# simon-ging/coot-videotext

Measured on AMD Instinct MI355X. Metric: clip-pairs/sec (COOT retrieval train step, whole job), higher is better.
Workload: dtype bf16; 1 GPU; ActivityNet-shaped paper config (anet_coot): 64 videos x 4 clips per GPU, Lc=Lv=80, Ls=16, Lp=64, Dv=2048, Dt=1536, d_model=384; global_batch_videos=64, parallelism=dp1, mode=train, launch=native, deterministic=True, batches=two different synthetic batches in turn

## Files before the change

### coot-videotext_amd/csrc/api.hip

```cpp
#include <stdarg.h>
#include <stdio.h>
#include <string.h>

#include <algorithm>
#include <mutex>
#include <string>
#include <unordered_map>
#include <vector>

#include "../../include/coot_hip.h"
#include "attention.h"
#include "common.h"
#include "fused.h"
#include "gemm.h"
#include "loss.h"
#include "pool.h"
#include "ref_f32.h"
#include "rowops.h"

namespace coot {

static thread_local char g_err[512] = "";
static thread_local hipStream_t g_glob_flush_stream = nullptr;
static thread_local hipEvent_t g_glob_flush_ev = nullptr;
// ... 454 lines not shown
    }
    f.tstamps = g_fz_tstamps;
    RUN(launch_pre_attn_bwd(f, st));
  } else {
    LnBwd l; l.dy = dz2; l.lddy = D; l.dy32 = dz2_f32; l.lddy32 = lddz2_f32; l.x = b.r2; l.x_f32 = 0; l.ldx = D; l.gain = P + lp.ln2g;
    l.R = rows_q; l.D = D; l.dx = w.dr2; l.lddx = D; l.dgain = G + lp.ln2g; l.dbias = G + lp.ln2b; l.dxcolsum = G + lp.b2;
    if (d_ff2.thr) { l.dxm = w.dr2m; l.lddxm = D; l.dxm_drop = d_ff2; l.dxm_drop_ld = D; }
    RUN(launch_ln_bwd(l, st));
  }
  const bf16_t* df2 = d_ff2.thr ? w.dr2m : w.dr2;
  if (!fused) {
    GemmNT g; g.X = df2; g.ldx = D; g.W = lw.w2_kn; g.ldw = D; g.M = rows_q; g.N = F; g.K = D;
    g.epi.act = 2; g.epi.aux = b.h1; g.epi.ldaux = F; g.epi.colsum = G + lp.b1; g.epi.out = w.dh1; g.epi.ldc = F;
    epi_drop(g.epi, mkdrop(train, pdrop, seed, site_base + SITE_FF1), F);
    RUN(launch_gemm_nt(g, st));
  }
  { GemmTN t; t.A = df2; t.lda = D; t.B = b.a1; t.ldb = F; t.T = rows_q; t.Mo = D; t.No = F; t.C = G + lp.w2; t.ldc = F; RUN(launch_gemm_tn(t, st)); }
  if (!fused) {
    GemmNT g; g.X = w.dh1; g.ldx = F; g.W = lw.w1_kn; g.ldw = F; g.M = rows_q; g.N = D; g.K = F;
    g.epi.res = w.dr2; g.epi.ldres = D; g.epi.out = w.dz1; g.epi.ldc = D;
    RUN(launch_gemm_nt(g, st));
  }
  { GemmTN t; t.A = w.dh1; t.lda = F; t.B = b.z1; t.ldb = D; t.T = rows_q; t.Mo = F; t.No = D; t.C = G + lp.w1; t.ldc = D; RUN(launch_gemm_tn(t, st)); }
  if (!fused) {
    LnBwd l; l.dy = w.dz1; l.lddy = D; l.x = b.r1; l.x_f32 = 0; l.ldx = D; l.gain = P + lp.ln1g; l.R = rows_q; l.D = D;
    l.dx = w.dr1; l.lddx = D; l.dgain = G + lp.ln1g; l.dbias = G + lp.ln1b; l.dxcolsum = G + lp.bo;
    l.drop = mkdrop(train, pdrop, seed, site_base + SITE_POSTLN);
    RUN(launch_ln_bwd(l, st));
  }
  if (!fused) {
    GemmNT g; g.X = w.dr1; g.ldx = D; g.W = lw.wo_kn; g.ldw = D; g.M = rows_q; g.N = D; g.K = D; g.epi.out = w.dctx; g.epi.ldc = D;
    RUN(launch_gemm_nt(g, st));
  }
  { GemmTN t; t.A = w.dr1; t.lda = D; t.B = b.ctx; t.ldb = D; t.T = rows_q; t.Mo = D; t.No = D; t.C = G + lp.wo; t.ldc = D; RUN(launch_gemm_tn(t, st)); }
  AttnArgs a; a.q = b.q; a.ldq = b.ldq; a.k = b.k; a.ldk = b.ldk; a.v = b.v; a.ldv = b.ldv; a.o = b.ctx; a.ldo = D; a.lse = b.lse;
  a.H = H; a.dh = dh; a.scale = 1.0f / sqrtf((float)dh);
  a.drop = mkdrop(train, pdrop, seed, site_base + SITE_ATTN);
  a.dout = w.dctx; a.lddo = D; a.delta = w.delta; a.dq = w.dq; a.lddq = w.lddq; a.dk = w.dk; a.lddk = w.lddk; a.dv = w.dv; a.lddv = w.lddv;
  RUN(attention_all(a, sg, !self, true, st));
  if (self) {
    { GemmTN t; t.A = w.dq; t.lda = 3 * D; t.B = xq; t.ldb = D; t.T = rows_q; t.Mo = 3 * D; t.No = D; t.C = G + lp.wqkv; t.ldc = D;
      t.a_colsum = G + lp.bq; RUN(launch_gemm_tn(t, st)); }
    if (qkv_bwd_is_fused(lw, rows_q, dxq_f32 != nullptr, part_ws)) {
      QkvBwd f; f.T = rows_q; f.dqkv = w.dq; f.wqkv = lw.f_wqkv_kn; f.res = w.dr1; f.aux = gelu_aux; f.dz = dxq; f.colsum = gelu_colsum; f.part = part_ws;
      f.colsum_overwrite = 1;
      RUN(launch_qkv_bwd(f, st));
    } else {
      GemmNT g; g.X = w.dq; g.ldx = 3 * D; g.W = lw.wqkv_kn; g.ldw = 3 * D; g.M = rows_q; g.N = D; g.K = 3 * D;
      g.epi.res = w.dr1; g.epi.ldres = D;
      if (gelu_aux) { g.epi.act = 2; g.epi.aux = gelu_aux; g.epi.ldaux = D; g.epi.colsum = gelu_colsum; }
      if (dxq_f32) { g.epi.out = dxq_f32; g.epi.out_f32 = 1; } else g.epi.out = dxq;
      g.epi.ldc = D;
      RUN(launch_gemm_nt(g, st));
    }
  } else {
    { GemmTN t; t.A = w.dq; t.lda = w.lddq; t.B = xq; t.ldb = D; t.T = rows_q; t.Mo = D; t.No = D; t.C = G + lp.wqkv; t.ldc = D;
      t.a_colsum = G + lp.bq; RUN(launch_gemm_tn(t, st)); }
    { GemmTN t; t.A = w.dk; t.lda = w.lddk; t.B = xkv; t.ldb = D; t.T = rows_kv; t.Mo = 2 * D; t.No = D; t.C = G + lp.wqkv + (size_t)D * D; t.ldc = D;
      t.a_colsum = G + lp.bk; RUN(launch_gemm_tn(t, st)); }
    {
      GemmNT g; g.X = w.dq; g.ldx = w.lddq; g.W = lw.wqkv_kn; g.ldw = 3 * D; g.M = rows_q; g.N = D; g.K = D;
      g.epi.res = w.dr1; g.epi.ldres = D;
      if (dxq_f32) { g.epi.out = dxq_f32; g.epi.out_f32 = 1; } else g.epi.out = dxq;
      g.epi.ldc = D;
      RUN(launch_gemm_nt(g, st));
    }
    {
      GemmNT g; g.X = w.dk; g.ldx = w.lddk; g.W = lw.wqkv_kn + D; g.ldw = 3 * D; g.M = rows_kv; g.N = D; g.K = 2 * D;
      g.epi.res = dxkv_accum; g.epi.ldres = D; g.epi.out = dxkv_accum; g.epi.ldc = D;
      RUN(launch_gemm_nt(g, st));
    }
  }
  return 0;
}

static int g_use_glob_fused_bwd = 1;
static int g_use_glob_fused = 1;
static bool glob_fused_ok(const coot_net_config& c, const Segs& sg) {
  return g_use_fused && g_use_glob_fused && fused_layer_ok(c) && c.num_heads == 8 && c.use_context && !c.use_input_fc && c.pooler != 0 &&
         c.num_layers == 1 && c.ctx_num_layers == 1 && sg.n == 1 && glob_fwd_supported(sg.L[0]);
}

static int g_use_packed = 1;
static bool packed_ok(const coot_net_config& c, const WPack& W, const Segs& sg, const coot_packed_seqs* pk) {
  if (!g_use_packed || !pk || !pk->cu_seqlens || pk->total_tokens <= 0) return false;
  return g_use_fused && g_use_fused_infc && c.use_input_fc && !c.use_context && fused_pool_ok(c) && W.f_in_w && W.f_pw1 &&
         W.f_pw1_kn && c.input_dim % 64 == 0 && pk->total_tokens >= g_fused_min_rows && pk->total_tokens <= sg.Tpad() &&
         attn_short_path(sg.L[0]) && (sg.n == 1 || attn_short_path(sg.L[1]));
}

static LayerBufs self_bufs(const LayerS& s, int D) {
  LayerBufs b; b.q = s.qkv; b.ldq = 3 * D; b.k = s.qkv + D; b.ldk = 3 * D; b.v = s.qkv + 2 * D; b.ldv = 3 * D;
  b.ctx = s.ctx; b.r1 = s.r1; b.z1 = s.z1; b.h1 = s.h1; b.a1 = s.a1; b.r2 = s.r2; b.z2 = s.z2; b.lse = s.lse;
  return b;
}
static LayerBufs ctx_bufs(const CtxS& s, int D) {
  LayerBufs b; b.q = s.q; b.ldq = D; b.k = s.kv; b.ldk = 2 * D; b.v = s.kv + D; b.ldv = 2 * D;
  b.ctx = s.cctx; b.r1 = s.r1; b.z1 = s.z1; b.h1 = s.h1; b.a1 = s.a1; b.r2 = s.r2; b.z2 = s.z2; b.lse = s.lse;
  return b;
}

}

using namespace coot;

extern "C" {

const char* coot_last_error(void) { return coot::g_err; }
int coot_version(void) { return COOT_ABI_VERSION; }
int coot_debug_dropout_scales(uint64_t seed, unsigned site, uint64_t idx0, int64_t n, float p, float* out_host) {
  COOT_REQUIRE(out_host && n >= 0 && p > 0.f, "debug_dropout_scales: bad arguments");
  const DropCfg d = mkdrop(1, p, seed, site);
  const unsigned key = drop_key(seed, site);
  for (int64_t i = 0; i < n; ++i) out_host[i] = drop_scale_key(key, idx0 + (uint64_t)i, d.thr, d.inv_keep);
  return 0;
}
int coot_debug_attn_dropout_scales(uint64_t seed, unsigned site, unsigned row32, int Lk, float p, float* out_host) {
  COOT_REQUIRE(out_host && Lk >= 0 && p > 0.f, "debug_attn_dropout_scales: bad arguments");
  const DropCfg d = mkdrop(1, p, seed, site);
  const unsigned key = drop_key(seed, site);
  for (int k = 0; k < Lk; ++k) out_host[k] = attn_drop_scale(key, row32, k, (unsigned)(Lk + 1) >> 1, d.thr, d.inv_keep);
  return 0;
}
int coot_debug_timestamps(void* dev_u64) { g_fz_tstamps = (unsigned long long*)dev_u64; return 0; }
extern "C" void coot_step_stamps_enable(int on);
extern "C" void coot_step_grad_write(int on);
extern "C" void coot_step_det_seg_flush(int on);
extern "C" int coot_step_det_seg_flush_get(void);
extern "C" int coot_internal_stage_hits(void);
extern "C" void coot_step_text_ahead(int on);
extern "C" int coot_step_text_ahead_get(void);
extern "C" int coot_internal_text_ahead_steps(void);
extern "C" int coot_internal_stream_counter(int which);
extern "C++" { namespace coot { int det_bypass_count(); int det_overflow_count(); int det_set_overflow_guard(int on); int det_overflow_guard(); } }
extern "C++" { namespace coot { void set_rt_topk_splits(int n); int get_rt_topk_splits(); void set_rt_few_splits(int n); int get_rt_few_splits(); void set_rt_grouped_splits(int n); int get_rt_grouped_splits(); void set_rt_knn_splits(int n); int get_rt_knn_splits(); void set_rt_comp_blocks_per_wg(int n); int get_rt_comp_blocks_per_wg(); } }
int coot_get_option(const char* name, int* value) {
  if (!value) { set_error("get_option: null result"); return -1; }
  if (!strcmp(name, "tn_dma")) { *value = get_tn_dma(); return 0; }
  if (!strcmp(name, "xcd_order")) { *value = get_xcd_order(); return 0; }
  if (!strcmp(name, "tn_mode")) { *value = get_tn_mode(); return 0; }
  if (!strcmp(name, "stage_hits")) { *value = coot_internal_stage_hits(); return 0; }
  if (!strcmp(name, "text_ahead")) { *value = coot_step_text_ahead_get(); return 0; }
  if (!strcmp(name, "text_ahead_steps")) { *value = coot_internal_text_ahead_steps(); return 0; }
  if (!strcmp(name, "fused_attn_launches")) { *value = fused_attn_launches(); return 0; }
  if (!strcmp(name, "stream_overlap_tests")) { *value = coot_internal_stream_counter(0); return 0; }
  if (!strcmp(name, "stream_candidates_rejected")) { *value = coot_internal_stream_counter(1); return 0; }
  if (!strcmp(name, "stream_unresolved")) { *value = coot_internal_stream_counter(2); return 0; }
  if (!strcmp(name, "operand_f16")) { *value = COOT_OPERAND_IS_F16; return 0; }
  if (!strcmp(name, "det_seg_flush")) { *value = coot_step_det_seg_flush_get(); return 0; }
  if (!strcmp(name, "det_bypasses")) { *value = det_bypass_count(); return 0; }
  if (!strcmp(name, "det_overflows")) { *value = det_overflow_count(); return 0; }
  if (!strcmp(name, "det_overflow_check")) { *value = det_overflow_guard(); return 0; }
  if (!strcmp(name, "attn_bwd_loop")) { *value = get_attn_bwd_loop(); return 0; }
  if (!strcmp(name, "attn_bwd_share")) { *value = get_attn_bwd_share(); return 0; }
  if (!strcmp(name, "attn_bwd_grid")) { *value = get_attn_bwd_grid(); return 0; }
  if (!strcmp(name, "rt_topk_splits")) { *value = get_rt_topk_splits(); return 0; }
  if (!strcmp(name, "rt_few_splits")) { *value = get_rt_few_splits(); return 0; }
  if (!strcmp(name, "rt_grouped_splits")) { *value = get_rt_grouped_splits(); return 0; }
  if (!strcmp(name, "rt_knn_splits")) { *value = get_rt_knn_splits(); return 0; }
  if (!strcmp(name, "rt_comp_blocks_per_wg")) { *value = get_rt_comp_blocks_per_wg(); return 0; }
  set_error("get_option: unknown or write-only option %s", name);
  return -2;
}
int coot_set_option(const char* name, int value) {
  if (!strcmp(name, "tn_mode")) { set_tn_mode(value); return 0; }
  if (!strcmp(name, "step_stamps")) { coot_step_stamps_enable(value); return 0; }
  if (!strcmp(name, "fused")) { g_use_fused = value; return 0; }
  if (!strcmp(name, "glob_fused")) { g_use_glob_fused = value; return 0; }
  if (!strcmp(name, "glob_fused_bwd")) { g_use_glob_fused_bwd = value; return 0; }
  if (!strcmp(name, "packed")) { g_use_packed = value; return 0; }
  if (!strcmp(name, "fused_infc")) { g_use_fused_infc = value; return 0; }
  if (!strcmp(name, "fused_attn")) { set_fused_attn(value); return 0; }
  if (!strcmp(name, "tn_dma")) { set_tn_dma(value); return 0; }
  if (!strcmp(name, "pack_lazy")) { g_pack_lazy = value; return 0; }
  if (!strcmp(name, "pack_poison")) { g_pack_poison = value; return 0; }
  if (!strcmp(name, "grad_poison")) { g_grad_poison = value; return 0; }
  if (!strcmp(name, "tn_target_wgs")) { set_tn_target_wgs(value); return 0; }
  if (!strcmp(name, "xcd_order")) { set_xcd_order(value); return 0; }
  if (!strcmp(name, "grad_write")) { coot_step_grad_write(value); return 0; }
  if (!strcmp(name, "det_seg_flush")) { coot_step_det_seg_flush(value); return 0; }
  if (!strcmp(name, "text_ahead")) { coot_step_text_ahead(value); return 0; }
  if (!strcmp(name, "det_overflow_check")) return det_set_overflow_guard(value);
  if (!strcmp(name, "glob_flush_aux")) { g_glob_flush_aux = value; return 0; }
  if (!strcmp(name, "pool_handover")) { g_pool_handover_on = value; return 0; }
  if (!strcmp(name, "cl_col_split")) { set_cl_col_split(value); return 0; }
  if (!strcmp(name, "cl_small")) { set_cl_small(value); return 0; }
  if (!strcmp(name, "fz_debug")) { g_fz_debug = value; return 0; }
  if (!strcmp(name, "fused_min_rows")) { g_fused_min_rows = value; return 0; }
  if (!strcmp(name, "attn_bwd_loop")) { set_attn_bwd_loop(value); return 0; }
  if (!strcmp(name, "attn_bwd_share")) { set_attn_bwd_share(value); return 0; }
  if (!strcmp(name, "attn_bwd_grid")) { set_attn_bwd_grid(value); return 0; }
  if (!strcmp(name, "rt_topk_splits")) { set_rt_topk_splits(value); return 0; }
  if (!strcmp(name, "rt_few_splits")) { set_rt_few_splits(value); return 0; }
  if (!strcmp(name, "rt_grouped_splits")) { set_rt_grouped_splits(value); return 0; }
  if (!strcmp(name, "rt_knn_splits")) { set_rt_knn_splits(value); return 0; }
  if (!strcmp(name, "rt_comp_blocks_per_wg")) { set_rt_comp_blocks_per_wg(value); return 0; }
  set_error("unknown option %s", name);
  return -2;
}

int64_t coot_net_param_numel(const coot_net_config* cfg) {
  coot_net_config c; if (norm_cfg(cfg, &c)) return -1;
  NetLayout L; build_layout(c, L); return L.total;
}
int coot_net_param_count(const coot_net_config* cfg) {
  coot_net_config c; if (norm_cfg(cfg, &c)) return -1;
  NetLayout L; build_layout(c, L); return (int)L.entries.size();
}
int coot_net_param_info(const coot_net_config* cfg, int index, char* name, int name_len, int64_t* offset, int64_t shape[4], int* ndim) {
  coot_net_config c; RUN(norm_cfg(cfg, &c));
  NetLayout L; build_layout(c, L);
  COOT_REQUIRE(index >= 0 && index < (int)L.entries.size(), "param index %d out of range", index);
  const PEntry& e = L.entries[index];
  snprintf(name, name_len, "%s", e.name.c_str());
  *offset = e.off; *ndim = e.ndim;
  for (int i = 0; i < 4; ++i) shape[i] = e.shape[i];
  return 0;
}
int coot_net_out_dim(const coot_net_config* cfg) { return cfg->hidden_dim * (cfg->use_context ? 2 : 1); }

size_t coot_net_wpack_bytes(const coot_net_config* cfg) {
  coot_net_config c; if (norm_cfg(cfg, &c)) return 0;
  Arena A(nullptr, 0); WPack W; layout_wpack(c, A, W); return A.off + 256;
}

enum { PACK_ALL = 0, PACK_FUSED = 1, PACK_PEROP_REST = 2 };
struct PackState { bool perop_fresh = false, perop_wanted = false; };
static std::mutex g_pack_mu;
static std::unordered_map<const void*, PackState> g_pack_state;
static PackState pack_state_get(const void* wpack) { std::lock_guard<std::mutex> lk(g_pack_mu); auto it = g_pack_state.find(wpack); return it == g_pack_state.end() ? PackState() : it->second; }
static void pack_state_set(const void* wpack, PackState s) { std::lock_guard<std::mutex> lk(g_pack_mu); g_pack_state[wpack] = s; }

static int pack_net_jobs(const coot_net_config* cfg, const float* P, void* wpack, const float* P0, void* wpack0, PackJobs& jobs, hipStream_t st,
                         int mode = PACK_ALL, bool* has_lazy = nullptr) {
  coot_net_config c; RUN(norm_cfg(cfg, &c));
  const int64_t pd = P - P0;
  NetLayout L; build_layout(c, L);
  Arena A(wpack, (size_t)-1); WPack W; layout_wpack(c, A, W);
  const int D = c.hidden_dim, F = c.ff_dim, Din = c.input_dim;
  auto flush = [&]() -> int { int rc = launch_pack_jobs(P0, wpack0, jobs, st); jobs.n = 0; jobs.mv = PackMatvec(); return rc; };
  auto add = [&](int64_t src_off, long lds, int R, int Cc, bf16_t* dst, long ldd, int transpose, int64_t colscale_off) -> int {
    if (jobs.n == 56) RUN(flush());
    PackJob& j = jobs.j[jobs.n++];
    j.src_off = src_off + pd; j.dst_byte_off = (char*)dst - (char*)wpack0; j.R = R; j.C = Cc; j.lds = lds; j.ldd = ldd;
    j.transpose = transpose; j.p48 = 0; j.colscale_off = colscale_off >= 0 ? colscale_off + pd : -1;
    return 0;
  };
  auto add48 = [&](int64_t src_off, long lds, int R, int Cc, bf16_t* dst, int transpose) -> int {
    RUN(add(src_off, lds, R, Cc, dst, 0, transpose, -1));
    jobs.j[jobs.n - 1].p48 = 1;
    return 0;
  };
  bool lazy = false;
  auto perop = [&](bool has_fused) { if (has_fused && mode == PACK_FUSED) lazy = true; return mode == PACK_ALL || (mode == PACK_FUSED ? !has_fused : has_fused); };
  const bool fused_on = mode != PACK_PEROP_REST;
  auto poison = [&](bf16_t* dst, size_t elems) -> int {
    if (!g_pack_poison || mode != PACK_FUSED) return 0;
    return check_hip(hipMemsetAsync(dst, 0xFF, elems * sizeof(bf16_t), st), "poison");
  };
  if (c.use_input_fc) {
    if (perop(W.f_in_w != nullptr)) RUN(add(L.in_w, Din, D, Din, W.in_w, Din, 0, L.n_gain));
    else RUN(poison(W.in_w, (size_t)D * Din));
    if (W.f_in_w && fused_on) { RUN(add(L.in_w, Din, D, Din, W.f_in_w, 0, 0, L.n_gain)); jobs.j[jobs.n - 1].p48 = 1; }
    if (fused_on) { jobs.mv.W = P + L.in_w; jobs.mv.ldw = Din; jobs.mv.N = D; jobs.mv.K = Din; jobs.mv.v = P + L.n_bias; jobs.mv.b = P + L.in_b; jobs.mv.out = W.in_bias; }
  }
  auto pack_layer = [&](const LayerP& lp, const LayerW& lw) -> int {
    if (perop(lw.f_wo != nullptr)) {
      RUN(add(lp.wqkv, D, 3 * D, D, lw.wqkv_nk, D, 0, -1));
      RUN(add(lp.wqkv, D, 3 * D, D, lw.wqkv_kn, 3 * D, 1, -1));
      RUN(add(lp.wo, D, D, D, lw.wo_nk, D, 0, -1));
      RUN(add(lp.wo, D, D, D, lw.wo_kn, D, 1, -1));
      RUN(add(lp.w1, D, F, D, lw.w1_nk, D, 0, -1));
      RUN(add(lp.w1, D, F, D, lw.w1_kn, F, 1, -1));
      RUN(add(lp.w2, F, D, F, lw.w2_nk, F, 0, -1));
      RUN(add(lp.w2, F, D, F, lw.w2_kn, D, 1, -1));
    } else {
      RUN(poison(lw.wqkv_nk, (size_t)(6 * D * D + 4 * F * D)));
    }
    if (lw.f_wo && fused_on) {
      RUN(add48(lp.wo, D, D, D, lw.f_wo, 0));
      RUN(add48(lp.w1, D, F, D, lw.f_w1, 0));
      RUN(add48(lp.w2, F, D, F, lw.f_w2, 0));
      RUN(add48(lp.wo, D, D, D, lw.f_wo_kn, 1));
      RUN(add48(lp.w1, D, F, D, lw.f_w1_kn, 1));
      RUN(add48(lp.w2, F, D, F, lw.f_w2_kn, 1));
      RUN(add48(lp.wqkv, D, 3 * D, D, lw.f_wqkv, 0));
      RUN(add48(lp.wqkv, D, 3 * D, D, lw.f_wqkv_kn, 1));
    }
    return 0;
  };
  for (int i = 0; i < c.num_layers; ++i) RUN(pack_layer(L.layers[i], W.layers[i]));
  for (size_t i = 0; i < L.ctx.size(); ++i) RUN(pack_layer(L.ctx[i], W.ctx[i]));
  if (c.pooler == 0) {
    const int H = c.pool_heads, PH = c.pool_hidden, dhp = PH / H, dop = D / H;
    const bool pool_perop = perop(W.f_pw1 != nullptr);
    if (!pool_perop) RUN(poison(W.pw1_nk, (size_t)(2 * PH * D + 2 * PH * dop)));
    for (int h = 0; h < H; ++h) {
      if (pool_perop) {
        RUN(add(L.pw1 + (int64_t)h * D * dhp, dhp, D, dhp, W.pw1_nk + (size_t)h * dhp * D, D, 1, -1));
        RUN(add(L.pw1 + (int64_t)h * D * dhp, dhp, D, dhp, W.pw1_kn + (size_t)h * dhp, PH, 0, -1));
        RUN(add(L.pw2 + (int64_t)h * dhp * dop, dop, dhp, dop, W.pw2_nk + (size_t)h * dop * dhp, dhp, 1, -1));
        RUN(add(L.pw2 + (int64_t)h * dhp * dop, dop, dhp, dop, W.pw2_kn + (size_t)h * dhp * dop, dop, 0, -1));
      }
      if (W.f_pw1 && fused_on) {
        RUN(add48(L.pw1 + (int64_t)h * D * dhp, dhp, D, dhp, W.f_pw1 + (size_t)h * dhp * D, 1));
        RUN(add48(L.pw2 + (int64_t)h * dhp * dop, dop, dhp, dop, W.f_pw2 + (size_t)h * dop * dhp, 1));
        RUN(add48(L.pw1 + (int64_t)h * D * dhp, dhp, D, dhp, W.f_pw1_kn + (size_t)h * D * dhp, 0));
        RUN(add48(L.pw2 + (int64_t)h * dhp * dop, dop, dhp, dop, W.f_pw2_kn + (size_t)h * dhp * dop, 0));
      }
    }
  }
  if (has_lazy) *has_lazy = lazy;
  return 0;
}

struct PerOpGuard { bool armed = false; coot_net_config cfg; const float* P = nullptr; void* wpack = nullptr; const char* lo[8]; const char* hi[8]; int n = 0; };
static thread_local PerOpGuard g_guard;
static int perop_weight_hook(const void* Wp, hipStream_t st) {
  PerOpGuard& G = g_guard;
  if (!G.armed) return 0;
  bool hit = false;
  for (int i = 0; i < G.n && !hit; ++i) hit = (const char*)Wp >= G.lo[i] && (const char*)Wp < G.hi[i];
  if (!hit) return 0;
  G.armed = false;
  PackJobs jobs;
  RUN(pack_net_jobs(&G.cfg, G.P, G.wpack, G.P, G.wpack, jobs, st, PACK_PEROP_REST));
  RUN(launch_pack_jobs(G.P, G.wpack, jobs, st));
  PackState ps; ps.perop_fresh = true; ps.perop_wanted = true;
  pack_state_set(G.wpack, ps);
  return 0;
}
struct PerOpGuardScope {
  PerOpGuardScope(const coot_net_config& c, const WPack& W, const float* P, const void* wpack) {
    PerOpGuard& G = g_guard;
    G.armed = false;
    if (pack_state_get(wpack).perop_fresh) return;
// ... 498 lines not shown
```

### coot-videotext_amd/csrc/fused.h

```cpp
#pragma once
#include "common.h"
#include "rowops.h"

namespace coot {

constexpr int FZ_D = 384;

__host__ __device__ inline long p48_offset(int n, int k, int K) {
  const int g = n / 48, b = (n % 48) / 16, r = n % 16, kb = k / 32, q = (k % 32) / 8, e = k % 8;
  return ((((long)g * (K / 32) + kb) * 3 + b) * 64 + (q * 16 + r)) * 8 + e;
}

struct FusedAttn {
  int on = 0;
  const bf16_t* qkv = nullptr;
  float* lse = nullptr;
  int N0 = 0, L0 = 0, N1 = 0, L1 = 0;
  const long long *lens0 = nullptr, *lens1 = nullptr;
  DropCfg drop; unsigned long long seed2_delta = 0;
  float scale = 0.f;
};
constexpr int FZ_ATTN_RP(int) { return 56; }
constexpr int FZ_ATTN_LMAX(int RF) { return RF == 8 ? 80 : 64; }
constexpr int FZ_ATTN_SMEM(int RF) { return RF >= 4 ? 8 * 2 * FZ_ATTN_LMAX(RF) * FZ_ATTN_RP(RF) * 2 : 0; }
struct PostAttnFwd {
  int T = 0;
  FusedAttn attn;
  bf16_t* ctx_w = nullptr;
  const bf16_t* ctx = nullptr;
  const bf16_t* xres = nullptr;
  const bf16_t *wo = nullptr, *w1 = nullptr, *w2 = nullptr, *pw1 = nullptr, *pw2 = nullptr;
  const float *bo = nullptr, *ln1g = nullptr, *ln1b = nullptr, *b1 = nullptr, *b2 = nullptr, *ln2g = nullptr, *ln2b = nullptr,
              *pb1 = nullptr, *pb2 = nullptr;
  bf16_t *r1 = nullptr, *z1 = nullptr, *h1 = nullptr, *a1 = nullptr, *r2 = nullptr, *z2 = nullptr;
  float* z2_f32 = nullptr; long ldz2_f32 = 0;
  int do_pool = 0;
  bf16_t *hp = nullptr, *ap = nullptr, *s = nullptr;
  DropCfg d_postln, d_ff1, d_ff2, d_pool1, d_pool2;
  unsigned long long* tstamps = nullptr;
};
int launch_post_attn_fwd(const PostAttnFwd& p, hipStream_t st);
bool post_attn_can_fuse_attention(int T, bool do_pool, int N0, int L0, int N1, int L1);
void set_fused_attn(int on);
int fused_attn_launches();

struct PreAttnBwd {
  int T = 0;
  int do_pool = 0;
  const bf16_t *ds = nullptr, *dzp = nullptr;
  const bf16_t* dz2 = nullptr;
  const bf16_t *hp = nullptr, *h1 = nullptr, *r2 = nullptr, *r1 = nullptr;
  const bf16_t *pw2 = nullptr, *pw1 = nullptr, *w2 = nullptr, *w1 = nullptr, *wo = nullptr;
  const float *ln2g = nullptr, *ln1g = nullptr;
  bf16_t *dhp = nullptr, *dr2 = nullptr, *dr2m = nullptr, *dh1 = nullptr, *dr1 = nullptr, *dctx = nullptr;
  float* part = nullptr;
  float *g_pb1 = nullptr, *g_ln2g = nullptr, *g_ln2b = nullptr, *g_b2 = nullptr, *g_b1 = nullptr, *g_ln1g = nullptr, *g_ln1b = nullptr,
        *g_bo = nullptr;
  DropCfg d_pool1, d_ff2, d_ff1, d_postln;
  unsigned long long* tstamps = nullptr;
};
struct InfcQkvFwd {
  int T = 0, Din = 0;
  const bf16_t* xhat = nullptr;
  const bf16_t* win = nullptr;
  const float* bin = nullptr;
  const float* pe = nullptr; int T0 = 0, L1 = 1, L2 = 1;
  const int* pos = nullptr;
  const bf16_t* wqkv = nullptr; const float* bqkv = nullptr;
  bf16_t *h0 = nullptr, *z0 = nullptr, *qkv = nullptr;
  unsigned long long* tstamps = nullptr;
};
int launch_infc_qkv_fwd(const InfcQkvFwd& p, hipStream_t st);

struct QkvFwd { int T = 0; const bf16_t* z = nullptr; const bf16_t* wqkv = nullptr; const float* bias = nullptr; bf16_t* qkv = nullptr; };
int launch_qkv_fwd(const QkvFwd& p, hipStream_t st);

struct QkvBwd {
  int T = 0;
  const bf16_t* dqkv = nullptr;
  const bf16_t* wqkv = nullptr;
  const bf16_t* res = nullptr;
  const bf16_t* aux = nullptr;
  bf16_t* dz = nullptr;
  float* colsum = nullptr;
  int colsum_overwrite = 0;
  float* part = nullptr;
};
int launch_qkv_bwd(const QkvBwd& p, hipStream_t st);

struct GlobLayerFwd {
  const bf16_t *wqkv = nullptr, *wo = nullptr, *w1 = nullptr, *w2 = nullptr;
  const float *bqkv = nullptr, *bo = nullptr, *ln1g = nullptr, *ln1b = nullptr, *b1 = nullptr, *b2 = nullptr, *ln2g = nullptr, *ln2b = nullptr;
  bf16_t* q = nullptr; long ldq = 0; bf16_t* k = nullptr; long ldk = 0; bf16_t* v = nullptr; long ldv = 0;
  bf16_t *ctx = nullptr, *r1 = nullptr, *z1 = nullptr, *h1 = nullptr, *a1 = nullptr, *r2 = nullptr, *z2 = nullptr; float* lse = nullptr;
  DropCfg d_attn, d_postln, d_ff1, d_ff2;
};
struct GlobFwd {
  int B = 0, Cmax = 0;
  const float* x = nullptr;
  const long long* lens = nullptr;
  const float* hidden = nullptr;
  const float* pe = nullptr;
  const float *n_gain = nullptr, *n_bias = nullptr;
  GlobLayerFwd self, ctx;
  bf16_t *z0 = nullptr, *cq_in = nullptr;
  float* pooled = nullptr;
  float* per_token = nullptr;
  int train = 0;
  int tiles = 0, warm_per_xcd = 0, xcd_first = 0, xcd_count = 8, tiles_per_xcd = 0;
  unsigned long long* tstamps = nullptr;
};
int launch_glob_fwd(const GlobFwd& p, hipStream_t st);
bool glob_fwd_supported(int Cmax);

struct GlobLayerBwd {
  const bf16_t *wqkv_kn = nullptr, *wo_kn = nullptr, *w1_kn = nullptr, *w2_kn = nullptr;
  const float *ln1g = nullptr, *ln2g = nullptr;
  const bf16_t* q = nullptr; long ldq = 0; const bf16_t* k = nullptr; long ldk = 0; const bf16_t* v = nullptr; long ldv = 0;
  const bf16_t *r1 = nullptr, *h1 = nullptr, *r2 = nullptr; const float* lse = nullptr;
  bf16_t *dr2 = nullptr, *dr2m = nullptr, *dh1 = nullptr, *dr1 = nullptr;
  bf16_t* dq = nullptr; long lddq = 0; bf16_t* dk = nullptr; long lddk = 0; bf16_t* dv = nullptr; long lddv = 0;
  float *g_ln2g = nullptr, *g_ln2b = nullptr, *g_ln1g = nullptr, *g_ln1b = nullptr;
  DropCfg d_attn, d_postln, d_ff1, d_ff2;
};
struct GlobBwd {
  int B = 0, Cmax = 0;
  const float* x = nullptr;
  const long long* lens = nullptr;
  const float* n_gain = nullptr;
  const float* dpooled = nullptr;
  GlobLayerBwd self, ctx;
  float* dx = nullptr;
  float* dhidden = nullptr;
  float *g_n_gain = nullptr, *g_n_bias = nullptr;
  int tiles = 0, warm_per_xcd = 0, xcd_first = 0, xcd_count = 8, tiles_per_xcd = 0;
  unsigned long long* tstamps = nullptr;
};
int launch_glob_bwd(const GlobBwd& p, hipStream_t st);
void glob_xcd_set(int first, int count);

constexpr int FZ_BWD_NCS = 9 * FZ_D;
bool half_tiles(int T, int kernel);
int launch_pre_attn_bwd(const PreAttnBwd& p, hipStream_t st);

}
```

### coot-videotext_amd/csrc/fused.hip

```cpp
#include "fused.h"
#include "det.h"
#include "gemm.h"

#include <type_traits>

namespace coot {
namespace {

constexpr int APITCH = 400;
constexpr int SPITCH = 388;
constexpr int NTHR = 512;
constexpr long GSZ = 12L * 3 * 512;

__device__ __forceinline__ void unpack8(u32x4_t u, float* v) {
  v[0] = bflo(u[0]); v[1] = bfhi(u[0]); v[2] = bflo(u[1]); v[3] = bfhi(u[1]);
  v[4] = bflo(u[2]); v[5] = bfhi(u[2]); v[6] = bflo(u[3]); v[7] = bfhi(u[3]);
}
__device__ __forceinline__ u32x4_t pack8(const float* v) {
  return u32x4_t{pack2bf(v[0], v[1]), pack2bf(v[2], v[3]), pack2bf(v[4], v[5]), pack2bf(v[6], v[7])};
}
__device__ __forceinline__ void load8f(const float* p, float* v) {
  const f32x4_t a = reinterpret_cast<const f32x4_t*>(p)[0], b = reinterpret_cast<const f32x4_t*>(p)[1];
  v[0] = a[0]; v[1] = a[1]; v[2] = a[2]; v[3] = a[3]; v[4] = b[0]; v[5] = b[1]; v[6] = b[2]; v[7] = b[3];
}
__device__ __forceinline__ void drop8(const DropCfg& d, unsigned long long idx0, float* sc) {
  drop_scales<8>(eff_seed(d.seed, d.seed_ptr), d.site, idx0, d.thr, d.inv_keep, sc);
}

__device__ __forceinline__ u32x4_t gld16(const void* base, unsigned boff) {
  return *reinterpret_cast<const u32x4_t*>(reinterpret_cast<const char*>(base) + boff);
}
__device__ __forceinline__ void gst16(void* base, unsigned boff, u32x4_t v) {
#ifdef FZ_NO_STORES
  if (boff != 0xFFFFFFF0u) return;
#endif
  *reinterpret_cast<u32x4_t*>(reinterpret_cast<char*>(base) + boff) = v;
}

#ifdef FZ_XCDS
__device__ __forceinline__ int fz_tile_index(int ntiles) {
  const int x = blockIdx.x & 7;
  if (x >= FZ_XCDS) return -1;
  const int t = (blockIdx.x >> 3) * FZ_XCDS + x;
  return t < ntiles ? t : -1;
}
static inline int fz_grid(int tiles) { return (tiles + FZ_XCDS - 1) / FZ_XCDS * 8; }
#else
__device__ __forceinline__ int fz_tile_index(int) { return blockIdx.x; }
static inline int fz_grid(int tiles) { return tiles; }
#endif

__device__ __forceinline__ void lds_barrier() { asm volatile("s_waitcnt lgkmcnt(0)\n\ts_barrier" ::: "memory"); }

template <int RF>
__device__ __forceinline__ void zero_acc(f32x4_t (&acc)[RF][3]) {
#pragma unroll
  for (int a = 0; a < RF; ++a)
#pragma unroll
    for (int b = 0; b < 3; ++b) acc[a][b] = f32x4_t{0.f, 0.f, 0.f, 0.f};
}

constexpr int kPdFull = 2;
#ifndef FZ_PD_SMALL
#define FZ_PD_SMALL 5
#endif
constexpr int kPdSmall = FZ_PD_SMALL;
constexpr int kCarryMaxRF = 4;
template <int PD_, bool CARRY_>
struct WRing { static constexpr int PD = PD_, NB = PD_ + 1; static constexpr bool CARRY = CARRY_; bf16x8_t w[PD_ + 1][3]; };
template <int RF> using TileRing = WRing<(RF <= 2 ? kPdSmall : kPdFull), (RF <= kCarryMaxRF)>;

template <typename Ring>
__device__ __forceinline__ void gemm_load_first(Ring& R, const bf16_t* wg, int lane) {
  const bf16x8_t* wp = reinterpret_cast<const bf16x8_t*>(wg) + lane;
#ifndef FZ_NO_WLOAD
#pragma unroll
  for (int s = 0; s < Ring::PD; ++s)
#pragma unroll
    for (int b = 0; b < 3; ++b) R.w[s][b] = wp[(s * 3 + b) * 64];
#else
  (void)wp;
#endif
  __builtin_amdgcn_sched_barrier(0);
}
template <typename Ring>
__device__ __forceinline__ void gemm_issue(Ring& R, const bf16_t* wg, int lane) {
  if constexpr (Ring::CARRY) gemm_load_first(R, wg, lane);
}

template <int RF, int KB, bool NEXT, typename Ring>
__device__ __forceinline__ void gemm_run(Ring& R, const bf16_t* As, const bf16_t* wg, const bf16_t* next, f32x4_t (&acc)[RF][3], int lane) {
  constexpr int PD = Ring::PD, NB = Ring::NB;
  static_assert(KB % NB == 0 && KB >= PD, "the ring must wrap at the end of a pass");
  asm volatile("" : "+v"(lane));
  if constexpr (!Ring::CARRY) gemm_load_first(R, wg, lane);
  const bf16_t* arow = As + (lane & 15) * APITCH + (lane >> 4) * 8;
  const bf16x8_t* wp = reinterpret_cast<const bf16x8_t*>(wg) + lane;
  const bf16x8_t* np = reinterpret_cast<const bf16x8_t*>(next) + lane;
  bf16x8_t xf[RF];
#pragma unroll
  for (int a = 0; a < RF; ++a) xf[a] = *reinterpret_cast<const bf16x8_t*>(arow + a * 16 * APITCH);
#pragma unroll
  for (int kb = 0; kb < KB; ++kb) {
#ifndef FZ_NO_WLOAD
    if (kb + PD < KB) {
#pragma unroll
      for (int b = 0; b < 3; ++b) R.w[(kb + PD) % NB][b] = wp[((kb + PD) * 3 + b) * 64];
    } else if constexpr (NEXT && Ring::CARRY) {
#pragma unroll
      for (int b = 0; b < 3; ++b) R.w[(kb + PD) % NB][b] = np[((kb + PD - KB) * 3 + b) * 64];
    }
#else
    (void)wp; (void)np;
#endif
    __builtin_amdgcn_sched_barrier(0);
#pragma unroll
    for (int a = 0; a < RF; ++a) {
#pragma unroll
      for (int b = 0; b < 3; ++b) {
#ifndef FZ_NO_MFMA
        acc[a][b] = COOT_MFMA_16x16x32(R.w[kb % NB][b], xf[a], acc[a][b]);
#else
        acc[a][b][0] += __builtin_bit_cast(float, (int)(__builtin_bit_cast(u32x4_t, R.w[kb % NB][b])[0] ^ __builtin_bit_cast(u32x4_t, xf[a])[b]));
#endif
      }
      if (kb + 1 < KB) xf[a] = *reinterpret_cast<const bf16x8_t*>(arow + a * 16 * APITCH + (kb + 1) * 32);
    }
  }
}

template <int RF, int CPR = 48>
__device__ __forceinline__ void load_tile(bf16_t* As, const bf16_t* src, long ld, int col0, int row0) {
  constexpr int CH = 16 * RF * CPR, IT = (CH + NTHR - 1) / NTHR;
  asm volatile("" : "+s"(row0));
  u32x4_t v[IT];
#pragma unroll
  for (int i = 0; i < IT; ++i) {
    const int c = threadIdx.x + NTHR * i, rl = c / CPR, ch = c - rl * CPR;
    v[i] = u32x4_t{0u, 0u, 0u, 0u};
    if (CH % NTHR == 0 || c < CH) v[i] = gld16(src, (unsigned)((row0 + rl) * (int)ld + col0 + ch * 8) * 2u);
  }
#pragma unroll
  for (int i = 0; i < IT; ++i) {
    const int c = threadIdx.x + NTHR * i, rl = c / CPR, ch = c - rl * CPR;
    if (CH % NTHR == 0 || c < CH) *reinterpret_cast<u32x4_t*>(&As[rl * APITCH + ch * 8]) = v[i];
  }
}

template <int NCH, int IT>
__device__ __forceinline__ void load_bias(const float* bias, float (&bs)[IT][8]) {
#pragma unroll
  for (int i = 0; i < IT; ++i) load8f(bias + ((threadIdx.x + NTHR * i) % NCH) * 8, bs[i]);
}

template <int RF, int NCG, typename PreF, typename Fn>
__device__ __forceinline__ void epilogue(f32x4_t (&acc)[RF * NCG / 8][3], float* Stg, bf16_t* As, int row0, const float* bias_lds,
                                         PreF pre, Fn fn, bool to_lds, unsigned long long* prof = nullptr) {
#ifdef FZ_PROFILE_EPI
  unsigned long long pt[7] = {0, 0, 0, 0, 0, 0, 0}, pacc[6] = {0, 0, 0, 0, 0, 0};
  const bool profiling = prof && blockIdx.x == 0 && threadIdx.x == 0;
#define FZ_PT(k) do { if (prof) { asm volatile("s_waitcnt lgkmcnt(0)" ::: "memory"); pt[k] = __builtin_amdgcn_s_memtime(); } } while (0)
#else
#define FZ_PT(k) do { } while (0)
#endif
  constexpr int RR = RF >= 2 ? 32 : 16, FR = RR / 16, RPR = (NCG == 8 ? RR : 2 * RR), ROUNDS = 16 * RF / RPR, CH = RR * 48, IT = CH / NTHR;
  static_assert(CH % NTHR == 0 && IT == 3 && ROUNDS <= 4 && (NCG == 8 || (NCG == 4 && ((ROUNDS == 2 && RF == 8) || (ROUNDS == 1 && RF == 4)))),
                "tile pass geometry");
  int tid = threadIdx.x;
  asm volatile("" : "+v"(tid));
  const int lane = tid & 63, wave = tid >> 6;
  const int cg = wave % NCG, rh = wave / NCG;
  int rl[IT], col[IT];
#pragma unroll
  for (int i = 0; i < IT; ++i) {
    const int c = tid + NTHR * i, r_ = c / 48, ch = c - r_ * 48;
    if constexpr (NCG == 8) { rl[i] = r_; col[i] = ch * 8; }
    else { rl[i] = r_ + (ch >= 24 ? 32 : 0); col[i] = (ch >= 24 ? ch - 24 : ch) * 8; }
  }
  float bs[IT][8];
  if (bias_lds) {
#pragma unroll
    for (int i = 0; i < IT; ++i) load8f(bias_lds + col[i], bs[i]);
  }
  using P = decltype(pre(0, 0));
  P pv[IT];
#pragma unroll
  for (int i = 0; i < IT; ++i) pv[i] = pre(row0 + rl[i], col[i]);
  float* sw = &Stg[(lane & 15) * SPITCH + cg * 48 + (lane >> 4) * 4];
#pragma unroll 1
  for (int r = 0; r < ROUNDS; ++r) {
    FZ_PT(0);
    lds_barrier();
    FZ_PT(1);
#ifndef FZ_NO_STAGING
    if constexpr (NCG == 8) {
      auto put = [&](auto rc) {
        constexpr int R = decltype(rc)::value;
        if constexpr (R < ROUNDS) {
#pragma unroll
          for (int a2 = 0; a2 < FR; ++a2)
#pragma unroll
            for (int b = 0; b < 3; ++b) *reinterpret_cast<f32x4_t*>(sw + a2 * 16 * SPITCH + b * 16) = acc[R * FR + a2][b];
          asm volatile("" ::: "memory");
        }
      };
      switch (r) {
        case 0: put(std::integral_constant<int, 0>{}); break;
        case 1: put(std::integral_constant<int, 1>{}); break;
        case 2: put(std::integral_constant<int, 2>{}); break;
        default: put(std::integral_constant<int, 3>{}); break;
      }
    } else if constexpr (RF == 8) {
      if (rh == r) {
#pragma unroll
        for (int a = 0; a < 4; ++a)
#pragma unroll
          for (int b = 0; b < 3; ++b) *reinterpret_cast<f32x4_t*>(sw + (a & 1) * 16 * SPITCH + (a >> 1) * 192 + b * 16) = acc[a][b];
      }
    } else {
#pragma unroll
      for (int a = 0; a < 2; ++a)
#pragma unroll
        for (int b = 0; b < 3; ++b) *reinterpret_cast<f32x4_t*>(sw + a * 16 * SPITCH + rh * 192 + b * 16) = acc[a][b];
    }
#else
    if (r == 0) {
#pragma unroll
      for (int a = 0; a < RF * NCG / 8; ++a)
#pragma unroll
        for (int b = 0; b < 3; ++b) asm volatile("" :: "v"(acc[a][b]));
    }
#endif
    const int rbase = row0 + r * RPR;
    FZ_PT(2);
    lds_barrier();
    FZ_PT(3);
    float v[IT][8];
#pragma unroll
    for (int i = 0; i < IT; ++i) load8f(&Stg[(rl[i] & 31) * SPITCH + col[i] + (rl[i] >= 32 ? 192 : 0)], v[i]);
    FZ_PT(4);
#pragma unroll
    for (int i = 0; i < IT; ++i) {
      if (bias_lds) {
#pragma unroll
        for (int j = 0; j < 8; ++j) v[i][j] += bs[i][j];
      }
      fn(rbase + rl[i], col[i], v[i], pv[i], i);
      __builtin_amdgcn_sched_barrier(0);
    }
    FZ_PT(5);
    if (to_lds) {
#pragma unroll
      for (int i = 0; i < IT; ++i) *reinterpret_cast<u32x4_t*>(&As[(r * RPR + rl[i]) * APITCH + col[i]]) = pack8(v[i]);
    }
    if (r + 1 < ROUNDS) {
#pragma unroll
      for (int i = 0; i < IT; ++i) pv[i] = pre(rbase + RPR + rl[i], col[i]);
    }
    FZ_PT(6);
#ifdef FZ_PROFILE_EPI
    if (prof) {
#pragma unroll
      for (int k = 0; k < 6; ++k) pacc[k] += pt[k + 1] - pt[k];
    }
#endif
  }
  lds_barrier();
#ifdef FZ_PROFILE_EPI
  if (profiling) {
#pragma unroll
    for (int k = 0; k < 6; ++k) prof[k] = pacc[k];
  }
#endif
#undef FZ_PT
}

__device__ __forceinline__ float row16_sum(float v) {
  auto dpp = [](float x, auto ctrl) {
    return __builtin_bit_cast(float, __builtin_amdgcn_update_dpp(0, __builtin_bit_cast(int, x), decltype(ctrl)::value, 0xF, 0xF, false));
  };
  v += dpp(v, std::integral_constant<int, 0xB1>{});
  v += dpp(v, std::integral_constant<int, 0x4E>{});
  v += dpp(v, std::integral_constant<int, 0x141>{});
  v += dpp(v, std::integral_constant<int, 0x140>{});
  return v;
}

struct DropK { unsigned key = 0, thr = 0; float inv_keep = 1.f; };
__device__ __forceinline__ DropK resolve_drop(const DropCfg& d, unsigned long long base) {
  DropK k; k.key = drop_key(d.seed + base, d.site); k.thr = d.thr; k.inv_keep = d.inv_keep; return k;
}

__device__ __forceinline__ float attn_drop_f(unsigned key, unsigned row, int k, unsigned lk_half, unsigned thr, float inv_keep) {
  return attn_drop_scale(key, row, k, lk_half, thr, inv_keep);
}

template <bool DROP>
__device__ __forceinline__ void apply_drop(const DropK& d, unsigned long long idx0, float (&v)[8]) {
#ifdef FZ_NO_EPI_MATH
  return;
#endif
  if constexpr (DROP) {
    float sc[8];
    drop_scales_key<8>(d.key, idx0, d.thr, d.inv_keep, sc);
#pragma unroll
    for (int j = 0; j < 8; ++j) v[j] *= sc[j];
  }
}

template <bool DROP>
__device__ __forceinline__ void mask_from_saved(const DropK& d, const float (&saved)[8], float (&v)[8]) {
  if constexpr (DROP) {
#ifdef FZ_NO_EPI_MATH
    return;
#endif
#pragma unroll
    for (int j = 0; j < 8; ++j) v[j] = saved[j] != 0.0f ? v[j] * d.inv_keep : 0.0f;
  }
}

template <int RF, bool DROP, bool OUT32, bool MASK = false>
__device__ __forceinline__ void ln_tile(bf16_t* As, const float* gain, const float* bias, int row0, int T, bf16_t* out, float* out32,
                                        long ld32, const DropK& drop) {
#ifdef FZ_NO_LN
  return;
#endif
  asm volatile("" : "+s"(row0));
  const int lane = threadIdx.x & 63, wave = threadIdx.x >> 6, j16 = lane & 15, g = lane >> 4;
  constexpr int RW = 2 * RF, ITR = (RW + 3) / 4;
  float gn[3][8], bi[3][8];
#pragma unroll
  for (int m = 0; m < 3; ++m) { load8f(gain + m * 128 + j16 * 8, gn[m]); load8f(bias + m * 128 + j16 * 8, bi[m]); }
#pragma unroll
  for (int it = 0; it < ITR; ++it) {
    const int rw = (RW >= 4) ? it * 4 + g : (g < RW ? g : 0);
    const int rl = wave * RW + rw, row = row0 + rl;
    bf16_t* ar = As + rl * APITCH + j16 * 8;
    float x[3][8];
    float s = 0.f;
#pragma unroll
    for (int m = 0; m < 3; ++m) {
      unpack8(*reinterpret_cast<const u32x4_t*>(ar + m * 128), x[m]);
#pragma unroll
      for (int e = 0; e < 8; ++e) s += x[m][e];
    }
    const float mean = row16_sum(s) * (1.0f / 384.0f);
    float q = 0.f;
#pragma unroll
    for (int m = 0; m < 3; ++m)
#pragma unroll
      for (int e = 0; e < 8; ++e) { x[m][e] -= mean; q += x[m][e] * x[m][e]; }
    const float rs = 1.0f / (sqrtf(row16_sum(q) * (1.0f / 383.0f)) + kLnEps);
#pragma unroll
    for (int m = 0; m < 3; ++m) {
      float y[8];
#pragma unroll
      for (int e = 0; e < 8; ++e) y[e] = x[m][e] * rs * gn[m][e] + bi[m][e];
      if constexpr (DROP) {
        float sc[8];
        drop_scales_key<8>(drop.key, (unsigned long long)row * FZ_D + m * 128 + j16 * 8, drop.thr, drop.inv_keep, sc);
#pragma unroll
        for (int e = 0; e < 8; ++e) y[e] *= sc[e];
      }
      const u32x4_t o = pack8(y);
      *reinterpret_cast<u32x4_t*>(ar + m * 128) = o;
      if (!MASK || row < T) gst16(out, (unsigned)(row * FZ_D + m * 128 + j16 * 8) * 2u, o);
      if constexpr (OUT32) {
        if (row < T) {
          float* o32 = out32 + (long)row * ld32 + m * 128 + j16 * 8;
          *reinterpret_cast<f32x4_t*>(o32) = f32x4_t{y[0], y[1], y[2], y[3]};
          *reinterpret_cast<f32x4_t*>(o32 + 4) = f32x4_t{y[4], y[5], y[6], y[7]};
        }
      }
    }
  }
}

struct PreNone {};
struct PreRes { u32x4_t res; };

template <int RF>
__device__ __forceinline__ void fused_self_attn(const PostAttnFwd& p, bf16_t* As, unsigned char* smem_base, int row0, unsigned long long sbase) {
  constexpr int DH = 48, RP = FZ_ATTN_RP(RF), NK = DH / 16, H = 8, CPR = DH / 8, LDQ = 3 * FZ_D, LMAX = FZ_ATTN_LMAX(RF);
  const FusedAttn& A = p.attn;
  int tid = threadIdx.x;
  asm volatile("" : "+v"(tid));
  const int lane = tid & 63, h = tid >> 6, lq = lane & 15, lg = lane >> 4;
  const int T0 = A.N0 * A.L0;
  const bool second = row0 >= T0;
  const int L = second ? A.L1 : A.L0, segbase = second ? T0 : 0, segend = second ? p.T : T0;
  const long long* lens = second ? A.lens1 : A.lens0;
  const int last = (row0 + 16 * RF < segend ? row0 + 16 * RF : segend) - 1;
  const int s_first = (row0 - segbase) / L, s_last = (last - segbase) / L;
  const int nkt = L >> 4;
  const unsigned dkey = A.drop.thr ? drop_key(A.drop.seed + (second ? A.seed2_delta : 0ull) + sbase, A.drop.site) : 0u;
  bf16_t* Ks = reinterpret_cast<bf16_t*>(smem_base) + h * (2 * LMAX * RP);
  bf16_t* Vs = Ks + LMAX * RP;
  u32x2_t out[RF][NK];
#pragma unroll
  for (int f = 0; f < RF; ++f)
#pragma unroll
    for (int dt = 0; dt < NK; ++dt) out[f][dt] = u32x2_t{0u, 0u};
  const int half = L * CPR;
  constexpr bool QALL = RF <= 4;
  s16x4_t qall[QALL ? RF : 1][NK];
  if constexpr (QALL) {
#pragma unroll
    for (int f = 0; f < RF; ++f)
#pragma unroll
      for (int ks = 0; ks < NK; ++ks) {
        qall[f][ks] = s16x4_t{0, 0, 0, 0};
        if (row0 + 16 * f < segend) qall[f][ks] = *reinterpret_cast<const s16x4_t*>(A.qkv + (long)(row0 + 16 * f + lq) * LDQ + h * DH + ks * 16 + lg * 4);
      }
  }
  constexpr int NH = (LMAX * CPR + 63) / 64;
  u32x4_t sk[NH], sv[NH];
  auto ld = [&](int kb0, int kv, u32x4_t (&st)[NH]) {
#pragma unroll
    for (int i = 0; i < NH; ++i) {
      const int c = lane + 64 * i, r = c / CPR, ch = c - r * CPR;
      st[i] = u32x4_t{0u, 0u, 0u, 0u};
      if (c < half) st[i] = gld16(A.qkv, (unsigned)((kb0 + r) * LDQ + FZ_D * (1 + kv) + h * DH + ch * 8) * 2u);
    }
  };
  auto sto = [&](bf16_t* dst, const u32x4_t (&st)[NH]) {
#pragma unroll
    for (int i = 0; i < NH; ++i) {
      const int c = lane + 64 * i, r = c / CPR, ch = c - r * CPR;
      if (c < half) *reinterpret_cast<u32x4_t*>(&dst[r * RP + ch * 8]) = st[i];
    }
  };
  constexpr bool KVPRE = RF <= 4;
  if constexpr (KVPRE) { ld(segbase + s_first * L, 0, sk); ld(segbase + s_first * L, 1, sv); }
#pragma unroll 1
  for (int sq = s_first; sq <= s_last; ++sq) {
    const int kbase = segbase + sq * L;
    if constexpr (!KVPRE) { ld(kbase, 0, sk); ld(kbase, 1, sv); }
    asm volatile("s_waitcnt lgkmcnt(0)" ::: "memory");
    sto(Ks, sk);
    sto(Vs, sv);
    if constexpr (KVPRE) { if (sq < s_last) { ld(kbase + L, 0, sk); ld(kbase + L, 1, sv); } }
    asm volatile("s_waitcnt lgkmcnt(0)" ::: "memory");
    const int nvalid = (int)lens[sq];
    const int f_lo = kbase > row0 ? (kbase - row0) >> 4 : 0;
    const int f_hi_row = (kbase + L < row0 + 16 * RF ? kbase + L : row0 + 16 * RF);
    const int f_hi = ((f_hi_row < segend ? f_hi_row : segend) - row0) >> 4;
    s16x4_t qnext[NK];
    auto qload = [&](int f, s16x4_t (&q)[NK]) {
#pragma unroll
      for (int ks = 0; ks < NK; ++ks) q[ks] = *reinterpret_cast<const s16x4_t*>(A.qkv + (long)(row0 + 16 * f + lq) * LDQ + h * DH + ks * 16 + lg * 4);
    };
    if constexpr (!QALL) { if (f_lo < f_hi) qload(f_lo, qnext); }
#pragma unroll
    for (int f = 0; f < RF; ++f) {
      if (f >= f_lo && f < f_hi) {
        const int g0 = row0 + 16 * f, qpos = g0 - kbase + lq;
        s16x4_t qf[NK];
#pragma unroll
        for (int ks = 0; ks < NK; ++ks) {
          if constexpr (QALL) qf[ks] = qall[f][ks];
          else qf[ks] = qnext[ks];
        }
        if constexpr (!QALL) { if (f + 1 < f_hi) qload(f + 1, qnext); }
        f32x4_t sc[LMAX / 16];
        float mx = -INFINITY;
#pragma unroll
        for (int kt = 0; kt < LMAX / 16; ++kt) {
          if (kt < nkt) {
            sc[kt] = f32x4_t{0.f, 0.f, 0.f, 0.f};
#pragma unroll
            for (int ks = 0; ks < NK; ++ks) {
              const s16x4_t kf = *reinterpret_cast<const s16x4_t*>(&Ks[(kt * 16 + lq) * RP + ks * 16 + lg * 4]);
              sc[kt] = COOT_MFMA_16x16x16(kf, qf[ks], sc[kt]);
            }
#pragma unroll
            for (int i = 0; i < 4; ++i) {
              float v = sc[kt][i] * A.scale;
              if (kt * 16 + lg * 4 + i >= nvalid) v = kMaskFill;
              sc[kt][i] = v;
              mx = fmaxf(mx, v);
            }
          }
        }
        mx = fmaxf(mx, __shfl_xor(mx, 16, 64));
        mx = fmaxf(mx, __shfl_xor(mx, 32, 64));
        float sum = 0.f;
        s16x4_t pf[LMAX / 16];
#pragma unroll
        for (int kt = 0; kt < LMAX / 16; ++kt) {
          if (kt < nkt) {
            float pr[4];
#pragma unroll
            for (int i = 0; i < 4; ++i) {
              pr[i] = __expf(sc[kt][i] - mx);
              sum += pr[i];
              if (A.drop.thr)
                pr[i] *= attn_drop_f(dkey, (unsigned)((sq * H + h) * L + qpos), kt * 16 + lg * 4 + i, (unsigned)(L + 1) >> 1, A.drop.thr, A.drop.inv_keep);
            }
            const unsigned lo = pack2bf(pr[0], pr[1]), hi = pack2bf(pr[2], pr[3]);
            pf[kt] = s16x4_t{(short)(lo & 0xFFFF), (short)(lo >> 16), (short)(hi & 0xFFFF), (short)(hi >> 16)};
          }
        }
        sum += __shfl_xor(sum, 16, 64);
        sum += __shfl_xor(sum, 32, 64);
        const float inv = 1.0f / sum;
#pragma unroll
        for (int dt = 0; dt < NK; ++dt) {
          f32x4_t o = f32x4_t{0.f, 0.f, 0.f, 0.f};
#pragma unroll
          for (int kt = 0; kt < LMAX / 16; ++kt) {
            if (kt < nkt) {
              const bf16_t* addr = &Vs[(kt * 16) * RP + dt * 16] + (4 * lg + (lq >> 2)) * RP + (lq & 3) * 4;
              const s16x4_t vt = __builtin_amdgcn_ds_read_tr16_b64_v4i16((s16x4_t __attribute__((address_space(3)))*)(addr));
              o = COOT_MFMA_16x16x16(vt, pf[kt], o);
            }
          }
          out[f][dt] = u32x2_t{pack2bf(o[0] * inv, o[1] * inv), pack2bf(o[2] * inv, o[3] * inv)};
        }
// ... 298 lines not shown
    const int col = ((tid + NTHR * i) % 48) * 8;
    lds_barrier();
    *reinterpret_cast<f32x4_t*>(&red[k * FZ_D + col]) = f32x4_t{cs[i][0], cs[i][1], cs[i][2], cs[i][3]};
    *reinterpret_cast<f32x4_t*>(&red[k * FZ_D + col + 4]) = f32x4_t{cs[i][4], cs[i][5], cs[i][6], cs[i][7]};
    lds_barrier();
    if (tid < FZ_D) {
      const int ch = (tid / 8 + 48 * 2 - 32 * i) % 48;
      const int nk = (NTHR - ch + 47) / 48;
      for (int kk = 0; kk < nk; ++kk) tot += red[kk * FZ_D + tid];
    }
  }
  if (tid < FZ_D) dst[tid] = tot;
}

template <int RF, bool DROP>
__global__ __launch_bounds__(512) void pre_attn_bwd_kernel(PreAttnBwd p) {
  constexpr int BT = 16 * RF, RR = 32;
  constexpr long GSZ192 = 6L * 3 * 512;
  __shared__ __attribute__((aligned(16))) unsigned char smem[BT * APITCH * 2 + RR * SPITCH * 4 + 4 * FZ_D * 4];
  bf16_t* As = reinterpret_cast<bf16_t*>(smem);
  float* Stg = reinterpret_cast<float*>(smem + BT * APITCH * 2);
  float* Bsm = reinterpret_cast<float*>(smem + BT * APITCH * 2 + RR * SPITCH * 4);
  float* zero = Bsm, *g2 = Bsm + FZ_D, *g1 = Bsm + 2 * FZ_D, *cred = Bsm + 3 * FZ_D;
  const int lane = threadIdx.x & 63, wave = threadIdx.x >> 6;
  const int row0 = blockIdx.x * BT, T = p.T;
  float* part = p.part + (long)blockIdx.x * FZ_BWD_NCS;
  if (threadIdx.x < FZ_D / 4) {
    reinterpret_cast<f32x4_t*>(zero)[threadIdx.x] = f32x4_t{0.f, 0.f, 0.f, 0.f};
    reinterpret_cast<f32x4_t*>(g2)[threadIdx.x] = reinterpret_cast<const f32x4_t*>(p.ln2g)[threadIdx.x];
    reinterpret_cast<f32x4_t*>(g1)[threadIdx.x] = reinterpret_cast<const f32x4_t*>(p.ln1g)[threadIdx.x];
  }
  f32x4_t acc[RF][3];
  float cs[3][8];
  int tsn = 0;
  auto stamp = [&]() {
    unsigned long long* ts = p.tstamps;
    asm volatile("" : "+s"(ts));
    if (ts && blockIdx.x == 0 && threadIdx.x == 0) ts[tsn] = __builtin_amdgcn_s_memtime();
    ++tsn;
  };
  unsigned long long sbase = 0;
  if constexpr (DROP) { if (p.d_ff1.seed_ptr) sbase = *p.d_ff1.seed_ptr; }
  const DropK d_postln = resolve_drop(p.d_postln, sbase), d_ff1 = resolve_drop(p.d_ff1, sbase), d_ff2 = resolve_drop(p.d_ff2, sbase),
                d_pool1 = resolve_drop(p.d_pool1, sbase);
  stamp();
  auto cs_zero = [&]() {
#pragma unroll
    for (int i = 0; i < 3; ++i)
#pragma unroll
      for (int j = 0; j < 8; ++j) cs[i][j] = 0.f;
  };

  TileRing<RF> R;
  auto WG = [&](const bf16_t* base, int grp, long gsz) { asm volatile("" : "+v"(grp)); return base + grp * gsz; };
  if (p.do_pool) {
    gemm_issue(R, WG(p.pw2, wave, GSZ192), lane);
#pragma unroll 1
    for (int h = 0; h < 2; ++h) {
      load_tile<RF, 24>(As, p.ds, FZ_D, h * (FZ_D / 2), row0);
      __syncthreads();
      zero_acc<RF>(acc);
      gemm_run<RF, 6, true>(R, As, WG(p.pw2, h * 8 + wave, GSZ192), h == 0 ? WG(p.pw2, 8 + wave, GSZ192) : WG(p.pw1, 8 + wave, GSZ), acc, lane);
      cs_zero();
      epilogue<RF, 8>(acc, Stg, As, row0, nullptr,
          [&](int row, int col) { return PreRes{gld16(p.hp, (unsigned)(row * (2 * FZ_D) + h * FZ_D + col) * 2u)}; },
          [&](int row, int col, float (&v)[8], const PreRes& pr, int i) {
            float a[8];
            unpack8(pr.res, a);
#pragma unroll
            for (int j = 0; j < 8; ++j) v[j] *= gelu_grad_f(a[j]);
#ifdef FZ_HASH_BWD_MASKS
            apply_drop<DROP>(d_pool1, (unsigned long long)row * (2 * FZ_D) + h * FZ_D + col, v);
#else
            mask_from_saved<DROP>(d_pool1, a, v);
#endif
            if (row < T) {
#pragma unroll
              for (int j = 0; j < 8; ++j) cs[i][j] += v[j];
            }
            gst16(p.dhp, (unsigned)(row * (2 * FZ_D) + h * FZ_D + col) * 2u, pack8(v));
          }, true);
      colsum_flush(cs, Stg, part + h * FZ_D);
      stamp();
    }
    zero_acc<RF>(acc);
    gemm_run<RF, 12, true>(R, As, WG(p.pw1, 8 + wave, GSZ), WG(p.pw1, wave, GSZ), acc, lane);
    __syncthreads();
    load_tile<RF>(As, p.dhp, 2 * FZ_D, 0, row0);
    __syncthreads();
    gemm_run<RF, 12, true>(R, As, WG(p.pw1, wave, GSZ), WG(p.w2, wave, GSZ), acc, lane);
    epilogue<RF, 8>(acc, Stg, As, row0, nullptr,
        [&](int row, int col) { return PreRes{gld16(p.dzp, (unsigned)(row * FZ_D + col) * 2u)}; },
        [&](int, int, float (&v)[8], const PreRes& pr, int) {
          float r[8];
          unpack8(pr.res, r);
#pragma unroll
          for (int j = 0; j < 8; ++j) v[j] += r[j];
        }, true);
  } else {
    gemm_issue(R, WG(p.w2, wave, GSZ), lane);
    load_tile<RF>(As, p.dz2, FZ_D, 0, row0);
    __syncthreads();
  }
  stamp();
  ln_bwd_tile<RF, false, DROP>(As, g2, p.r2, row0, T, p.dr2, p.dr2m, d_ff2, d_ff2, Stg, part + 2 * FZ_D);
  stamp();
  zero_acc<RF>(acc);
  gemm_run<RF, 12, true>(R, As, WG(p.w2, wave, GSZ), WG(p.w1, wave, GSZ), acc, lane);
  cs_zero();
  epilogue<RF, 8>(acc, Stg, As, row0, nullptr,
      [&](int row, int col) { return PreRes{gld16(p.h1, (unsigned)(row * FZ_D + col) * 2u)}; },
      [&](int row, int col, float (&v)[8], const PreRes& pr, int i) {
        float a[8];
        unpack8(pr.res, a);
#pragma unroll
        for (int j = 0; j < 8; ++j) v[j] *= gelu_grad_f(a[j]);
#ifdef FZ_HASH_BWD_MASKS
        apply_drop<DROP>(d_ff1, (unsigned long long)row * FZ_D + col, v);
#else
        mask_from_saved<DROP>(d_ff1, a, v);
#endif
        if (row < T) {
#pragma unroll
          for (int j = 0; j < 8; ++j) cs[i][j] += v[j];
        }
        gst16(p.dh1, (unsigned)(row * FZ_D + col) * 2u, pack8(v));
      }, true);
  colsum_flush(cs, Stg, part + 5 * FZ_D);
  stamp();
  zero_acc<RF>(acc);
  gemm_run<RF, 12, true>(R, As, WG(p.w1, wave, GSZ), WG(p.wo, wave, GSZ), acc, lane);
  epilogue<RF, 8>(acc, Stg, As, row0, nullptr,
      [&](int row, int col) { return PreRes{gld16(p.dr2, (unsigned)(row * FZ_D + col) * 2u)}; },
      [&](int, int, float (&v)[8], const PreRes& pr, int) {
        float r[8];
        unpack8(pr.res, r);
#pragma unroll
        for (int j = 0; j < 8; ++j) v[j] += r[j];
      }, true);
  stamp();
  ln_bwd_tile<RF, DROP, false>(As, g1, p.r1, row0, T, p.dr1, nullptr, d_postln, d_postln, Stg, part + 6 * FZ_D);
  stamp();
  zero_acc<RF>(acc);
  gemm_run<RF, 12, false>(R, As, WG(p.wo, wave, GSZ), nullptr, acc, lane);
  epilogue<RF, 8>(acc, Stg, As, row0, nullptr, [&](int, int) { return PreNone{}; },
      [&](int row, int col, float (&v)[8], const PreNone&, int) { gst16(p.dctx, (unsigned)(row * FZ_D + col) * 2u, pack8(v)); }, false);
  stamp();
}


template <bool SELF, bool DROP>
__device__ __forceinline__ void tile_attn(const bf16_t* Qs, const bf16_t* Ks, const bf16_t* Vs, bf16_t* Os, float* Sc, int nq, int Lk,
                                          int seq0, const long long* lens, float scale, const DropK& dk, bf16_t* o_glob, float* lse_glob,
                                          int grow0) {
  const int tid = threadIdx.x, pair = tid >> 1, half = tid & 1, r = pair >> 3, h = pair & 7;
  const bool on = r < nq;
  const int sl = on ? (SELF ? r / Lk : r) : 0;
  const int kr0 = sl * Lk;
  const int nvalid = on ? (int)lens[seq0 + sl] : 0;
  const int coff = h * 48 + half * 24;
  float q[24];
#pragma unroll
  for (int c = 0; c < 3; ++c) unpack8(*reinterpret_cast<const u32x4_t*>(&Qs[(on ? r : 0) * APITCH + coff + c * 8]), &q[c * 8]);
  float m = -3.0e38f;
  for (int j = 0; j < Lk; ++j) {
    float kk[24];
#pragma unroll
    for (int c = 0; c < 3; ++c) unpack8(*reinterpret_cast<const u32x4_t*>(&Ks[(kr0 + j) * APITCH + coff + c * 8]), &kk[c * 8]);
    float sv = 0.f;
#pragma unroll
    for (int c = 0; c < 24; ++c) sv += q[c] * kk[c];
    sv += __shfl_xor(sv, 1, 64);
    sv *= scale;
    if (j >= nvalid) sv = kMaskFill;
    if (half == 0) Sc[pair * 32 + j] = sv;
    m = fmaxf(m, sv);
  }
  asm volatile("s_waitcnt lgkmcnt(0)" ::: "memory");
  float sum = 0.f;
  for (int j = 0; j < Lk; ++j) sum += __expf(Sc[pair * 32 + j] - m);
  const float lse = m + __logf(sum);
  float o[24];
#pragma unroll
  for (int c = 0; c < 24; ++c) o[c] = 0.f;
  const unsigned mrow = SELF ? (unsigned)(((seq0 + sl) * 8 + h) * Lk + (r - kr0)) : (unsigned)((seq0 + sl) * 8 + h);
  for (int j = 0; j < Lk; ++j) {
    float pj = __expf(Sc[pair * 32 + j] - lse);
    if constexpr (DROP) pj *= attn_drop_f(dk.key, mrow, j, (unsigned)(Lk + 1) >> 1, dk.thr, dk.inv_keep);
    float vv[24];
#pragma unroll
    for (int c = 0; c < 3; ++c) unpack8(*reinterpret_cast<const u32x4_t*>(&Vs[(kr0 + j) * APITCH + coff + c * 8]), &vv[c * 8]);
#pragma unroll
    for (int c = 0; c < 24; ++c) o[c] += pj * vv[c];
  }
  if (r < 32) {
#pragma unroll
    for (int c = 0; c < 3; ++c) {
      const u32x4_t pk = on ? pack8(&o[c * 8]) : u32x4_t{0u, 0u, 0u, 0u};
      *reinterpret_cast<u32x4_t*>(&Os[r * APITCH + coff + c * 8]) = pk;
      if (on) gst16(o_glob, (unsigned)((grow0 + r) * FZ_D + coff + c * 8) * 2u, pk);
    }
    if (on && half == 0) lse_glob[(long)(grow0 + r) * 8 + h] = lse;
  }
}

__device__ __forceinline__ void l2_prefetch(const bf16_t* const (&ws)[8], int h, int n) {
  constexpr unsigned SZQKV = 3u * FZ_D * FZ_D * 2u, SZ = FZ_D * FZ_D * 2u, PIECE = 8192u;
  unsigned x = 0;
#pragma unroll
  for (int a = 0; a < 8; ++a) {
    const unsigned bytes = (a & 3) == 0 ? SZQKV : SZ;
    for (unsigned piece = (unsigned)h; piece * PIECE < bytes; piece += (unsigned)n) {
      const u32x4_t v = gld16(ws[a], piece * PIECE + threadIdx.x * 16u);
      x ^= v[0];
    }
  }
  asm volatile("" :: "v"(x));
}

template <typename P>
__device__ __forceinline__ int glob_tile_or_help(const P& p, const bf16_t* const (&ws)[8]) {
  const int b = blockIdx.x, xr = (b & 7) - p.xcd_first, slot = b >> 3;
  if (xr < 0 || xr >= p.xcd_count) return -1;
  if (slot < p.tiles_per_xcd) {
    const int tile = slot * p.xcd_count + xr;
    return tile < p.tiles ? tile : -1;
  }
  l2_prefetch(ws, slot - p.tiles_per_xcd, p.warm_per_xcd);
  return -1;
}

template <bool DROP, bool OUT32>
__device__ __forceinline__ void glob_chain_fwd(bf16_t* As, float* Stg, const GlobLayerFwd& L, const bf16_t* xres, int row0, int rowEnd,
                                               float* z2_f32, long ldz2_f32, unsigned long long sbase, TileRing<2>& R, const bf16_t* next) {
  constexpr int RF = 2;
  const int lane = threadIdx.x & 63, wave = threadIdx.x >> 6;
  const DropK d_postln = resolve_drop(L.d_postln, sbase), d_ff1 = resolve_drop(L.d_ff1, sbase), d_ff2 = resolve_drop(L.d_ff2, sbase);
  f32x4_t acc[RF][3];
  zero_acc<RF>(acc);
  gemm_run<RF, 12, true>(R, As, L.wo + wave * GSZ, L.w1 + wave * GSZ, acc, lane);
  epilogue<RF, 8>(acc, Stg, As, row0, L.bo,
      [&](int row, int col) { return PreRes{row < rowEnd ? gld16(xres, (unsigned)(row * FZ_D + col) * 2u) : u32x4_t{0u, 0u, 0u, 0u}}; },
      [&](int row, int col, float (&v)[8], const PreRes& pr, int) {
        float r[8];
        unpack8(pr.res, r);
#pragma unroll
        for (int j = 0; j < 8; ++j) v[j] += r[j];
        if (row < rowEnd) gst16(L.r1, (unsigned)(row * FZ_D + col) * 2u, pack8(v));
      }, true);
  ln_tile<RF, DROP, false, true>(As, L.ln1g, L.ln1b, row0, rowEnd, L.z1, nullptr, 0, d_postln);
  __syncthreads();
  zero_acc<RF>(acc);
  gemm_run<RF, 12, true>(R, As, L.w1 + wave * GSZ, L.w2 + wave * GSZ, acc, lane);
  epilogue<RF, 8>(acc, Stg, As, row0, L.b1, [&](int, int) { return PreNone{}; },
      [&](int row, int col, float (&v)[8], const PreNone&, int) {
        apply_drop<DROP>(d_ff1, (unsigned long long)row * FZ_D + col, v);
        if (row < rowEnd) gst16(L.h1, (unsigned)(row * FZ_D + col) * 2u, pack8(v));
#pragma unroll
        for (int j = 0; j < 8; ++j) v[j] = gelu_f(v[j]);
        if (row < rowEnd) gst16(L.a1, (unsigned)(row * FZ_D + col) * 2u, pack8(v));
      }, true);
  zero_acc<RF>(acc);
  gemm_run<RF, 12, true>(R, As, L.w2 + wave * GSZ, next, acc, lane);
  __syncthreads();
  epilogue<RF, 8>(acc, Stg, As, row0, L.b2,
      [&](int row, int col) { return PreRes{row < rowEnd ? gld16(L.z1, (unsigned)(row * FZ_D + col) * 2u) : u32x4_t{0u, 0u, 0u, 0u}}; },
      [&](int row, int col, float (&v)[8], const PreRes& pr, int) {
        float r[8];
        unpack8(pr.res, r);
        apply_drop<DROP>(d_ff2, (unsigned long long)row * FZ_D + col, v);
#pragma unroll
        for (int j = 0; j < 8; ++j) v[j] += r[j];
        if (row < rowEnd) gst16(L.r2, (unsigned)(row * FZ_D + col) * 2u, pack8(v));
      }, true);
  {
    const DropK none;
    ln_tile<RF, false, OUT32, true>(As, L.ln2g, L.ln2b, row0, rowEnd, L.z2, z2_f32, ldz2_f32, none);
  }
  __syncthreads();
}

template <bool DROP>
__global__ __launch_bounds__(512) void glob_fwd_kernel(GlobFwd p) {
  constexpr int RF = 2, BT = 32;
  __shared__ __attribute__((aligned(16))) unsigned char smem[4 * BT * APITCH * 2 + BT * SPITCH * 4];
  static_assert(BT * SPITCH * 4 >= 256 * 32 * 4, "the staging buffer holds the attention scores [256 pairs][32 keys]");
  bf16_t* As = reinterpret_cast<bf16_t*>(smem);
  bf16_t* Qs = As + BT * APITCH;
  bf16_t* Ks = Qs + BT * APITCH;
  bf16_t* Vs = Ks + BT * APITCH;
  float* Stg = reinterpret_cast<float*>(smem + 4 * BT * APITCH * 2);
  const int tid = threadIdx.x, lane = tid & 63, wave = tid >> 6;
  const int Cm = p.Cmax, G = 32 / Cm;
  int tile;
  {
    const bf16_t* ws[8] = {p.self.wqkv, p.self.wo, p.self.w1, p.self.w2, p.ctx.wqkv, p.ctx.wo, p.ctx.w1, p.ctx.w2};
    tile = glob_tile_or_help(p, ws);
    if (tile < 0) return;
  }
  const int v0 = tile * G, nv = (p.B - v0) < G ? (p.B - v0) : G;
  const int row0 = v0 * Cm, nrows = nv * Cm, rowEnd = row0 + nrows;
  unsigned long long sbase = 0;
  if constexpr (DROP) { if (p.self.d_ff1.seed_ptr) sbase = *p.self.d_ff1.seed_ptr; }
  const float scale = 0.14433756729740643f;
  f32x4_t acc[RF][3];
  int tsn = 0;
  auto stamp = [&]() { if (p.tstamps && tile == 0 && threadIdx.x == 0) p.tstamps[tsn] = __builtin_amdgcn_s_memtime(); ++tsn; };
  stamp();
  TileRing<RF> R;
  gemm_issue(R, p.self.wqkv + wave * GSZ, lane);

  {
    const int j16 = lane & 15, g = lane >> 4, rl = wave * 4 + g, row = row0 + rl;
    const bool on = rl < nrows;
    float x[3][8];
    float s = 0.f;
#pragma unroll
    for (int m = 0; m < 3; ++m) {
      if (on) load8f(p.x + (long)row * FZ_D + m * 128 + j16 * 8, x[m]);
      else {
#pragma unroll
        for (int e = 0; e < 8; ++e) x[m][e] = 0.f;
      }
#pragma unroll
      for (int e = 0; e < 8; ++e) s += x[m][e];
    }
    const float mean = row16_sum(s) * (1.0f / 384.0f);
    float qq = 0.f;
#pragma unroll
    for (int m = 0; m < 3; ++m)
#pragma unroll
      for (int e = 0; e < 8; ++e) { x[m][e] -= mean; qq += x[m][e] * x[m][e]; }
    const float rs = 1.0f / (sqrtf(row16_sum(qq) * (1.0f / 383.0f)) + kLnEps);
    const int pos = rl % Cm;
#pragma unroll
    for (int m = 0; m < 3; ++m) {
      const int col = m * 128 + j16 * 8;
      float gn[8], bi[8], pe[8], y[8];
      load8f(p.n_gain + col, gn); load8f(p.n_bias + col, bi); load8f(p.pe + (long)pos * FZ_D + col, pe);
#pragma unroll
      for (int e = 0; e < 8; ++e) y[e] = on ? x[m][e] * rs * gn[e] + bi[e] + pe[e] : 0.f;
      const u32x4_t o = pack8(y);
      *reinterpret_cast<u32x4_t*>(&As[rl * APITCH + col]) = o;
      if (on) gst16(p.z0, (unsigned)(row * FZ_D + col) * 2u, o);
    }
  }
  __syncthreads();
  stamp();

#pragma unroll 1
  for (int q = 0; q < 3; ++q) {
    zero_acc<RF>(acc);
    gemm_run<RF, 12, true>(R, As, p.self.wqkv + (q * 8 + wave) * GSZ, q < 2 ? p.self.wqkv + ((q + 1) * 8 + wave) * GSZ : p.self.wo + wave * GSZ, acc, lane);
    bf16_t* dst = q == 0 ? Qs : (q == 1 ? Ks : Vs);
    epilogue<RF, 8>(acc, Stg, dst, row0, p.self.bqkv + q * FZ_D, [&](int, int) { return PreNone{}; },
        [&](int row, int col, float (&v)[8], const PreNone&, int) {
          if (row < rowEnd) gst16(p.self.q, (unsigned)(row * (3 * FZ_D) + q * FZ_D + col) * 2u, pack8(v));
        }, true);
    stamp();
  }
  __syncthreads();
  {
    const DropK dk = resolve_drop(p.self.d_attn, sbase);
    tile_attn<true, DROP>(Qs, Ks, Vs, As, Stg, nrows, Cm, v0, p.lens, scale, dk, p.self.ctx, p.self.lse, row0);
  }
  __syncthreads();
  stamp();
  {
    const bf16_t* nx = p.ctx.wqkv + (8 + wave) * GSZ;
    if (p.per_token) glob_chain_fwd<DROP, true>(As, Stg, p.self, p.z0, row0, rowEnd, p.per_token, FZ_D, sbase, R, nx);
    else glob_chain_fwd<DROP, false>(As, Stg, p.self, p.z0, row0, rowEnd, nullptr, 0, sbase, R, nx);
  }
  stamp();

  if (tid < FZ_D) {
    for (int gv = 0; gv < nv; ++gv) {
      float a = 0.f;
      for (int j = 0; j < Cm; ++j) a += bf2f(As[(gv * Cm + j) * APITCH + tid]);
      p.pooled[(long)(v0 + gv) * (2 * FZ_D) + tid] = a / (float)p.lens[v0 + gv];
    }
  }

#pragma unroll 1
  for (int q = 1; q < 3; ++q) {
    zero_acc<RF>(acc);
    gemm_run<RF, 12, true>(R, As, p.ctx.wqkv + (q * 8 + wave) * GSZ, q == 1 ? p.ctx.wqkv + (16 + wave) * GSZ : p.ctx.wqkv + wave * GSZ, acc, lane);
    bf16_t* dst = q == 1 ? Ks : Vs;
    bf16_t* gdst = q == 1 ? p.ctx.k : p.ctx.v;
    const int ldkv = (int)(q == 1 ? p.ctx.ldk : p.ctx.ldv);
    epilogue<RF, 8>(acc, Stg, dst, row0, p.ctx.bqkv + q * FZ_D, [&](int, int) { return PreNone{}; },
        [&](int row, int col, float (&v)[8], const PreNone&, int) {
          if (row < rowEnd) gst16(gdst, (unsigned)(row * ldkv + col) * 2u, pack8(v));
        }, true);
  }
  __syncthreads();
  stamp();
  {
    for (int c = tid; c < BT * 48; c += 512) {
      const int rl = c / 48, ch = c - rl * 48;
      u32x4_t o = {0u, 0u, 0u, 0u};
      if (rl < nv) {
        float h[8];
        load8f(p.hidden + (long)(v0 + rl) * FZ_D + ch * 8, h);
        o = pack8(h);
        gst16(p.cq_in, (unsigned)((v0 + rl) * FZ_D + ch * 8) * 2u, o);
      }
      *reinterpret_cast<u32x4_t*>(&As[rl * APITCH + ch * 8]) = o;
    }
  }
  __syncthreads();
  zero_acc<RF>(acc);
  gemm_run<RF, 12, true>(R, As, p.ctx.wqkv + wave * GSZ, p.ctx.wo + wave * GSZ, acc, lane);
  epilogue<RF, 8>(acc, Stg, Qs, v0, p.ctx.bqkv, [&](int, int) { return PreNone{}; },
      [&](int row, int col, float (&v)[8], const PreNone&, int) {
        if (row < v0 + nv) gst16(p.ctx.q, (unsigned)(row * (int)p.ctx.ldq + col) * 2u, pack8(v));
      }, true);
  __syncthreads();
  stamp();
  {
    const DropK dk = resolve_drop(p.ctx.d_attn, sbase);
    tile_attn<false, DROP>(Qs, Ks, Vs, As, Stg, nv, Cm, v0, p.lens, scale, dk, p.ctx.ctx, p.ctx.lse, v0);
  }
  __syncthreads();
  stamp();
  glob_chain_fwd<DROP, true>(As, Stg, p.ctx, p.cq_in, v0, v0 + nv, p.pooled + FZ_D, 2 * FZ_D, sbase, R, p.ctx.w2 + wave * GSZ );
  stamp();
}


template <int NQ>
__device__ __forceinline__ void rows_colsum_flush(const float (&cs)[NQ][3][8], float* red, float* const (&dst)[NQ]) {
  const int lane = threadIdx.x & 63, wave = threadIdx.x >> 6, j16 = lane & 15, g = lane >> 4;
  const int rl = wave * 4 + g;
#pragma unroll
  for (int m = 0; m < 3; ++m) {
    lds_barrier();
#pragma unroll
    for (int q = 0; q < NQ; ++q) {
      float* w = red + rl * (NQ * 128) + q * 128 + j16 * 8;
      *reinterpret_cast<f32x4_t*>(w) = f32x4_t{cs[q][m][0], cs[q][m][1], cs[q][m][2], cs[q][m][3]};
      *reinterpret_cast<f32x4_t*>(w + 4) = f32x4_t{cs[q][m][4], cs[q][m][5], cs[q][m][6], cs[q][m][7]};
    }
    lds_barrier();
    if (threadIdx.x < NQ * 128) {
      float v = 0.f;
#pragma unroll 8
      for (int r = 0; r < 32; ++r) v += red[r * (NQ * 128) + threadIdx.x];
      float* d = dst[threadIdx.x / 128];
      if (d) acc_add(d + m * 128 + (threadIdx.x & 127), v);
    }
  }
  lds_barrier();
}

template <bool DROPY, bool MASKX, bool DY32, bool X32>
__device__ __forceinline__ void glob_ln_bwd(bf16_t* As, const float* dy32, long lddy32, const void* xsrc, const float* gain, int row0, int rowEnd,
                                            bf16_t* out_dx, bf16_t* out_dxm, float* out32, const DropK& dy_drop, const DropK& dx_drop, float* red,
                                            float* g_gain, float* g_bias) {
  const int lane = threadIdx.x & 63, wave = threadIdx.x >> 6, j16 = lane & 15, g = lane >> 4;
  const int rl = wave * 4 + g, row = row0 + rl;
  const bool on = row < rowEnd;
  float x[3][8], dy[3][8], gn[3][8];
  float s = 0.f;
#pragma unroll
  for (int m = 0; m < 3; ++m) {
    const int col = m * 128 + j16 * 8;
    load8f(gain + col, gn[m]);
#pragma unroll
    for (int e = 0; e < 8; ++e) { x[m][e] = 0.f; dy[m][e] = 0.f; }
    if (on) {
      if constexpr (X32) load8f(reinterpret_cast<const float*>(xsrc) + (long)row * FZ_D + col, x[m]);
      else unpack8(gld16(xsrc, (unsigned)(row * FZ_D + col) * 2u), x[m]);
      if constexpr (DY32) load8f(dy32 + (long)row * lddy32 + col, dy[m]);
      else unpack8(*reinterpret_cast<const u32x4_t*>(&As[rl * APITCH + col]), dy[m]);
      if constexpr (DROPY) {
        float sc[8];
        drop_scales_key<8>(dy_drop.key, (unsigned long long)row * FZ_D + col, dy_drop.thr, dy_drop.inv_keep, sc);
#pragma unroll
        for (int e = 0; e < 8; ++e) dy[m][e] *= sc[e];
      }
    }
#pragma unroll
    for (int e = 0; e < 8; ++e) s += x[m][e];
  }
  const float mu = row16_sum(s) * (1.0f / 384.0f);
  float q = 0.f, hs = 0.f, hx = 0.f;
#pragma unroll
  for (int m = 0; m < 3; ++m)
#pragma unroll
    for (int e = 0; e < 8; ++e) {
      x[m][e] -= mu;
      q += x[m][e] * x[m][e];
      const float h = dy[m][e] * gn[m][e];
      hs += h; hx += h * x[m][e];
    }
  q = row16_sum(q); hs = row16_sum(hs); hx = row16_sum(hx);
  const float stdv = sqrtf(q * (1.0f / 383.0f));
  const float rs = 1.0f / (stdv + kLnEps), hmean = hs * (1.0f / 384.0f);
  const float k2 = stdv > 0.f ? hx * rs * rs / (383.0f * stdv) : 0.f;
  float cs[2][3][8];
#pragma unroll
  for (int m = 0; m < 3; ++m) {
    const int col = m * 128 + j16 * 8;
    float dx[8], dm[8];
#pragma unroll
    for (int e = 0; e < 8; ++e) dx[e] = (dy[m][e] * gn[m][e] - hmean) * rs - k2 * x[m][e];
    if constexpr (MASKX) {
      float sc[8];
      drop_scales_key<8>(dx_drop.key, (unsigned long long)row * FZ_D + col, dx_drop.thr, dx_drop.inv_keep, sc);
#pragma unroll
      for (int e = 0; e < 8; ++e) dm[e] = dx[e] * sc[e];
    } else {
#pragma unroll
      for (int e = 0; e < 8; ++e) dm[e] = dx[e];
    }
#pragma unroll
    for (int e = 0; e < 8; ++e) {
      cs[0][m][e] = on ? dy[m][e] * x[m][e] * rs : 0.f;
      cs[1][m][e] = on ? dy[m][e] : 0.f;
    }
    const u32x4_t om = on ? pack8(dm) : u32x4_t{0u, 0u, 0u, 0u};
    *reinterpret_cast<u32x4_t*>(&As[rl * APITCH + col]) = om;
    if (on) {
      const unsigned boff = (unsigned)(row * FZ_D + col) * 2u;
      if (out_dx) gst16(out_dx, boff, pack8(dx));
      if constexpr (MASKX) gst16(out_dxm, boff, om);
      if (out32) {
        float* o32 = out32 + (long)row * FZ_D + col;
        *reinterpret_cast<f32x4_t*>(o32) = f32x4_t{dx[0], dx[1], dx[2], dx[3]};
        *reinterpret_cast<f32x4_t*>(o32 + 4) = f32x4_t{dx[4], dx[5], dx[6], dx[7]};
      }
    }
  }
  float* const dst[2] = {g_gain, g_bias};
  rows_colsum_flush<2>(cs, red, dst);
}

__device__ __forceinline__ void load_rows32(bf16_t* Ts, const bf16_t* src, long ld, int col0, int grow0, int nvalid) {
  for (int c = threadIdx.x; c < 32 * 48; c += NTHR) {
    const int rl = c / 48, ch = c - rl * 48;
    u32x4_t v = {0u, 0u, 0u, 0u};
    if (rl < nvalid) v = gld16(src, (unsigned)((grow0 + rl) * (int)ld + col0 + ch * 8) * 2u);
    *reinterpret_cast<u32x4_t*>(&Ts[rl * APITCH + ch * 8]) = v;
  }
}

template <bool DROP, bool DY32>
__device__ __forceinline__ void glob_chain_bwd(bf16_t* As, float* Stg, const GlobLayerBwd& L, const float* dy32, long lddy32, int row0, int rowEnd,
                                               unsigned long long sbase, TileRing<2>& R, const bf16_t* next) {
  constexpr int RF = 2;
  const int lane = threadIdx.x & 63, wave = threadIdx.x >> 6;
  const DropK d_postln = resolve_drop(L.d_postln, sbase), d_ff1 = resolve_drop(L.d_ff1, sbase), d_ff2 = resolve_drop(L.d_ff2, sbase);
  f32x4_t acc[RF][3];
  glob_ln_bwd<false, DROP, DY32, false>(As, dy32, lddy32, L.r2, L.ln2g, row0, rowEnd, L.dr2, L.dr2m, nullptr, d_ff2, d_ff2, Stg, L.g_ln2g, L.g_ln2b);
  __syncthreads();
  zero_acc<RF>(acc);
  gemm_run<RF, 12, true>(R, As, L.w2_kn + wave * GSZ, L.w1_kn + wave * GSZ, acc, lane);
  epilogue<RF, 8>(acc, Stg, As, row0, nullptr,
      [&](int row, int col) { return PreRes{row < rowEnd ? gld16(L.h1, (unsigned)(row * FZ_D + col) * 2u) : u32x4_t{0u, 0u, 0u, 0u}}; },
      [&](int row, int col, float (&v)[8], const PreRes& pr, int) {
        float a[8];
        unpack8(pr.res, a);
#pragma unroll
        for (int j = 0; j < 8; ++j) v[j] *= gelu_grad_f(a[j]);
        apply_drop<DROP>(d_ff1, (unsigned long long)row * FZ_D + col, v);
        if (row < rowEnd) {
          gst16(L.dh1, (unsigned)(row * FZ_D + col) * 2u, pack8(v));
        } else {
#pragma unroll
          for (int j = 0; j < 8; ++j) v[j] = 0.f;
        }
      }, true);
  zero_acc<RF>(acc);
  gemm_run<RF, 12, true>(R, As, L.w1_kn + wave * GSZ, L.wo_kn + wave * GSZ, acc, lane);
  epilogue<RF, 8>(acc, Stg, As, row0, nullptr,
      [&](int row, int col) { return PreRes{row < rowEnd ? gld16(L.dr2, (unsigned)(row * FZ_D + col) * 2u) : u32x4_t{0u, 0u, 0u, 0u}}; },
      [&](int, int, float (&v)[8], const PreRes& pr, int) {
        float r[8];
        unpack8(pr.res, r);
#pragma unroll
        for (int j = 0; j < 8; ++j) v[j] += r[j];
      }, true);
  glob_ln_bwd<DROP, false, false, false>(As, nullptr, 0, L.r1, L.ln1g, row0, rowEnd, L.dr1, nullptr, nullptr, d_postln, d_postln, Stg, L.g_ln1g,
                                         L.g_ln1b);
  __syncthreads();
  zero_acc<RF>(acc);
  gemm_run<RF, 12, true>(R, As, L.wo_kn + wave * GSZ, next, acc, lane);
  epilogue<RF, 8>(acc, Stg, As, row0, nullptr, [&](int, int) { return PreNone{}; }, [&](int, int, float (&)[8], const PreNone&, int) {}, true);
  __syncthreads();
}

template <bool DROP>
__global__ __launch_bounds__(512) void glob_bwd_kernel(GlobBwd p) {
  constexpr int RF = 2, BT = 32;
  __shared__ __attribute__((aligned(16))) unsigned char smem[4 * BT * APITCH * 2 + BT * SPITCH * 4];
  bf16_t* As = reinterpret_cast<bf16_t*>(smem);
  bf16_t* Qs = As + BT * APITCH;
  bf16_t* Ks = Qs + BT * APITCH;
  bf16_t* Vs = Ks + BT * APITCH;
  float* Stg = reinterpret_cast<float*>(smem + 4 * BT * APITCH * 2);
  float* Sc = Stg;
  float* Dl = Stg + 256 * 32;
  float* Ls = Dl + 256;
  static_assert(BT * SPITCH >= 256 * 32 + 512, "staging buffer holds the attention scratch");
  const int tid = threadIdx.x, lane = tid & 63, wave = tid >> 6;
  const int Cm = p.Cmax, G = 32 / Cm;
  int tile;
  {
    const bf16_t* ws[8] = {p.ctx.wqkv_kn, p.ctx.wo_kn, p.ctx.w1_kn, p.ctx.w2_kn, p.self.wqkv_kn, p.self.wo_kn, p.self.w1_kn, p.self.w2_kn};
    tile = glob_tile_or_help(p, ws);
    if (tile < 0) return;
  }
  const int v0 = tile * G, nv = (p.B - v0) < G ? (p.B - v0) : G;
  const int row0 = v0 * Cm, nrows = nv * Cm, rowEnd = row0 + nrows;
  unsigned long long sbase = 0;
  if constexpr (DROP) { if (p.self.d_ff1.seed_ptr) sbase = *p.self.d_ff1.seed_ptr; }
  const float scale = 0.14433756729740643f;
  f32x4_t acc[RF][3];
  const int pair = tid >> 1, half = tid & 1, pr_ = pair >> 3, ph = pair & 7, coff = ph * 48 + half * 24;
  int tsn = 0;
  auto stamp = [&]() { if (p.tstamps && tile == 0 && threadIdx.x == 0) p.tstamps[tsn] = __builtin_amdgcn_s_memtime(); ++tsn; };
  stamp();

  TileRing<RF> R;
  const bf16_t* cqkv = p.ctx.wqkv_kn + (long)wave * (36L * 3 * 512);
  const bf16_t* sqkv = p.self.wqkv_kn + (long)wave * (36L * 3 * 512);
  gemm_issue(R, p.ctx.w2_kn + wave * GSZ, lane);
  glob_chain_bwd<DROP, true>(As, Stg, p.ctx, p.dpooled + FZ_D, 2 * FZ_D, v0, v0 + nv, sbase, R, cqkv);
  stamp();
  load_rows32(Qs, p.ctx.q, p.ctx.ldq, 0, v0, nv);
  load_rows32(Ks, p.ctx.k, p.ctx.ldk, 0, row0, nrows);
  load_rows32(Vs, p.ctx.v, p.ctx.ldv, 0, row0, nrows);
  __syncthreads();
  {
    const DropK dk_ = resolve_drop(p.ctx.d_attn, sbase);
    const bool on = pr_ < nv;
    const int r = on ? pr_ : 0, kr0 = r * Cm;
    const int nvalid = on ? (int)p.lens[v0 + r] : 0;
    const float lse = on ? p.ctx.lse[(long)(v0 + r) * 8 + ph] : 0.f;
    float q[24], dO[24];
#pragma unroll
    for (int c = 0; c < 3; ++c) {
      unpack8(*reinterpret_cast<const u32x4_t*>(&Qs[r * APITCH + coff + c * 8]), &q[c * 8]);
      unpack8(*reinterpret_cast<const u32x4_t*>(&As[r * APITCH + coff + c * 8]), &dO[c * 8]);
    }
    const unsigned mrow = (unsigned)((v0 + r) * 8 + ph);
    float delta = 0.f;
    for (int j = 0; j < Cm; ++j) {
      float kk[24], vv[24];
#pragma unroll
      for (int c = 0; c < 3; ++c) {
        unpack8(*reinterpret_cast<const u32x4_t*>(&Ks[(kr0 + j) * APITCH + coff + c * 8]), &kk[c * 8]);
        unpack8(*reinterpret_cast<const u32x4_t*>(&Vs[(kr0 + j) * APITCH + coff + c * 8]), &vv[c * 8]);
      }
      float sv = 0.f, dp = 0.f;
#pragma unroll
      for (int c = 0; c < 24; ++c) { sv += q[c] * kk[c]; dp += dO[c] * vv[c]; }
      sv += __shfl_xor(sv, 1, 64); dp += __shfl_xor(dp, 1, 64);
      sv = j < nvalid ? sv * scale : kMaskFill;
      const float pj = __expf(sv - lse);
      float dr = 1.f;
      if constexpr (DROP) dr = attn_drop_f(dk_.key, mrow, j, (unsigned)(Cm + 1) >> 1, dk_.thr, dk_.inv_keep);
      delta += pj * dr * dp;
      if (half == 0) { Sc[pair * 32 + j] = pj; }
    }
    asm volatile("s_waitcnt lgkmcnt(0)" ::: "memory");
    float dq[24];
#pragma unroll
    for (int c = 0; c < 24; ++c) dq[c] = 0.f;
    for (int j = 0; j < Cm; ++j) {
      float kk[24], vv[24];
#pragma unroll
      for (int c = 0; c < 3; ++c) {
        unpack8(*reinterpret_cast<const u32x4_t*>(&Ks[(kr0 + j) * APITCH + coff + c * 8]), &kk[c * 8]);
        unpack8(*reinterpret_cast<const u32x4_t*>(&Vs[(kr0 + j) * APITCH + coff + c * 8]), &vv[c * 8]);
      }
      float dp = 0.f;
#pragma unroll
      for (int c = 0; c < 24; ++c) dp += dO[c] * vv[c];
      dp += __shfl_xor(dp, 1, 64);
      const float pj = Sc[pair * 32 + j];
      float dr = 1.f;
      if constexpr (DROP) dr = attn_drop_f(dk_.key, mrow, j, (unsigned)(Cm + 1) >> 1, dk_.thr, dk_.inv_keep);
      const float ds = j < nvalid ? pj * (dr * dp - delta) * scale : 0.f;
      const float pd = pj * dr;
#pragma unroll
      for (int c = 0; c < 24; ++c) dq[c] += ds * kk[c];
      if (on) {
#pragma unroll
        for (int c = 0; c < 3; ++c) {
          float t8[8], u8[8];
#pragma unroll
          for (int e = 0; e < 8; ++e) { t8[e] = ds * q[c * 8 + e]; u8[e] = pd * dO[c * 8 + e]; }
          const u32x4_t pk = pack8(t8), pv = pack8(u8);
          *reinterpret_cast<u32x4_t*>(&Ks[(kr0 + j) * APITCH + coff + c * 8]) = pk;
          *reinterpret_cast<u32x4_t*>(&Vs[(kr0 + j) * APITCH + coff + c * 8]) = pv;
          gst16(p.ctx.dk, (unsigned)((row0 + kr0 + j) * (int)p.ctx.lddk + coff + c * 8) * 2u, pk);
          gst16(p.ctx.dv, (unsigned)((row0 + kr0 + j) * (int)p.ctx.lddv + coff + c * 8) * 2u, pv);
        }
      }
    }
    if (on) {
#pragma unroll
      for (int c = 0; c < 3; ++c) {
        const u32x4_t pk = pack8(&dq[c * 8]);
        *reinterpret_cast<u32x4_t*>(&Qs[r * APITCH + coff + c * 8]) = pk;
        gst16(p.ctx.dq, (unsigned)((v0 + r) * (int)p.ctx.lddq + coff + c * 8) * 2u, pk);
      }
    }
  }
  __syncthreads();
  stamp();
  zero_acc<RF>(acc);
  gemm_run<RF, 12, true>(R, Qs, cqkv, cqkv + 12L * 3 * 512, acc, lane);
  epilogue<RF, 8>(acc, Stg, As, v0, nullptr,
      [&](int row, int col) { return PreRes{row < v0 + nv ? gld16(p.ctx.dr1, (unsigned)(row * FZ_D + col) * 2u) : u32x4_t{0u, 0u, 0u, 0u}}; },
      [&](int row, int col, float (&v)[8], const PreRes& pr, int) {
        float r[8];
        unpack8(pr.res, r);
        if (row < v0 + nv) {
          float* o = p.dhidden + (long)row * FZ_D + col;
          *reinterpret_cast<f32x4_t*>(o) = f32x4_t{v[0] + r[0], v[1] + r[1], v[2] + r[2], v[3] + r[3]};
          *reinterpret_cast<f32x4_t*>(o + 4) = f32x4_t{v[4] + r[4], v[5] + r[5], v[6] + r[6], v[7] + r[7]};
        }
      }, false);
  stamp();
  zero_acc<RF>(acc);
  gemm_run<RF, 12, true>(R, Ks, cqkv + 12L * 3 * 512, cqkv + 24L * 3 * 512, acc, lane);
  gemm_run<RF, 12, true>(R, Vs, cqkv + 24L * 3 * 512, p.self.w2_kn + wave * GSZ, acc, lane);
  epilogue<RF, 8>(acc, Stg, As, row0, nullptr, [&](int, int) { return PreNone{}; },
      [&](int row, int col, float (&v)[8], const PreNone&, int) {
        if (row < rowEnd) {
          const int vid = row / Cm;
          const float inv = 1.0f / (float)p.lens[vid];
          float g[8];
          load8f(p.dpooled + (long)vid * (2 * FZ_D) + col, g);
#pragma unroll
          for (int j = 0; j < 8; ++j) v[j] += g[j] * inv;
        } else {
#pragma unroll
          for (int j = 0; j < 8; ++j) v[j] = 0.f;
        }
      }, true);
  __syncthreads();
  stamp();

  glob_chain_bwd<DROP, false>(As, Stg, p.self, nullptr, 0, row0, rowEnd, sbase, R, sqkv);
  stamp();
  load_rows32(Qs, p.self.q, p.self.ldq, 0, row0, nrows);
  load_rows32(Ks, p.self.k, p.self.ldk, 0, row0, nrows);
  load_rows32(Vs, p.self.v, p.self.ldv, 0, row0, nrows);
  __syncthreads();
  {
    const DropK dk_ = resolve_drop(p.self.d_attn, sbase);
    const bool on = pr_ < nrows;
    const int r = on ? pr_ : 0, sl = r / Cm, kr0 = sl * Cm, cpos = r - kr0;
    const int nvalid = on ? (int)p.lens[v0 + sl] : 0;
    {
      const float lse = on ? p.self.lse[(long)(row0 + r) * 8 + ph] : 0.f;
      float q[24], dO[24];
#pragma unroll
      for (int c = 0; c < 3; ++c) {
        unpack8(*reinterpret_cast<const u32x4_t*>(&Qs[r * APITCH + coff + c * 8]), &q[c * 8]);
        unpack8(*reinterpret_cast<const u32x4_t*>(&As[r * APITCH + coff + c * 8]), &dO[c * 8]);
      }
      const unsigned mrow = (unsigned)(((v0 + sl) * 8 + ph) * Cm + cpos);
      float delta = 0.f;
      for (int j = 0; j < Cm; ++j) {
        float kk[24], vv[24];
#pragma unroll
        for (int c = 0; c < 3; ++c) {
          unpack8(*reinterpret_cast<const u32x4_t*>(&Ks[(kr0 + j) * APITCH + coff + c * 8]), &kk[c * 8]);
          unpack8(*reinterpret_cast<const u32x4_t*>(&Vs[(kr0 + j) * APITCH + coff + c * 8]), &vv[c * 8]);
        }
        float sv = 0.f, dp = 0.f;
#pragma unroll
        for (int c = 0; c < 24; ++c) { sv += q[c] * kk[c]; dp += dO[c] * vv[c]; }
        sv += __shfl_xor(sv, 1, 64); dp += __shfl_xor(dp, 1, 64);
        sv = j < nvalid ? sv * scale : kMaskFill;
        const float pj = __expf(sv - lse);
        float dr = 1.f;
        if constexpr (DROP) dr = attn_drop_f(dk_.key, mrow, j, (unsigned)(Cm + 1) >> 1, dk_.thr, dk_.inv_keep);
        delta += pj * dr * dp;
        if (half == 0) Sc[pair * 32 + j] = pj;
      }
      if (half == 0) { Dl[pair] = delta; Ls[pair] = lse; }
      asm volatile("s_waitcnt lgkmcnt(0)" ::: "memory");
      float dq[24];
#pragma unroll
      for (int c = 0; c < 24; ++c) dq[c] = 0.f;
      for (int j = 0; j < Cm; ++j) {
        float kk[24], vv[24];
#pragma unroll
        for (int c = 0; c < 3; ++c) {
          unpack8(*reinterpret_cast<const u32x4_t*>(&Ks[(kr0 + j) * APITCH + coff + c * 8]), &kk[c * 8]);
          unpack8(*reinterpret_cast<const u32x4_t*>(&Vs[(kr0 + j) * APITCH + coff + c * 8]), &vv[c * 8]);
        }
        float dp = 0.f;
#pragma unroll
        for (int c = 0; c < 24; ++c) dp += dO[c] * vv[c];
        dp += __shfl_xor(dp, 1, 64);
        const float pj = Sc[pair * 32 + j];
        float dr = 1.f;
        if constexpr (DROP) dr = attn_drop_f(dk_.key, mrow, j, (unsigned)(Cm + 1) >> 1, dk_.thr, dk_.inv_keep);
        const float ds = j < nvalid ? pj * (dr * dp - delta) * scale : 0.f;
#pragma unroll
        for (int c = 0; c < 24; ++c) dq[c] += ds * kk[c];
      }
      if (on) {
#pragma unroll
        for (int c = 0; c < 3; ++c) gst16(p.self.dq, (unsigned)((row0 + r) * (int)p.self.lddq + coff + c * 8) * 2u, pack8(&dq[c * 8]));
      }
    }
    lds_barrier();
    {
      float kk[24], vv[24], dkr[24], dvr[24];
#pragma unroll
      for (int c = 0; c < 3; ++c) {
        unpack8(*reinterpret_cast<const u32x4_t*>(&Ks[r * APITCH + coff + c * 8]), &kk[c * 8]);
        unpack8(*reinterpret_cast<const u32x4_t*>(&Vs[r * APITCH + coff + c * 8]), &vv[c * 8]);
      }
#pragma unroll
      for (int c = 0; c < 24; ++c) { dkr[c] = 0.f; dvr[c] = 0.f; }
      const bool kvalid = on && cpos < nvalid;
      for (int i = 0; i < Cm; ++i) {
        float q[24], dO[24];
#pragma unroll
        for (int c = 0; c < 3; ++c) {
          unpack8(*reinterpret_cast<const u32x4_t*>(&Qs[(kr0 + i) * APITCH + coff + c * 8]), &q[c * 8]);
          unpack8(*reinterpret_cast<const u32x4_t*>(&As[(kr0 + i) * APITCH + coff + c * 8]), &dO[c * 8]);
        }
        float sv = 0.f, dp = 0.f;
#pragma unroll
        for (int c = 0; c < 24; ++c) { sv += q[c] * kk[c]; dp += dO[c] * vv[c]; }
        sv += __shfl_xor(sv, 1, 64); dp += __shfl_xor(dp, 1, 64);
        const int qp = (kr0 + i) * 8 + ph;
        const float pj = kvalid ? __expf(sv * scale - Ls[qp]) : 0.f;
        float dr = 1.f;
        if constexpr (DROP) dr = attn_drop_f(dk_.key, (unsigned)(((v0 + sl) * 8 + ph) * Cm + i), cpos, (unsigned)(Cm + 1) >> 1, dk_.thr, dk_.inv_keep);
        const float ds = pj * (dr * dp - Dl[qp]) * scale;
        const float pd = pj * dr;
#pragma unroll
        for (int c = 0; c < 24; ++c) { dkr[c] += ds * q[c]; dvr[c] += pd * dO[c]; }
      }
      if (on) {
#pragma unroll
        for (int c = 0; c < 3; ++c) {
          gst16(p.self.dk, (unsigned)((row0 + r) * (int)p.self.lddk + coff + c * 8) * 2u, pack8(&dkr[c * 8]));
          gst16(p.self.dv, (unsigned)((row0 + r) * (int)p.self.lddv + coff + c * 8) * 2u, pack8(&dvr[c * 8]));
        }
      }
    }
  }
  __syncthreads();
  stamp();
  zero_acc<RF>(acc);
  load_rows32(Qs, p.self.dq, p.self.lddq, 0, row0, nrows);
  load_rows32(Ks, p.self.dk, p.self.lddk, 0, row0, nrows);
  load_rows32(Vs, p.self.dv, p.self.lddv, 0, row0, nrows);
  __syncthreads();
#pragma unroll 1
  for (int c = 0; c < 3; ++c) {
    const bf16_t* Ts = c == 0 ? Qs : (c == 1 ? Ks : Vs);
    gemm_run<RF, 12, true>(R, Ts, sqkv + (long)c * 12 * 3 * 512, sqkv + (long)(c < 2 ? c + 1 : c) * 12 * 3 * 512, acc, lane);
  }
  epilogue<RF, 8>(acc, Stg, As, row0, nullptr,
      [&](int row, int col) { return PreRes{row < rowEnd ? gld16(p.self.dr1, (unsigned)(row * FZ_D + col) * 2u) : u32x4_t{0u, 0u, 0u, 0u}}; },
      [&](int, int, float (&v)[8], const PreRes& pr, int) {
        float r[8];
        unpack8(pr.res, r);
#pragma unroll
        for (int j = 0; j < 8; ++j) v[j] += r[j];
      }, true);
  stamp();
  {
    const DropK none;
    glob_ln_bwd<false, false, false, true>(As, nullptr, 0, p.x, p.n_gain, row0, rowEnd, nullptr, nullptr, p.dx, none, none, Stg, p.g_n_gain, p.g_n_bias);
  }
  stamp();
}

constexpr int XPITCH = 80;

template <int RF>
__global__ __launch_bounds__(512) void infc_qkv_fwd_kernel(InfcQkvFwd p) {
  constexpr int BT = 16 * RF, RR = 32, CPT = RF / 4;
  static_assert(RF == 8 || RF == 4, "tile height");
  __shared__ __attribute__((aligned(16))) unsigned char smem[BT * APITCH * 2 + RR * SPITCH * 4 + 4 * FZ_D * 4];
  bf16_t* As = reinterpret_cast<bf16_t*>(smem);
  float* Stg = reinterpret_cast<float*>(smem + BT * APITCH * 2);
  float* Bsm = reinterpret_cast<float*>(smem + BT * APITCH * 2 + RR * SPITCH * 4);
  const int tid = threadIdx.x, lane = tid & 63, wave = tid >> 6;
  const int tile_idx = fz_tile_index((p.T + BT - 1) / BT);
  if (tile_idx < 0) return;
  const int row0 = tile_idx * BT, Din = p.Din;
  int tsn = 48;
  auto stamp = [&]() {
    unsigned long long* ts = p.tstamps;
    asm volatile("" : "+s"(ts));
    if (ts && blockIdx.x == 0 && threadIdx.x == 0) ts[tsn] = __builtin_amdgcn_s_memtime();
    ++tsn;
  };
  stamp();
  if (tid < FZ_D / 4) reinterpret_cast<f32x4_t*>(Bsm)[tid] = reinterpret_cast<const f32x4_t*>(p.bin)[tid];
  else if (tid < 4 * FZ_D / 4) reinterpret_cast<f32x4_t*>(Bsm)[tid] = reinterpret_cast<const f32x4_t*>(p.bqkv)[tid - FZ_D / 4];
  bf16_t* Xs = As;
  const int sr = tid >> 3, sc = (tid & 7) * 8;
  const unsigned g0 = (unsigned)((row0 + sr) * Din + sc) * 2u, g1 = (unsigned)((row0 + sr + 64) * Din + sc) * 2u;
  u32x4_t xr[2][2];
  auto gload = [&](int set, int k0) {
    xr[set][0] = gld16(p.xhat, g0 + (unsigned)k0 * 2u);
    if constexpr (CPT == 2) xr[set][1] = gld16(p.xhat, g1 + (unsigned)k0 * 2u);
  };
  auto sstore = [&](int set, int buf) {
    *reinterpret_cast<u32x4_t*>(&Xs[buf * BT * XPITCH + sr * XPITCH + sc]) = xr[set][0];
    if constexpr (CPT == 2) *reinterpret_cast<u32x4_t*>(&Xs[buf * BT * XPITCH + (sr + 64) * XPITCH + sc]) = xr[set][1];
  };
  f32x4_t acc[RF][3];
  zero_acc<RF>(acc);
  const int nkb = Din / 32, nslab = Din / 64;
  const bf16x8_t* wp = reinterpret_cast<const bf16x8_t*>(p.win + (long)wave * nkb * 3 * 512) + lane;
  bf16x8_t w[6][3];
  auto wload = [&](int s, auto slot3) {
    constexpr int S3 = decltype(slot3)::value;
#pragma unroll
    for (int kk = 0; kk < 2; ++kk)
#pragma unroll
      for (int b = 0; b < 3; ++b) w[2 * S3 + kk][b] = wp[((s * 2 + kk) * 3 + b) * 64];
  };
  wload(0, std::integral_constant<int, 0>{});
  if (nslab > 1) wload(1, std::integral_constant<int, 1>{});
  gload(0, 0);
  sstore(0, 0);
  if (nslab > 1) gload(1, 64);
  if (nslab > 2) gload(0, 128);
  __syncthreads();
  const bf16_t* arow = Xs + (lane & 15) * XPITCH + (lane >> 4) * 8;
  auto slab = [&](int s, auto j6) {
    constexpr int J = decltype(j6)::value, PAR = J & 1, S3 = J % 3;
    if (s + 2 < nslab) wload(s + 2, std::integral_constant<int, (S3 + 2) % 3>{});
    __builtin_amdgcn_sched_barrier(0);
    const bf16_t* ab = arow + PAR * BT * XPITCH;
#pragma unroll
    for (int kk = 0; kk < 2; ++kk)
#pragma unroll
      for (int a = 0; a < RF; ++a) {
        const bf16x8_t xf = *reinterpret_cast<const bf16x8_t*>(ab + a * 16 * XPITCH + kk * 32);
#pragma unroll
        for (int b = 0; b < 3; ++b) acc[a][b] = COOT_MFMA_16x16x32(w[2 * S3 + kk][b], xf, acc[a][b]);
      }
    if (s + 1 < nslab) sstore(1 - PAR, 1 - PAR);
    if (s + 3 < nslab) gload(1 - PAR, (s + 3) * 64);
    lds_barrier();
  };
#pragma unroll 1
  for (int s = 0; s < nslab; s += 6) {
    slab(s, std::integral_constant<int, 0>{});
    if (s + 1 < nslab) slab(s + 1, std::integral_constant<int, 1>{});
    if (s + 2 < nslab) slab(s + 2, std::integral_constant<int, 2>{});
    if (s + 3 < nslab) slab(s + 3, std::integral_constant<int, 3>{});
    if (s + 4 < nslab) slab(s + 4, std::integral_constant<int, 4>{});
    if (s + 5 < nslab) slab(s + 5, std::integral_constant<int, 5>{});
  }
  stamp();
  TileRing<RF> R;
  gemm_issue(R, p.wqkv + wave * GSZ, lane);
  struct PrePe { f32x4_t a, b; };
  epilogue<RF, 8>(acc, Stg, As, row0, Bsm,
      [&](int row, int col) {
        const int pos = p.pos ? (row < p.T ? p.pos[row] : 0) : (row < p.T0 ? row % p.L1 : (row - p.T0) % p.L2);
        const float* pp = p.pe + (long)pos * FZ_D + col;
        return PrePe{*reinterpret_cast<const f32x4_t*>(pp), *reinterpret_cast<const f32x4_t*>(pp + 4)};
      },
      [&](int row, int col, float (&v)[8], const PrePe& pr, int) {
        gst16(p.h0, (unsigned)(row * FZ_D + col) * 2u, pack8(v));
#pragma unroll
        for (int j = 0; j < 8; ++j) v[j] = gelu_f(v[j]);
        v[0] += pr.a[0]; v[1] += pr.a[1]; v[2] += pr.a[2]; v[3] += pr.a[3]; v[4] += pr.b[0]; v[5] += pr.b[1]; v[6] += pr.b[2]; v[7] += pr.b[3];
        gst16(p.z0, (unsigned)(row * FZ_D + col) * 2u, pack8(v));
      }, true);
  stamp();
#pragma unroll 1
  for (int q = 0; q < 3; ++q) {
    zero_acc<RF>(acc);
    gemm_run<RF, 12, true>(R, As, p.wqkv + (q * 8 + wave) * GSZ, p.wqkv + ((q < 2 ? q + 1 : q) * 8 + wave) * GSZ, acc, lane);
    epilogue<RF, 8>(acc, Stg, As, row0, Bsm + (1 + q) * FZ_D, [&](int, int) { return PreNone{}; },
        [&](int row, int col, float (&v)[8], const PreNone&, int) { gst16(p.qkv, (unsigned)(row * (3 * FZ_D) + q * FZ_D + col) * 2u, pack8(v)); },
        false);
    stamp();
  }
}

__global__ __launch_bounds__(512) void qkv_fwd_kernel(QkvFwd p) {
  constexpr int RF = 8, BT = 128, RR = 32;
  __shared__ __attribute__((aligned(16))) unsigned char smem[BT * APITCH * 2 + RR * SPITCH * 4 + 3 * FZ_D * 4];
  bf16_t* As = reinterpret_cast<bf16_t*>(smem);
  float* Stg = reinterpret_cast<float*>(smem + BT * APITCH * 2);
  float* Bsm = reinterpret_cast<float*>(smem + BT * APITCH * 2 + RR * SPITCH * 4);
  const int lane = threadIdx.x & 63, wave = threadIdx.x >> 6;
  const int row0 = blockIdx.x * BT;
  if (threadIdx.x < 3 * FZ_D / 4) reinterpret_cast<f32x4_t*>(Bsm)[threadIdx.x] = reinterpret_cast<const f32x4_t*>(p.bias)[threadIdx.x];
  TileRing<RF> R;
  gemm_issue(R, p.wqkv + wave * GSZ, lane);
  load_tile<RF>(As, p.z, FZ_D, 0, row0);
  __syncthreads();
  f32x4_t acc[RF][3];
#pragma unroll 1
  for (int q = 0; q < 3; ++q) {
    zero_acc<RF>(acc);
    gemm_run<RF, 12, true>(R, As, p.wqkv + (q * 8 + wave) * GSZ, p.wqkv + ((q < 2 ? q + 1 : q) * 8 + wave) * GSZ, acc, lane);
    epilogue<RF, 8>(acc, Stg, As, row0, Bsm + q * FZ_D, [&](int, int) { return PreNone{}; },
        [&](int row, int col, float (&v)[8], const PreNone&, int) { gst16(p.qkv, (unsigned)(row * (3 * FZ_D) + q * FZ_D + col) * 2u, pack8(v)); },
        false);
  }
}

template <int RF, bool GELU>
__global__ __launch_bounds__(512) void qkv_bwd_kernel(QkvBwd p) {
  constexpr int BT = 16 * RF, RR = 32;
  __shared__ __attribute__((aligned(16))) unsigned char smem[BT * APITCH * 2 + RR * SPITCH * 4];
  bf16_t* As = reinterpret_cast<bf16_t*>(smem);
  float* Stg = reinterpret_cast<float*>(smem + BT * APITCH * 2);
  const int lane = threadIdx.x & 63, wave = threadIdx.x >> 6;
  const int row0 = blockIdx.x * BT, T = p.T;
  f32x4_t acc[RF][3];
  zero_acc<RF>(acc);
  const bf16_t* wg = p.wqkv + (long)wave * (36L * 3 * 512);
  TileRing<RF> R;
  gemm_issue(R, wg, lane);
// ... 69 lines not shown
__global__ __launch_bounds__(256) void colsum_scatter_kernel(ScatterArgs a) {
  const ScatterSeg& sg = a.s[blockIdx.y];
  const int c = blockIdx.x * 16 + (threadIdx.x & 15);
  const bool on = c < sg.n && sg.dst;
  const float r = colsum_groups(a.part + sg.off + c, FZ_BWD_NCS, a.ntiles, on);
  if ((threadIdx.x >> 4) == 0 && on) sg.dst[c] += r;
}

}

constexpr int kHalfTilesMax = 256 * 64;
bool half_tiles(int T, int ) { return T <= kHalfTilesMax; }

static int g_fused_attn = 1;
void set_fused_attn(int on) { g_fused_attn = on; }
static int g_fused_attn_launches = 0;
int fused_attn_launches() { return g_fused_attn_launches; }
static int post_attn_tile_rows(int T, bool do_pool) {
  if (!do_pool && T < 1024) return 0;
  return half_tiles(T, 1) ? 64 : 128;
}
bool post_attn_can_fuse_attention(int T, bool do_pool, int N0, int L0, int N1, int L1) {
  if (!g_fused_attn) return false;
  const int BT = post_attn_tile_rows(T, do_pool);
  if (BT == 0) return false;
  const int lmax = BT == 128 ? FZ_ATTN_LMAX(8) : FZ_ATTN_LMAX(4);
  if (N0 <= 0 || L0 <= 0 || L0 % 16 != 0 || L0 > lmax || (long)N0 * L0 + (long)N1 * L1 != (long)T) return false;
  if (N1 > 0 && (L1 <= 0 || L1 % 16 != 0 || L1 > lmax || ((long)N0 * L0) % BT != 0)) return false;
  return true;
}

int launch_post_attn_fwd(const PostAttnFwd& p, hipStream_t st) {
  if (p.attn.on) {
    COOT_REQUIRE(p.attn.qkv && p.attn.lse && p.ctx_w && p.attn.lens0 && (p.attn.N1 == 0 || p.attn.lens1), "post_attn_fwd: fused attention pointers");
    COOT_REQUIRE(post_attn_can_fuse_attention(p.T, p.do_pool != 0, p.attn.N0, p.attn.L0, p.attn.N1, p.attn.L1),
                 "post_attn_fwd: these segments cannot take the attention along (post_attn_can_fuse_attention)");
    COOT_REQUIRE((long)p.T * 3 * FZ_D * 2 < (1l << 32), "post_attn_fwd: qkv beyond the 32-bit byte offsets of the fused attention");
    ++g_fused_attn_launches;
  }
  COOT_REQUIRE((p.ctx || p.attn.on) && p.xres && p.wo && p.w1 && p.w2 && p.bo && p.b1 && p.b2 && p.ln1g && p.ln1b && p.ln2g && p.ln2b && p.r1 && p.z1 &&
               p.h1 && p.a1 && p.r2 && p.z2, "post_attn_fwd: null pointer");
  COOT_REQUIRE(!p.do_pool || (p.pw1 && p.pw2 && p.pb1 && p.pb2 && p.hp && p.ap && p.s), "post_attn_fwd: pooling pointers");
  if (p.T <= 0) return 0;
  const double attn_flops = p.attn.on ? 4.0 * 384.0 * ((double)p.attn.N0 * p.attn.L0 * p.attn.L0 + (double)p.attn.N1 * p.attn.L1 * p.attn.L1) : 0.0;
  void* ts = timing_begin(TIMING_FUSED, 2.0 * p.T * 384.0 * 384.0 * (p.do_pool ? 6.0 : 3.0) + attn_flops, 0, st);
  const bool drop = p.d_postln.thr || p.d_ff1.thr || p.d_ff2.thr || p.d_pool1.thr || p.d_pool2.thr;
  if (drop)
    COOT_REQUIRE(p.d_postln.thr && p.d_ff1.thr && p.d_ff2.thr && (!p.do_pool || (p.d_pool1.thr && p.d_pool2.thr)), "post_attn_fwd: dropout on some sites only");
  const bool small = !p.do_pool && p.T < 1024;
  if (small) {
    if (drop) hipLaunchKernelGGL((post_attn_fwd_kernel<2, true>), dim3((p.T + 31) / 32), dim3(NTHR), 0, st, p);
    else hipLaunchKernelGGL((post_attn_fwd_kernel<2, false>), dim3((p.T + 31) / 32), dim3(NTHR), 0, st, p);
  } else if (half_tiles(p.T, 1)) {
    if (drop) hipLaunchKernelGGL((post_attn_fwd_kernel<4, true>), dim3(fz_grid((p.T + 63) / 64)), dim3(NTHR), 0, st, p);
    else hipLaunchKernelGGL((post_attn_fwd_kernel<4, false>), dim3(fz_grid((p.T + 63) / 64)), dim3(NTHR), 0, st, p);
  } else if (drop) {
    hipLaunchKernelGGL((post_attn_fwd_kernel<8, true>), dim3(fz_grid((p.T + 127) / 128)), dim3(NTHR), 0, st, p);
  } else {
    hipLaunchKernelGGL((post_attn_fwd_kernel<8, false>), dim3(fz_grid((p.T + 127) / 128)), dim3(NTHR), 0, st, p);
  }
  timing_end(ts, st);
  COOT_CHECK_LAUNCH("post_attn_fwd");
  return 0;
}

}

namespace coot {
int launch_pre_attn_bwd(const PreAttnBwd& p_in, hipStream_t st) {
  PreAttnBwd p = p_in;
  COOT_REQUIRE(p.h1 && p.r2 && p.r1 && p.w2 && p.w1 && p.wo && p.ln2g && p.ln1g && p.dr2 && p.dh1 && p.dr1 && p.dctx && p.part,
               "pre_attn_bwd: null pointer");
  COOT_REQUIRE(p.do_pool ? (p.ds && p.dzp && p.hp && p.pw2 && p.pw1 && p.dhp) : (p.dz2 != nullptr), "pre_attn_bwd: input gradient pointers");
  if (p.T <= 0) return 0;
  const bool half = half_tiles(p.T, 2);
  const int tiles = half ? (p.T + 63) / 64 : (p.T + 127) / 128;
  float* top = colsum_defer_room() >= 8 ? partials_workspace_top((size_t)tiles * FZ_BWD_NCS) : nullptr;
  if (top) p.part = top;
  const bool drop = p.d_ff2.thr || p.d_ff1.thr || p.d_postln.thr || p.d_pool1.thr;
  void* ts = timing_begin(TIMING_FUSED, 2.0 * p.T * 384.0 * 384.0 * (p.do_pool ? 6.0 : 3.0), 0, st);
  if (drop) {
    COOT_REQUIRE(p.d_ff2.thr && p.d_ff1.thr && p.d_postln.thr && (!p.do_pool || p.d_pool1.thr) && p.dr2m, "pre_attn_bwd: dropout on some sites only");
    if (half) hipLaunchKernelGGL((pre_attn_bwd_kernel<4, true>), dim3(tiles), dim3(NTHR), 0, st, p);
    else hipLaunchKernelGGL((pre_attn_bwd_kernel<8, true>), dim3(tiles), dim3(NTHR), 0, st, p);
  } else {
    if (half) hipLaunchKernelGGL((pre_attn_bwd_kernel<4, false>), dim3(tiles), dim3(NTHR), 0, st, p);
    else hipLaunchKernelGGL((pre_attn_bwd_kernel<8, false>), dim3(tiles), dim3(NTHR), 0, st, p);
  }
  timing_end(ts, st);
  COOT_CHECK_LAUNCH("pre_attn_bwd");
  ScatterArgs a; a.ntiles = tiles; a.part = p.part; a.nseg = 8;
  a.s[0] = ScatterSeg{p.do_pool ? p.g_pb1 : nullptr, 0, 2 * FZ_D};
  a.s[1] = ScatterSeg{p.g_ln2g, 2 * FZ_D, FZ_D}; a.s[2] = ScatterSeg{p.g_ln2b, 3 * FZ_D, FZ_D}; a.s[3] = ScatterSeg{p.g_b2, 4 * FZ_D, FZ_D};
  a.s[4] = ScatterSeg{p.g_b1, 5 * FZ_D, FZ_D};
  a.s[5] = ScatterSeg{p.g_ln1g, 6 * FZ_D, FZ_D}; a.s[6] = ScatterSeg{p.g_ln1b, 7 * FZ_D, FZ_D}; a.s[7] = ScatterSeg{p.g_bo, 8 * FZ_D, FZ_D};
  if (top) {
    for (int i = 0; i < 8; ++i)
      if (a.s[i].dst) colsum_defer_add(a.s[i].dst, p.part + a.s[i].off, FZ_BWD_NCS, tiles, a.s[i].n, 0);
    return 0;
  }
  hipLaunchKernelGGL(colsum_scatter_kernel, dim3(48, 8), dim3(256), 0, st, a);
  COOT_CHECK_LAUNCH("colsum_scatter");
  return 0;
}
}

namespace coot {
int launch_qkv_fwd(const QkvFwd& p, hipStream_t st) {
  COOT_REQUIRE(p.z && p.wqkv && p.bias && p.qkv, "qkv_fwd: null pointer");
  if (p.T <= 0) return 0;
  void* ts = timing_begin(TIMING_FUSED, 2.0 * p.T * 384.0 * 1152.0, 0, st);
  hipLaunchKernelGGL(qkv_fwd_kernel, dim3((p.T + 127) / 128), dim3(NTHR), 0, st, p);
  timing_end(ts, st);
  COOT_CHECK_LAUNCH("qkv_fwd");
  return 0;
}
int launch_qkv_bwd(const QkvBwd& p_in, hipStream_t st) {
  QkvBwd p = p_in;
  COOT_REQUIRE(p.dqkv && p.wqkv && p.res && p.dz, "qkv_bwd: null pointer");
  COOT_REQUIRE(!p.aux || (p.colsum && p.part), "qkv_bwd: GELU' needs the column-sum buffers");
  if (p.T <= 0) return 0;
  const bool half = half_tiles(p.T, 3);
  const int tiles = half ? (p.T + 63) / 64 : (p.T + 127) / 128;
  bool deferred = false;
  if (p.aux) {
    float* top = partials_workspace_top((size_t)tiles * FZ_D);
    if (top && colsum_defer_add(p.colsum, top, FZ_D, tiles, FZ_D, p.colsum_overwrite)) { p.part = top; deferred = true; }
  }
  void* ts = timing_begin(TIMING_FUSED, 2.0 * p.T * 384.0 * 1152.0, 0, st);
  if (half) {
    if (p.aux) hipLaunchKernelGGL((qkv_bwd_kernel<4, true>), dim3(tiles), dim3(NTHR), 0, st, p);
    else hipLaunchKernelGGL((qkv_bwd_kernel<4, false>), dim3(tiles), dim3(NTHR), 0, st, p);
  } else {
    if (p.aux) hipLaunchKernelGGL((qkv_bwd_kernel<8, true>), dim3(tiles), dim3(NTHR), 0, st, p);
    else hipLaunchKernelGGL((qkv_bwd_kernel<8, false>), dim3(tiles), dim3(NTHR), 0, st, p);
  }
  timing_end(ts, st);
  COOT_CHECK_LAUNCH("qkv_bwd");
  if (p.aux) {
    if (deferred) return 0;
    hipLaunchKernelGGL(colsum_tiles_kernel, dim3((FZ_D + 15) / 16), dim3(256), 0, st, (const float*)p.part, tiles, FZ_D, p.colsum, p.colsum_overwrite);
    COOT_CHECK_LAUNCH("colsum_tiles");
  }
  return 0;
}
}

namespace coot {
static thread_local int g_glob_xcd_first = 0, g_glob_xcd_count = 8;
void glob_xcd_set(int first, int count) {
  if (first < 0 || count < 1 || first + count > 8) { first = 0; count = 8; }
  g_glob_xcd_first = first; g_glob_xcd_count = count;
}
template <typename P>
static int glob_grid(P& p, int tiles) {
  p.tiles = tiles;
  p.xcd_first = g_glob_xcd_first; p.xcd_count = g_glob_xcd_count;
  if (tiles > 8 * p.xcd_count) { p.xcd_first = 0; p.xcd_count = 8; }
  p.tiles_per_xcd = (tiles + p.xcd_count - 1) / p.xcd_count;
  p.warm_per_xcd = tiles >= 128 ? 0 : (tiles > 64 ? 8 : 16) * (8 / p.xcd_count);
  return 8 * (p.tiles_per_xcd + p.warm_per_xcd);
}
bool glob_fwd_supported(int Cmax) { return Cmax >= 1 && Cmax <= 32; }
int launch_glob_fwd(const GlobFwd& p_in, hipStream_t st) {
  COOT_REQUIRE(p_in.x && p_in.lens && p_in.hidden && p_in.pe && p_in.n_gain && p_in.n_bias && p_in.z0 && p_in.cq_in && p_in.pooled, "glob_fwd: null pointer");
  COOT_REQUIRE(glob_fwd_supported(p_in.Cmax), "glob_fwd: %d items per sequence (max 32)", p_in.Cmax);
  if (p_in.B <= 0) return 0;
  GlobFwd p = p_in;
  const int G = 32 / p.Cmax, tiles = (p.B + G - 1) / G;
  const int grid = glob_grid(p, tiles);
  const bool drop = p.self.d_attn.thr || p.self.d_postln.thr || p.self.d_ff1.thr || p.self.d_ff2.thr;
  if (drop) COOT_REQUIRE(p.self.d_attn.thr && p.self.d_postln.thr && p.self.d_ff1.thr && p.self.d_ff2.thr && p.ctx.d_attn.thr && p.ctx.d_postln.thr &&
                         p.ctx.d_ff1.thr && p.ctx.d_ff2.thr, "glob_fwd: dropout on some sites only");
  const double T = (double)p.B * p.Cmax;
  void* ts = timing_begin(TIMING_GLOB, 2.0 * 384.0 * 384.0 * (8.0 * T + 4.0 * p.B), 0, st);
  if (drop) hipLaunchKernelGGL(glob_fwd_kernel<true>, dim3(grid), dim3(NTHR), 0, st, p);
  else hipLaunchKernelGGL(glob_fwd_kernel<false>, dim3(grid), dim3(NTHR), 0, st, p);
  timing_end(ts, st);
  COOT_CHECK_LAUNCH("glob_fwd");
  return 0;
}
int launch_glob_bwd(const GlobBwd& p_in, hipStream_t st) {
  COOT_REQUIRE(p_in.x && p_in.lens && p_in.n_gain && p_in.dpooled && p_in.dhidden, "glob_bwd: null pointer");
  COOT_REQUIRE(glob_fwd_supported(p_in.Cmax), "glob_bwd: %d items per sequence (max 32)", p_in.Cmax);
  if (p_in.B <= 0) return 0;
  GlobBwd p = p_in;
  const int G = 32 / p.Cmax, tiles = (p.B + G - 1) / G;
  const int grid = glob_grid(p, tiles);
  const bool drop = p.self.d_attn.thr || p.self.d_postln.thr || p.self.d_ff1.thr || p.self.d_ff2.thr;
  if (drop) COOT_REQUIRE(p.self.d_attn.thr && p.self.d_postln.thr && p.self.d_ff1.thr && p.self.d_ff2.thr && p.ctx.d_attn.thr && p.ctx.d_postln.thr &&
                         p.ctx.d_ff1.thr && p.ctx.d_ff2.thr && p.self.dr2m && p.ctx.dr2m, "glob_bwd: dropout on some sites only");
  const double T = (double)p.B * p.Cmax;
  void* ts = timing_begin(TIMING_GLOB, 2.0 * 384.0 * 384.0 * (6.0 * T + 6.0 * T + 4.0 * p.B), 0, st);
  if (drop) hipLaunchKernelGGL(glob_bwd_kernel<true>, dim3(grid), dim3(NTHR), 0, st, p);
  else hipLaunchKernelGGL(glob_bwd_kernel<false>, dim3(grid), dim3(NTHR), 0, st, p);
  timing_end(ts, st);
  COOT_CHECK_LAUNCH("glob_bwd");
  return 0;
}
int launch_infc_qkv_fwd(const InfcQkvFwd& p, hipStream_t st) {
  COOT_REQUIRE(p.xhat && p.win && p.bin && p.pe && p.wqkv && p.bqkv && p.h0 && p.z0 && p.qkv, "infc_qkv_fwd: null pointer");
  COOT_REQUIRE(p.Din % 64 == 0 && p.Din >= 128 && p.L1 > 0 && p.L2 > 0, "infc_qkv_fwd: Din = %d must be a multiple of 64, >= 128", p.Din);
  if (p.T <= 0) return 0;
  void* ts = timing_begin(TIMING_FUSED, 2.0 * p.T * 384.0 * (p.Din + 1152.0), 0, st);
  if (half_tiles(p.T, 0)) hipLaunchKernelGGL(infc_qkv_fwd_kernel<4>, dim3(fz_grid((p.T + 63) / 64)), dim3(NTHR), 0, st, p);
  else hipLaunchKernelGGL(infc_qkv_fwd_kernel<8>, dim3(fz_grid((p.T + 127) / 128)), dim3(NTHR), 0, st, p);
  timing_end(ts, st);
  COOT_CHECK_LAUNCH("infc_qkv_fwd");
  return 0;
}
}

namespace coot {
COOT_DET_DEFINE_SETTER(fused)
}
```

Baseline: 223,600 clip-pairs/s.

## Issue glob kernel epilogue and parameter loads ahead of GEMMs, keep dq/dk/dv in LDS

Adds an EARLY variant of the fused global-context forward and backward kernels, on by default. Epilogue bias and residual loads are issued before each GEMM, and the layer parameter vectors and sequence lengths are staged into shared memory. The aim is to hide global-memory latency behind MFMA work. In backward, dq/dk/dv are written directly to LDS instead of being reloaded from global memory, which removes a round trip and a full barrier. In exchange the kernels use more LDS and registers, which may lower occupancy, and the code adds a second, more complex path.

```diff
diff --git a/coot-videotext_amd/csrc/api.hip b/coot-videotext_amd/csrc/api.hip
--- a/coot-videotext_amd/csrc/api.hip
+++ b/coot-videotext_amd/csrc/api.hip
@@ -630,6 +630,7 @@
   if (!strcmp(name, "det_overflows")) { *value = det_overflow_count(); return 0; }
   if (!strcmp(name, "det_overflow_check")) { *value = det_overflow_guard(); return 0; }
   if (!strcmp(name, "attn_bwd_loop")) { *value = get_attn_bwd_loop(); return 0; }
+  if (!strcmp(name, "glob_early_loads")) { *value = get_glob_early_loads(); return 0; }
   if (!strcmp(name, "attn_bwd_share")) { *value = get_attn_bwd_share(); return 0; }
   if (!strcmp(name, "attn_bwd_grid")) { *value = get_attn_bwd_grid(); return 0; }
   if (!strcmp(name, "rt_topk_splits")) { *value = get_rt_topk_splits(); return 0; }
@@ -660,6 +661,7 @@
   if (!strcmp(name, "text_ahead")) { coot_step_text_ahead(value); return 0; }
   if (!strcmp(name, "det_overflow_check")) return det_set_overflow_guard(value);
   if (!strcmp(name, "glob_flush_aux")) { g_glob_flush_aux = value; return 0; }
+  if (!strcmp(name, "glob_early_loads")) { set_glob_early_loads(value); return 0; }
   if (!strcmp(name, "pool_handover")) { g_pool_handover_on = value; return 0; }
   if (!strcmp(name, "cl_col_split")) { set_cl_col_split(value); return 0; }
   if (!strcmp(name, "cl_small")) { set_cl_small(value); return 0; }
diff --git a/coot-videotext_amd/csrc/fused.h b/coot-videotext_amd/csrc/fused.h
--- a/coot-videotext_amd/csrc/fused.h
+++ b/coot-videotext_amd/csrc/fused.h
@@ -138,6 +138,8 @@
 };
 int launch_glob_bwd(const GlobBwd& p, hipStream_t st);
 void glob_xcd_set(int first, int count);
+void set_glob_early_loads(int on);
+int get_glob_early_loads();
 
 constexpr int FZ_BWD_NCS = 9 * FZ_D;
 bool half_tiles(int T, int kernel);
diff --git a/coot-videotext_amd/csrc/fused.hip b/coot-videotext_amd/csrc/fused.hip
--- a/coot-videotext_amd/csrc/fused.hip
+++ b/coot-videotext_amd/csrc/fused.hip
@@ -153,9 +153,11 @@
   for (int i = 0; i < IT; ++i) load8f(bias + ((threadIdx.x + NTHR * i) % NCH) * 8, bs[i]);
 }
 
-template <int RF, int NCG, typename PreF, typename Fn>
+struct EpiLate {};
+template <typename P, bool BIAS> struct EpiEarly { float bs[BIAS ? 3 : 1][8]; P pv[3]; };
+template <int RF, int NCG, typename PreF, typename Fn, typename Early = EpiLate>
 __device__ __forceinline__ void epilogue(f32x4_t (&acc)[RF * NCG / 8][3], float* Stg, bf16_t* As, int row0, const float* bias_lds,
-                                         PreF pre, Fn fn, bool to_lds, unsigned long long* prof = nullptr) {
+                                         PreF pre, Fn fn, bool to_lds, unsigned long long* prof = nullptr, const Early& early = Early{}) {
 #ifdef FZ_PROFILE_EPI
   unsigned long long pt[7] = {0, 0, 0, 0, 0, 0, 0}, pacc[6] = {0, 0, 0, 0, 0, 0};
   const bool profiling = prof && blockIdx.x == 0 && threadIdx.x == 0;
@@ -177,15 +179,28 @@
     if constexpr (NCG == 8) { rl[i] = r_; col[i] = ch * 8; }
     else { rl[i] = r_ + (ch >= 24 ? 32 : 0); col[i] = (ch >= 24 ? ch - 24 : ch) * 8; }
   }
+  constexpr bool EARLY = !std::is_same<Early, EpiLate>::value;
+  constexpr bool EARLY_BIAS = std::is_same<Early, EpiEarly<decltype(pre(0, 0)), true>>::value;
+  static_assert(!EARLY || (ROUNDS == 1 && NCG == 8), "the caller's chunks are those of the only round");
   float bs[IT][8];
   if (bias_lds) {
 #pragma unroll
-    for (int i = 0; i < IT; ++i) load8f(bias_lds + col[i], bs[i]);
+    for (int i = 0; i < IT; ++i) {
+      if constexpr (EARLY_BIAS) {
+#pragma unroll
+        for (int j = 0; j < 8; ++j) bs[i][j] = early.bs[i][j];
+      } else {
+        load8f(bias_lds + col[i], bs[i]);
+      }
+    }
   }
   using P = decltype(pre(0, 0));
   P pv[IT];
 #pragma unroll
-  for (int i = 0; i < IT; ++i) pv[i] = pre(row0 + rl[i], col[i]);
+  for (int i = 0; i < IT; ++i) {
+    if constexpr (EARLY) pv[i] = early.pv[i];
+    else pv[i] = pre(row0 + rl[i], col[i]);
+  }
   float* sw = &Stg[(lane & 15) * SPITCH + cg * 48 + (lane >> 4) * 4];
 #pragma unroll 1
   for (int r = 0; r < ROUNDS; ++r) {
@@ -275,6 +290,21 @@
 #undef FZ_PT
 }
 
+template <bool BIAS, typename PreF>
+__device__ __forceinline__ auto epi_early(int row0, const float* bias, PreF pre) {
+  EpiEarly<decltype(pre(0, 0)), BIAS> e;
+  int tid = threadIdx.x;
+  asm volatile("" : "+v"(tid));
+#pragma unroll
+  for (int i = 0; i < 3; ++i) {
+    const int c = tid + NTHR * i, rl = c / 48, col = (c - rl * 48) * 8;
+    if constexpr (BIAS) load8f(bias + col, e.bs[i]);
+    e.pv[i] = pre(row0 + rl, col);
+  }
+  __builtin_amdgcn_sched_barrier(0);
+  return e;
+}
+
 __device__ __forceinline__ float row16_sum(float v) {
   auto dpp = [](float x, auto ctrl) {
     return __builtin_bit_cast(float, __builtin_amdgcn_update_dpp(0, __builtin_bit_cast(int, x), decltype(ctrl)::value, 0xF, 0xF, false));
@@ -319,9 +349,9 @@
   }
 }
 
-template <int RF, bool DROP, bool OUT32, bool MASK = false>
+template <int RF, bool DROP, bool OUT32, bool MASK = false, bool PARK = false>
 __device__ __forceinline__ void ln_tile(bf16_t* As, const float* gain, const float* bias, int row0, int T, bf16_t* out, float* out32,
-                                        long ld32, const DropK& drop) {
+                                        long ld32, const DropK& drop, bf16_t* park = nullptr) {
 #ifdef FZ_NO_LN
   return;
 #endif
@@ -364,6 +394,7 @@
       }
       const u32x4_t o = pack8(y);
       *reinterpret_cast<u32x4_t*>(ar + m * 128) = o;
+      if constexpr (PARK) *reinterpret_cast<u32x4_t*>(park + rl * APITCH + j16 * 8 + m * 128) = o;
       if (!MASK || row < T) gst16(out, (unsigned)(row * FZ_D + m * 128 + j16 * 8) * 2u, o);
       if constexpr (OUT32) {
         if (row < T) {
@@ -968,12 +999,12 @@
 template <bool SELF, bool DROP>
 __device__ __forceinline__ void tile_attn(const bf16_t* Qs, const bf16_t* Ks, const bf16_t* Vs, bf16_t* Os, float* Sc, int nq, int Lk,
                                           int seq0, const long long* lens, float scale, const DropK& dk, bf16_t* o_glob, float* lse_glob,
-                                          int grow0) {
+                                          int grow0, const int* lens_lds = nullptr) {
   const int tid = threadIdx.x, pair = tid >> 1, half = tid & 1, r = pair >> 3, h = pair & 7;
   const bool on = r < nq;
   const int sl = on ? (SELF ? r / Lk : r) : 0;
   const int kr0 = sl * Lk;
-  const int nvalid = on ? (int)lens[seq0 + sl] : 0;
+  const int nvalid = on ? (lens_lds ? lens_lds[sl] : (int)lens[seq0 + sl]) : 0;
   const int coff = h * 48 + half * 24;
   float q[24];
 #pragma unroll
@@ -1096,16 +1127,90 @@
   __syncthreads();
 }
 
-template <bool DROP>
+struct ChainVecs { float v[7]; };
+__device__ __forceinline__ ChainVecs chain_vecs_issue(const GlobLayerFwd& L) {
+  ChainVecs c;
+  if (threadIdx.x < FZ_D) {
+    const float* const src[7] = {L.bo, L.ln1g, L.ln1b, L.b1, L.b2, L.ln2g, L.ln2b};
+#pragma unroll
+    for (int k = 0; k < 7; ++k) c.v[k] = src[k][threadIdx.x];
+  }
+  __builtin_amdgcn_sched_barrier(0);
+  return c;
+}
+__device__ __forceinline__ void chain_vecs_commit(float* Ps, const ChainVecs& c) {
+  if (threadIdx.x < FZ_D) {
+#pragma unroll
+    for (int k = 0; k < 7; ++k) Ps[k * FZ_D + threadIdx.x] = c.v[k];
+  }
+}
+template <bool DROP, bool OUT32>
+__device__ __forceinline__ void glob_chain_fwd_early(bf16_t* As, float* Stg, const GlobLayerFwd& L, const bf16_t* xres, int row0, int rowEnd,
+                                                     float* z2_f32, long ldz2_f32, unsigned long long sbase, TileRing<2>& R, const bf16_t* next,
+                                                     bf16_t* Zs, const float* Ps) {
+  constexpr int RF = 2;
+  const int lane = threadIdx.x & 63, wave = threadIdx.x >> 6;
+  const DropK d_postln = resolve_drop(L.d_postln, sbase), d_ff1 = resolve_drop(L.d_ff1, sbase), d_ff2 = resolve_drop(L.d_ff2, sbase);
+  f32x4_t acc[RF][3];
+  zero_acc<RF>(acc);
+  {
+    auto pre_x = [&](int row, int col) { return PreRes{row < rowEnd ? gld16(xres, (unsigned)(row * FZ_D + col) * 2u) : u32x4_t{0u, 0u, 0u, 0u}}; };
+    const auto e = epi_early<false>(row0, nullptr, pre_x);
+    gemm_run<RF, 12, true>(R, As, L.wo + wave * GSZ, L.w1 + wave * GSZ, acc, lane);
+    epilogue<RF, 8>(acc, Stg, As, row0, Ps, pre_x,
+        [&](int row, int col, float (&v)[8], const PreRes& pr, int) {
+          float r[8];
+          unpack8(pr.res, r);
+#pragma unroll
+          for (int j = 0; j < 8; ++j) v[j] += r[j];
+          if (row < rowEnd) gst16(L.r1, (unsigned)(row * FZ_D + col) * 2u, pack8(v));
+        }, true, nullptr, e);
+  }
+  ln_tile<RF, DROP, false, true, true>(As, Ps + FZ_D, Ps + 2 * FZ_D, row0, rowEnd, L.z1, nullptr, 0, d_postln, Zs);
+  lds_barrier();
+  zero_acc<RF>(acc);
+  gemm_run<RF, 12, true>(R, As, L.w1 + wave * GSZ, L.w2 + wave * GSZ, acc, lane);
+  epilogue<RF, 8>(acc, Stg, As, row0, Ps + 3 * FZ_D, [&](int, int) { return PreNone{}; },
+      [&](int row, int col, float (&v)[8], const PreNone&, int) {
+        apply_drop<DROP>(d_ff1, (unsigned long long)row * FZ_D + col, v);
+        if (row < rowEnd) gst16(L.h1, (unsigned)(row * FZ_D + col) * 2u, pack8(v));
+#pragma unroll
+        for (int j = 0; j < 8; ++j) v[j] = gelu_f(v[j]);
+        if (row < rowEnd) gst16(L.a1, (unsigned)(row * FZ_D + col) * 2u, pack8(v));
+      }, true);
+  zero_acc<RF>(acc);
+  gemm_run<RF, 12, true>(R, As, L.w2 + wave * GSZ, next, acc, lane);
+  epilogue<RF, 8>(acc, Stg, As, row0, Ps + 4 * FZ_D,
+      [&](int row, int col) {
+        return PreRes{row < rowEnd ? *reinterpret_cast<const u32x4_t*>(&Zs[(row - row0) * APITCH + col]) : u32x4_t{0u, 0u, 0u, 0u}};
+      },
+      [&](int row, int col, float (&v)[8], const PreRes& pr, int) {
+        float r[8];
+        unpack8(pr.res, r);
+        apply_drop<DROP>(d_ff2, (unsigned long long)row * FZ_D + col, v);
+#pragma unroll
+        for (int j = 0; j < 8; ++j) v[j] += r[j];
+        if (row < rowEnd) gst16(L.r2, (unsigned)(row * FZ_D + col) * 2u, pack8(v));
+      }, true);
+  {
+    const DropK none;
+    ln_tile<RF, false, OUT32, true>(As, Ps + 5 * FZ_D, Ps + 6 * FZ_D, row0, rowEnd, L.z2, z2_f32, ldz2_f32, none);
+  }
+  __syncthreads();
+}
+
+template <bool DROP, bool EARLY>
 __global__ __launch_bounds__(512) void glob_fwd_kernel(GlobFwd p) {
   constexpr int RF = 2, BT = 32;
-  __shared__ __attribute__((aligned(16))) unsigned char smem[4 * BT * APITCH * 2 + BT * SPITCH * 4];
+  __shared__ __attribute__((aligned(16))) unsigned char smem[4 * BT * APITCH * 2 + BT * SPITCH * 4 + (EARLY ? 32 * 4 + 7 * FZ_D * 4 : 0)];
   static_assert(BT * SPITCH * 4 >= 256 * 32 * 4, "the staging buffer holds the attention scores [256 pairs][32 keys]");
   bf16_t* As = reinterpret_cast<bf16_t*>(smem);
   bf16_t* Qs = As + BT * APITCH;
   bf16_t* Ks = Qs + BT * APITCH;
   bf16_t* Vs = Ks + BT * APITCH;
   float* Stg = reinterpret_cast<float*>(smem + 4 * BT * APITCH * 2);
+  int* lens_s = reinterpret_cast<int*>(smem + 4 * BT * APITCH * 2 + BT * SPITCH * 4);
+  float* Ps = reinterpret_cast<float*>(lens_s + 32);
   const int tid = threadIdx.x, lane = tid & 63, wave = tid >> 6;
   const int Cm = p.Cmax, G = 32 / Cm;
   int tile;
@@ -1125,6 +1230,11 @@
   stamp();
   TileRing<RF> R;
   gemm_issue(R, p.self.wqkv + wave * GSZ, lane);
+  ChainVecs cv;
+  if constexpr (EARLY) {
+    if (tid < 32) lens_s[tid] = tid < nv ? (int)p.lens[v0 + tid] : 0;
+    cv = chain_vecs_issue(p.self);
+  }
 
   {
     const int j16 = lane & 15, g = lane >> 4, rl = wave * 4 + g, row = row0 + rl;
@@ -1161,85 +1271,157 @@
       if (on) gst16(p.z0, (unsigned)(row * FZ_D + col) * 2u, o);
     }
   }
+  if constexpr (EARLY) chain_vecs_commit(Ps, cv);
   __syncthreads();
   stamp();
 
 #pragma unroll 1
   for (int q = 0; q < 3; ++q) {
     zero_acc<RF>(acc);
+    if constexpr (EARLY) {
+      auto pre_none = [&](int, int) { return PreNone{}; };
+      const auto e = epi_early<true>(row0, p.self.bqkv + q * FZ_D, pre_none);
+      gemm_run<RF, 12, true>(R, As, p.self.wqkv + (q * 8 + wave) * GSZ, q < 2 ? p.self.wqkv + ((q + 1) * 8 + wave) * GSZ : p.self.wo + wave * GSZ, acc, lane);
+      bf16_t* dst = q == 0 ? Qs : (q == 1 ? Ks : Vs);
+      epilogue<RF, 8>(acc, Stg, dst, row0, p.self.bqkv, pre_none,
+          [&](int row, int col, float (&v)[8], const PreNone&, int) {
+            if (row < rowEnd) gst16(p.self.q, (unsigned)(row * (3 * FZ_D) + q * FZ_D + col) * 2u, pack8(v));
+          }, true, nullptr, e);
+    } else {
     gemm_run<RF, 12, true>(R, As, p.self.wqkv + (q * 8 + wave) * GSZ, q < 2 ? p.self.wqkv + ((q + 1) * 8 + wave) * GSZ : p.self.wo + wave * GSZ, acc, lane);
     bf16_t* dst = q == 0 ? Qs : (q == 1 ? Ks : Vs);
     epilogue<RF, 8>(acc, Stg, dst, row0, p.self.bqkv + q * FZ_D, [&](int, int) { return PreNone{}; },
         [&](int row, int col, float (&v)[8], const PreNone&, int) {
           if (row < rowEnd) gst16(p.self.q, (unsigned)(row * (3 * FZ_D) + q * FZ_D + col) * 2u, pack8(v));
         }, true);
+    }
     stamp();
   }
   __syncthreads();
   {
     const DropK dk = resolve_drop(p.self.d_attn, sbase);
-    tile_attn<true, DROP>(Qs, Ks, Vs, As, Stg, nrows, Cm, v0, p.lens, scale, dk, p.self.ctx, p.self.lse, row0);
+    tile_attn<true, DROP>(Qs, Ks, Vs, As, Stg, nrows, Cm, v0, p.lens, scale, dk, p.self.ctx, p.self.lse, row0, EARLY ? lens_s : nullptr);
   }
   __syncthreads();
   stamp();
   {
     const bf16_t* nx = p.ctx.wqkv + (8 + wave) * GSZ;
+    if constexpr (EARLY) {
+      if (p.per_token) glob_chain_fwd_early<DROP, true>(As, Stg, p.self, p.z0, row0, rowEnd, p.per_token, FZ_D, sbase, R, nx, Qs, Ps);
+      else glob_chain_fwd_early<DROP, false>(As, Stg, p.self, p.z0, row0, rowEnd, nullptr, 0, sbase, R, nx, Qs, Ps);
+    } else {
     if (p.per_token) glob_chain_fwd<DROP, true>(As, Stg, p.self, p.z0, row0, rowEnd, p.per_token, FZ_D, sbase, R, nx);
     else glob_chain_fwd<DROP, false>(As, Stg, p.self, p.z0, row0, rowEnd, nullptr, 0, sbase, R, nx);
-  }
-  stamp();
-
-  if (tid < FZ_D) {
-    for (int gv = 0; gv < nv; ++gv) {
-      float a = 0.f;
-      for (int j = 0; j < Cm; ++j) a += bf2f(As[(gv * Cm + j) * APITCH + tid]);
-      p.pooled[(long)(v0 + gv) * (2 * FZ_D) + tid] = a / (float)p.lens[v0 + gv];
-    }
-  }
-
+    }
+  }
+  stamp();
+
+  if constexpr (EARLY) {
+    float hq[3][8];
+#pragma unroll
+    for (int i = 0; i < 3; ++i) {
+      const int c = tid + NTHR * i, rl = c / 48, ch = c - rl * 48;
+      if (rl < nv) load8f(p.hidden + (long)(v0 + rl) * FZ_D + ch * 8, hq[i]);
+    }
+    cv = chain_vecs_issue(p.ctx);
+    if (tid < FZ_D) {
+      for (int gv = 0; gv < nv; ++gv) {
+        float a = 0.f;
+        for (int j = 0; j < Cm; ++j) a += bf2f(As[(gv * Cm + j) * APITCH + tid]);
+        p.pooled[(long)(v0 + gv) * (2 * FZ_D) + tid] = a / (float)lens_s[gv];
+      }
+    }
+    auto pre_none = [&](int, int) { return PreNone{}; };
 #pragma unroll 1
-  for (int q = 1; q < 3; ++q) {
+    for (int q = 1; q < 3; ++q) {
+      zero_acc<RF>(acc);
+      bf16_t* dst = q == 1 ? Ks : Vs;
+      bf16_t* gdst = q == 1 ? p.ctx.k : p.ctx.v;
+      const int ldkv = (int)(q == 1 ? p.ctx.ldk : p.ctx.ldv);
+      const auto e = epi_early<true>(row0, p.ctx.bqkv + q * FZ_D, pre_none);
+      gemm_run<RF, 12, true>(R, As, p.ctx.wqkv + (q * 8 + wave) * GSZ, q == 1 ? p.ctx.wqkv + (16 + wave) * GSZ : p.ctx.wqkv + wave * GSZ, acc, lane);
+      if (q == 1) {
+#pragma unroll
+        for (int i = 0; i < 3; ++i) {
+          const int c = tid + NTHR * i, rl = c / 48, ch = c - rl * 48;
+          u32x4_t o = {0u, 0u, 0u, 0u};
+          if (rl < nv) {
+            o = pack8(hq[i]);
+            gst16(p.cq_in, (unsigned)((v0 + rl) * FZ_D + ch * 8) * 2u, o);
+          }
+          *reinterpret_cast<u32x4_t*>(&Qs[rl * APITCH + ch * 8]) = o;
+        }
+        chain_vecs_commit(Ps, cv);
+      }
+      epilogue<RF, 8>(acc, Stg, dst, row0, p.ctx.bqkv, pre_none,
+          [&](int row, int col, float (&v)[8], const PreNone&, int) {
+            if (row < rowEnd) gst16(gdst, (unsigned)(row * ldkv + col) * 2u, pack8(v));
+          }, true, nullptr, e);
+    }
+    stamp();
     zero_acc<RF>(acc);
-    gemm_run<RF, 12, true>(R, As, p.ctx.wqkv + (q * 8 + wave) * GSZ, q == 1 ? p.ctx.wqkv + (16 + wave) * GSZ : p.ctx.wqkv + wave * GSZ, acc, lane);
-    bf16_t* dst = q == 1 ? Ks : Vs;
-    bf16_t* gdst = q == 1 ? p.ctx.k : p.ctx.v;
-    const int ldkv = (int)(q == 1 ? p.ctx.ldk : p.ctx.ldv);
-    epilogue<RF, 8>(acc, Stg, dst, row0, p.ctx.bqkv + q * FZ_D, [&](int, int) { return PreNone{}; },
+    const auto e = epi_early<true>(v0, p.ctx.bqkv, pre_none);
+    gemm_run<RF, 12, true>(R, Qs, p.ctx.wqkv + wave * GSZ, p.ctx.wo + wave * GSZ, acc, lane);
+    epilogue<RF, 8>(acc, Stg, Qs, v0, p.ctx.bqkv, pre_none,
         [&](int row, int col, float (&v)[8], const PreNone&, int) {
-          if (row < rowEnd) gst16(gdst, (unsigned)(row * ldkv + col) * 2u, pack8(v));
+          if (row < v0 + nv) gst16(p.ctx.q, (unsigned)(row * (int)p.ctx.ldq + col) * 2u, pack8(v));
+        }, true, nullptr, e);
+    __syncthreads();
+    stamp();
+  } else {
+    if (tid < FZ_D) {
+      for (int gv = 0; gv < nv; ++gv) {
+        float a = 0.f;
+        for (int j = 0; j < Cm; ++j) a += bf2f(As[(gv * Cm + j) * APITCH + tid]);
+        p.pooled[(long)(v0 + gv) * (2 * FZ_D) + tid] = a / (float)p.lens[v0 + gv];
+      }
+    }
+
+  #pragma unroll 1
+    for (int q = 1; q < 3; ++q) {
+      zero_acc<RF>(acc);
+      gemm_run<RF, 12, true>(R, As, p.ctx.wqkv + (q * 8 + wave) * GSZ, q == 1 ? p.ctx.wqkv + (16 + wave) * GSZ : p.ctx.wqkv + wave * GSZ, acc, lane);
+      bf16_t* dst = q == 1 ? Ks : Vs;
+      bf16_t* gdst = q == 1 ? p.ctx.k : p.ctx.v;
+      const int ldkv = (int)(q == 1 ? p.ctx.ldk : p.ctx.ldv);
+      epilogue<RF, 8>(acc, Stg, dst, row0, p.ctx.bqkv + q * FZ_D, [&](int, int) { return PreNone{}; },
+          [&](int row, int col, float (&v)[8], const PreNone&, int) {
+            if (row < rowEnd) gst16(gdst, (unsigned)(row * ldkv + col) * 2u, pack8(v));
+          }, true);
+    }
+    __syncthreads();
+    stamp();
+    {
+      for (int c = tid; c < BT * 48; c += 512) {
+        const int rl = c / 48, ch = c - rl * 48;
+        u32x4_t o = {0u, 0u, 0u, 0u};
+        if (rl < nv) {
+          float h[8];
+          load8f(p.hidden + (long)(v0 + rl) * FZ_D + ch * 8, h);
+          o = pack8(h);
+          gst16(p.cq_in, (unsigned)((v0 + rl) * FZ_D + ch * 8) * 2u, o);
+        }
+        *reinterpret_cast<u32x4_t*>(&As[rl * APITCH + ch * 8]) = o;
+      }
+    }
+    __syncthreads();
+    zero_acc<RF>(acc);
+    gemm_run<RF, 12, true>(R, As, p.ctx.wqkv + wave * GSZ, p.ctx.wo + wave * GSZ, acc, lane);
+    epilogue<RF, 8>(acc, Stg, Qs, v0, p.ctx.bqkv, [&](int, int) { return PreNone{}; },
+        [&](int row, int col, float (&v)[8], const PreNone&, int) {
+          if (row < v0 + nv) gst16(p.ctx.q, (unsigned)(row * (int)p.ctx.ldq + col) * 2u, pack8(v));
         }, true);
-  }
-  __syncthreads();
-  stamp();
-  {
-    for (int c = tid; c < BT * 48; c += 512) {
-      const int rl = c / 48, ch = c - rl * 48;
-      u32x4_t o = {0u, 0u, 0u, 0u};
-      if (rl < nv) {
-        float h[8];
-        load8f(p.hidden + (long)(v0 + rl) * FZ_D + ch * 8, h);
-        o = pack8(h);
-        gst16(p.cq_in, (unsigned)((v0 + rl) * FZ_D + ch * 8) * 2u, o);
-      }
-      *reinterpret_cast<u32x4_t*>(&As[rl * APITCH + ch * 8]) = o;
-    }
-  }
-  __syncthreads();
-  zero_acc<RF>(acc);
-  gemm_run<RF, 12, true>(R, As, p.ctx.wqkv + wave * GSZ, p.ctx.wo + wave * GSZ, acc, lane);
-  epilogue<RF, 8>(acc, Stg, Qs, v0, p.ctx.bqkv, [&](int, int) { return PreNone{}; },
-      [&](int row, int col, float (&v)[8], const PreNone&, int) {
-        if (row < v0 + nv) gst16(p.ctx.q, (unsigned)(row * (int)p.ctx.ldq + col) * 2u, pack8(v));
-      }, true);
-  __syncthreads();
-  stamp();
+    __syncthreads();
+    stamp();
+  }
   {
     const DropK dk = resolve_drop(p.ctx.d_attn, sbase);
-    tile_attn<false, DROP>(Qs, Ks, Vs, As, Stg, nv, Cm, v0, p.lens, scale, dk, p.ctx.ctx, p.ctx.lse, v0);
+    tile_attn<false, DROP>(Qs, Ks, Vs, As, Stg, nv, Cm, v0, p.lens, scale, dk, p.ctx.ctx, p.ctx.lse, v0, EARLY ? lens_s : nullptr);
   }
   __syncthreads();
   stamp();
-  glob_chain_fwd<DROP, true>(As, Stg, p.ctx, p.cq_in, v0, v0 + nv, p.pooled + FZ_D, 2 * FZ_D, sbase, R, p.ctx.w2 + wave * GSZ );
+  if constexpr (EARLY) glob_chain_fwd_early<DROP, true>(As, Stg, p.ctx, p.cq_in, v0, v0 + nv, p.pooled + FZ_D, 2 * FZ_D, sbase, R, p.ctx.w2 + wave * GSZ, Qs, Ps);
+  else glob_chain_fwd<DROP, true>(As, Stg, p.ctx, p.cq_in, v0, v0 + nv, p.pooled + FZ_D, 2 * FZ_D, sbase, R, p.ctx.w2 + wave * GSZ );
   stamp();
 }
 
@@ -1269,10 +1451,34 @@
   lds_barrier();
 }
 
-template <bool DROPY, bool MASKX, bool DY32, bool X32>
+template <bool DY32, bool X32>
+struct LnBwdIn { float gn[3][8]; typename std::conditional<X32, float, unsigned>::type x[3][X32 ? 8 : 4]; float dy[DY32 ? 3 : 1][8]; };
+template <bool DY32, bool X32>
+__device__ __forceinline__ LnBwdIn<DY32, X32> glob_ln_bwd_load(const float* dy32, long lddy32, const void* xsrc, const float* gain, int row0, int rowEnd) {
+  const int lane = threadIdx.x & 63, wave = threadIdx.x >> 6, j16 = lane & 15, g = lane >> 4;
+  const int rl = wave * 4 + g, row = row0 + rl;
+  LnBwdIn<DY32, X32> in;
+#pragma unroll
+  for (int m = 0; m < 3; ++m) {
+    const int col = m * 128 + j16 * 8;
+    load8f(gain + col, in.gn[m]);
+    if (row < rowEnd) {
+      if constexpr (X32) {
+        load8f(reinterpret_cast<const float*>(xsrc) + (long)row * FZ_D + col, in.x[m]);
+      } else {
+        const u32x4_t u = gld16(xsrc, (unsigned)(row * FZ_D + col) * 2u);
+        in.x[m][0] = u[0]; in.x[m][1] = u[1]; in.x[m][2] = u[2]; in.x[m][3] = u[3];
+      }
+      if constexpr (DY32) load8f(dy32 + (long)row * lddy32 + col, in.dy[m]);
+    }
+  }
+  __builtin_amdgcn_sched_barrier(0);
+  return in;
+}
+template <bool DROPY, bool MASKX, bool DY32, bool X32, bool PRE = false>
 __device__ __forceinline__ void glob_ln_bwd(bf16_t* As, const float* dy32, long lddy32, const void* xsrc, const float* gain, int row0, int rowEnd,
                                             bf16_t* out_dx, bf16_t* out_dxm, float* out32, const DropK& dy_drop, const DropK& dx_drop, float* red,
-                                            float* g_gain, float* g_bias) {
+                                            float* g_gain, float* g_bias, const LnBwdIn<DY32, X32>* pre = nullptr) {
   const int lane = threadIdx.x & 63, wave = threadIdx.x >> 6, j16 = lane & 15, g = lane >> 4;
   const int rl = wave * 4 + g, row = row0 + rl;
   const bool on = row < rowEnd;
@@ -1281,13 +1487,28 @@
 #pragma unroll
   for (int m = 0; m < 3; ++m) {
     const int col = m * 128 + j16 * 8;
-    load8f(gain + col, gn[m]);
+    if constexpr (PRE) {
+#pragma unroll
+      for (int e = 0; e < 8; ++e) gn[m][e] = pre->gn[m][e];
+    } else {
+      load8f(gain + col, gn[m]);
+    }
 #pragma unroll
     for (int e = 0; e < 8; ++e) { x[m][e] = 0.f; dy[m][e] = 0.f; }
     if (on) {
-      if constexpr (X32) load8f(reinterpret_cast<const float*>(xsrc) + (long)row * FZ_D + col, x[m]);
+      if constexpr (PRE) {
+        if constexpr (X32) {
+#pragma unroll
+          for (int e = 0; e < 8; ++e) x[m][e] = pre->x[m][e];
+        } else {
+          unpack8(u32x4_t{pre->x[m][0], pre->x[m][1], pre->x[m][2], pre->x[m][3]}, x[m]);
+        }
+      } else if constexpr (X32) load8f(reinterpret_cast<const float*>(xsrc) + (long)row * FZ_D + col, x[m]);
       else unpack8(gld16(xsrc, (unsigned)(row * FZ_D + col) * 2u), x[m]);
-      if constexpr (DY32) load8f(dy32 + (long)row * lddy32 + col, dy[m]);
+      if constexpr (DY32 && PRE) {
+#pragma unroll
+        for (int e = 0; e < 8; ++e) dy[m][e] = pre->dy[m][e];
+      } else if constexpr (DY32) load8f(dy32 + (long)row * lddy32 + col, dy[m]);
       else unpack8(*reinterpret_cast<const u32x4_t*>(&As[rl * APITCH + col]), dy[m]);
       if constexpr (DROPY) {
         float sc[8];
@@ -1361,44 +1582,81 @@
   }
 }
 
-template <bool DROP, bool DY32>
+struct Rows32 { u32x4_t v[3]; };
+__device__ __forceinline__ Rows32 rows32_issue(const bf16_t* src, long ld, int grow0, int nvalid) {
+  Rows32 t;
+#pragma unroll
+  for (int i = 0; i < 3; ++i) {
+    const int c = threadIdx.x + NTHR * i, rl = c / 48, ch = c - rl * 48;
+    t.v[i] = u32x4_t{0u, 0u, 0u, 0u};
+    if (rl < nvalid) t.v[i] = gld16(src, (unsigned)((grow0 + rl) * (int)ld + ch * 8) * 2u);
+  }
+  return t;
+}
+__device__ __forceinline__ void rows32_commit(bf16_t* Ts, const Rows32& t) {
+#pragma unroll
+  for (int i = 0; i < 3; ++i) {
+    const int c = threadIdx.x + NTHR * i, rl = c / 48, ch = c - rl * 48;
+    *reinterpret_cast<u32x4_t*>(&Ts[rl * APITCH + ch * 8]) = t.v[i];
+  }
+}
+struct QkvRows { bf16_t* Qs; int gq, nq, gkv, nkv; };
+
+template <bool DROP, bool DY32, bool EARLY>
 __device__ __forceinline__ void glob_chain_bwd(bf16_t* As, float* Stg, const GlobLayerBwd& L, const float* dy32, long lddy32, int row0, int rowEnd,
-                                               unsigned long long sbase, TileRing<2>& R, const bf16_t* next) {
-  constexpr int RF = 2;
+                                               unsigned long long sbase, TileRing<2>& R, const bf16_t* next,
+                                               const LnBwdIn<DY32, false>* ln2 = nullptr, const QkvRows* qkv = nullptr) {
+  constexpr int RF = 2, BT = 32;
   const int lane = threadIdx.x & 63, wave = threadIdx.x >> 6;
   const DropK d_postln = resolve_drop(L.d_postln, sbase), d_ff1 = resolve_drop(L.d_ff1, sbase), d_ff2 = resolve_drop(L.d_ff2, sbase);
   f32x4_t acc[RF][3];
-  glob_ln_bwd<false, DROP, DY32, false>(As, dy32, lddy32, L.r2, L.ln2g, row0, rowEnd, L.dr2, L.dr2m, nullptr, d_ff2, d_ff2, Stg, L.g_ln2g, L.g_ln2b);
+  glob_ln_bwd<false, DROP, DY32, false, EARLY>(As, dy32, lddy32, L.r2, L.ln2g, row0, rowEnd, L.dr2, L.dr2m, nullptr, d_ff2, d_ff2, Stg, L.g_ln2g, L.g_ln2b, ln2);
   __syncthreads();
+  auto pre_h1 = [&](int row, int col) { return PreRes{row < rowEnd ? gld16(L.h1, (unsigned)(row * FZ_D + col) * 2u) : u32x4_t{0u, 0u, 0u, 0u}}; };
+  auto fn_2 = [&](int row, int col, float (&v)[8], const PreRes& pr, int) {
+    float a[8];
+    unpack8(pr.res, a);
+#pragma unroll
+    for (int j = 0; j < 8; ++j) v[j] *= gelu_grad_f(a[j]);
+    apply_drop<DROP>(d_ff1, (unsigned long long)row * FZ_D + col, v);
+    if (row < rowEnd) {
+      gst16(L.dh1, (unsigned)(row * FZ_D + col) * 2u, pack8(v));
+    } else {
+#pragma unroll
+      for (int j = 0; j < 8; ++j) v[j] = 0.f;
+    }
+  };
+  auto pre_dr2 = [&](int row, int col) { return PreRes{row < rowEnd ? gld16(L.dr2, (unsigned)(row * FZ_D + col) * 2u) : u32x4_t{0u, 0u, 0u, 0u}}; };
+  auto fn_1 = [&](int, int, float (&v)[8], const PreRes& pr, int) {
+    float r[8];
+    unpack8(pr.res, r);
+#pragma unroll
+    for (int j = 0; j < 8; ++j) v[j] += r[j];
+  };
   zero_acc<RF>(acc);
-  gemm_run<RF, 12, true>(R, As, L.w2_kn + wave * GSZ, L.w1_kn + wave * GSZ, acc, lane);
-  epilogue<RF, 8>(acc, Stg, As, row0, nullptr,
-      [&](int row, int col) { return PreRes{row < rowEnd ? gld16(L.h1, (unsigned)(row * FZ_D + col) * 2u) : u32x4_t{0u, 0u, 0u, 0u}}; },
-      [&](int row, int col, float (&v)[8], const PreRes& pr, int) {
-        float a[8];
-        unpack8(pr.res, a);
-#pragma unroll
-        for (int j = 0; j < 8; ++j) v[j] *= gelu_grad_f(a[j]);
-        apply_drop<DROP>(d_ff1, (unsigned long long)row * FZ_D + col, v);
-        if (row < rowEnd) {
-          gst16(L.dh1, (unsigned)(row * FZ_D + col) * 2u, pack8(v));
-        } else {
-#pragma unroll
-          for (int j = 0; j < 8; ++j) v[j] = 0.f;
-        }
-      }, true);
-  zero_acc<RF>(acc);
-  gemm_run<RF, 12, true>(R, As, L.w1_kn + wave * GSZ, L.wo_kn + wave * GSZ, acc, lane);
-  epilogue<RF, 8>(acc, Stg, As, row0, nullptr,
-      [&](int row, int col) { return PreRes{row < rowEnd ? gld16(L.dr2, (unsigned)(row * FZ_D + col) * 2u) : u32x4_t{0u, 0u, 0u, 0u}}; },
-      [&](int, int, float (&v)[8], const PreRes& pr, int) {
-        float r[8];
-        unpack8(pr.res, r);
-#pragma unroll
-        for (int j = 0; j < 8; ++j) v[j] += r[j];
-      }, true);
-  glob_ln_bwd<DROP, false, false, false>(As, nullptr, 0, L.r1, L.ln1g, row0, rowEnd, L.dr1, nullptr, nullptr, d_postln, d_postln, Stg, L.g_ln1g,
-                                         L.g_ln1b);
+  if constexpr (EARLY) {
+    const auto e2 = epi_early<false>(row0, nullptr, pre_h1);
+    const Rows32 tq = rows32_issue(L.q, L.ldq, qkv->gq, qkv->nq), tk = rows32_issue(L.k, L.ldk, qkv->gkv, qkv->nkv), tv = rows32_issue(L.v, L.ldv, qkv->gkv, qkv->nkv);
+    __builtin_amdgcn_sched_barrier(0);
+    gemm_run<RF, 12, true>(R, As, L.w2_kn + wave * GSZ, L.w1_kn + wave * GSZ, acc, lane);
+    rows32_commit(qkv->Qs, tq); rows32_commit(qkv->Qs + BT * APITCH, tk); rows32_commit(qkv->Qs + 2 * BT * APITCH, tv);
+    const auto e1 = epi_early<false>(row0, nullptr, pre_dr2);
+    epilogue<RF, 8>(acc, Stg, As, row0, nullptr, pre_h1, fn_2, true, nullptr, e2);
+    zero_acc<RF>(acc);
+    gemm_run<RF, 12, true>(R, As, L.w1_kn + wave * GSZ, L.wo_kn + wave * GSZ, acc, lane);
+    const LnBwdIn<false, false> ln1 = glob_ln_bwd_load<false, false>(nullptr, 0, L.r1, L.ln1g, row0, rowEnd);
+    epilogue<RF, 8>(acc, Stg, As, row0, nullptr, pre_dr2, fn_1, true, nullptr, e1);
+    glob_ln_bwd<DROP, false, false, false, true>(As, nullptr, 0, L.r1, L.ln1g, row0, rowEnd, L.dr1, nullptr, nullptr, d_postln, d_postln, Stg, L.g_ln1g,
+                                                 L.g_ln1b, &ln1);
+  } else {
+    gemm_run<RF, 12, true>(R, As, L.w2_kn + wave * GSZ, L.w1_kn + wave * GSZ, acc, lane);
+    epilogue<RF, 8>(acc, Stg, As, row0, nullptr, pre_h1, fn_2, true);
+    zero_acc<RF>(acc);
+    gemm_run<RF, 12, true>(R, As, L.w1_kn + wave * GSZ, L.wo_kn + wave * GSZ, acc, lane);
+    epilogue<RF, 8>(acc, Stg, As, row0, nullptr, pre_dr2, fn_1, true);
+    glob_ln_bwd<DROP, false, false, false>(As, nullptr, 0, L.r1, L.ln1g, row0, rowEnd, L.dr1, nullptr, nullptr, d_postln, d_postln, Stg, L.g_ln1g,
+                                           L.g_ln1b);
+  }
   __syncthreads();
   zero_acc<RF>(acc);
   gemm_run<RF, 12, true>(R, As, L.wo_kn + wave * GSZ, next, acc, lane);
@@ -1406,15 +1664,16 @@
   __syncthreads();
 }
 
-template <bool DROP>
+template <bool DROP, bool EARLY>
 __global__ __launch_bounds__(512) void glob_bwd_kernel(GlobBwd p) {
   constexpr int RF = 2, BT = 32;
-  __shared__ __attribute__((aligned(16))) unsigned char smem[4 * BT * APITCH * 2 + BT * SPITCH * 4];
+  __shared__ __attribute__((aligned(16))) unsigned char smem[4 * BT * APITCH * 2 + BT * SPITCH * 4 + (EARLY ? 32 * 4 : 0)];
   bf16_t* As = reinterpret_cast<bf16_t*>(smem);
   bf16_t* Qs = As + BT * APITCH;
   bf16_t* Ks = Qs + BT * APITCH;
   bf16_t* Vs = Ks + BT * APITCH;
   float* Stg = reinterpret_cast<float*>(smem + 4 * BT * APITCH * 2);
+  int* lens_s = reinterpret_cast<int*>(smem + 4 * BT * APITCH * 2 + BT * SPITCH * 4);
   float* Sc = Stg;
   float* Dl = Stg + 256 * 32;
   float* Ls = Dl + 256;
@@ -1442,18 +1701,28 @@
   const bf16_t* cqkv = p.ctx.wqkv_kn + (long)wave * (36L * 3 * 512);
   const bf16_t* sqkv = p.self.wqkv_kn + (long)wave * (36L * 3 * 512);
   gemm_issue(R, p.ctx.w2_kn + wave * GSZ, lane);
-  glob_chain_bwd<DROP, true>(As, Stg, p.ctx, p.dpooled + FZ_D, 2 * FZ_D, v0, v0 + nv, sbase, R, cqkv);
-  stamp();
-  load_rows32(Qs, p.ctx.q, p.ctx.ldq, 0, v0, nv);
-  load_rows32(Ks, p.ctx.k, p.ctx.ldk, 0, row0, nrows);
-  load_rows32(Vs, p.ctx.v, p.ctx.ldv, 0, row0, nrows);
-  __syncthreads();
+  float lse_c = 0.f;
+  if constexpr (EARLY) {
+    if (tid < 32) lens_s[tid] = tid < nv ? (int)p.lens[v0 + tid] : 0;
+    if (pr_ < nv) lse_c = p.ctx.lse[(long)(v0 + pr_) * 8 + ph];
+    const LnBwdIn<true, false> ln2 = glob_ln_bwd_load<true, false>(p.dpooled + FZ_D, 2 * FZ_D, p.ctx.r2, p.ctx.ln2g, v0, v0 + nv);
+    const QkvRows rows = {Qs, v0, nv, row0, nrows};
+    glob_chain_bwd<DROP, true, true>(As, Stg, p.ctx, p.dpooled + FZ_D, 2 * FZ_D, v0, v0 + nv, sbase, R, cqkv, &ln2, &rows);
+    stamp();
+  } else {
+    glob_chain_bwd<DROP, true, false>(As, Stg, p.ctx, p.dpooled + FZ_D, 2 * FZ_D, v0, v0 + nv, sbase, R, cqkv);
+    stamp();
+    load_rows32(Qs, p.ctx.q, p.ctx.ldq, 0, v0, nv);
+    load_rows32(Ks, p.ctx.k, p.ctx.ldk, 0, row0, nrows);
+    load_rows32(Vs, p.ctx.v, p.ctx.ldv, 0, row0, nrows);
+    __syncthreads();
+  }
   {
     const DropK dk_ = resolve_drop(p.ctx.d_attn, sbase);
     const bool on = pr_ < nv;
     const int r = on ? pr_ : 0, kr0 = r * Cm;
-    const int nvalid = on ? (int)p.lens[v0 + r] : 0;
-    const float lse = on ? p.ctx.lse[(long)(v0 + r) * 8 + ph] : 0.f;
+    const int nvalid = on ? (EARLY ? lens_s[r] : (int)p.lens[v0 + r]) : 0;
+    const float lse = EARLY ? lse_c : (on ? p.ctx.lse[(long)(v0 + r) * 8 + ph] : 0.f);
     float q[24], dO[24];
 #pragma unroll
     for (int c = 0; c < 3; ++c) {
@@ -1528,20 +1797,61 @@
   __syncthreads();
   stamp();
   zero_acc<RF>(acc);
-  gemm_run<RF, 12, true>(R, Qs, cqkv, cqkv + 12L * 3 * 512, acc, lane);
-  epilogue<RF, 8>(acc, Stg, As, v0, nullptr,
-      [&](int row, int col) { return PreRes{row < v0 + nv ? gld16(p.ctx.dr1, (unsigned)(row * FZ_D + col) * 2u) : u32x4_t{0u, 0u, 0u, 0u}}; },
-      [&](int row, int col, float (&v)[8], const PreRes& pr, int) {
-        float r[8];
-        unpack8(pr.res, r);
-        if (row < v0 + nv) {
-          float* o = p.dhidden + (long)row * FZ_D + col;
-          *reinterpret_cast<f32x4_t*>(o) = f32x4_t{v[0] + r[0], v[1] + r[1], v[2] + r[2], v[3] + r[3]};
-          *reinterpret_cast<f32x4_t*>(o + 4) = f32x4_t{v[4] + r[4], v[5] + r[5], v[6] + r[6], v[7] + r[7]};
-        }
-      }, false);
+  {
+    auto pre_dr1 = [&](int row, int col) { return PreRes{row < v0 + nv ? gld16(p.ctx.dr1, (unsigned)(row * FZ_D + col) * 2u) : u32x4_t{0u, 0u, 0u, 0u}}; };
+    auto fn = [&](int row, int col, float (&v)[8], const PreRes& pr, int) {
+      float r[8];
+      unpack8(pr.res, r);
+      if (row < v0 + nv) {
+        float* o = p.dhidden + (long)row * FZ_D + col;
+        *reinterpret_cast<f32x4_t*>(o) = f32x4_t{v[0] + r[0], v[1] + r[1], v[2] + r[2], v[3] + r[3]};
+        *reinterpret_cast<f32x4_t*>(o + 4) = f32x4_t{v[4] + r[4], v[5] + r[5], v[6] + r[6], v[7] + r[7]};
+      }
+    };
+    if constexpr (EARLY) {
+      const auto e = epi_early<false>(v0, nullptr, pre_dr1);
+      gemm_run<RF, 12, true>(R, Qs, cqkv, cqkv + 12L * 3 * 512, acc, lane);
+      epilogue<RF, 8>(acc, Stg, As, v0, nullptr, pre_dr1, fn, false, nullptr, e);
+    } else {
+      gemm_run<RF, 12, true>(R, Qs, cqkv, cqkv + 12L * 3 * 512, acc, lane);
+      epilogue<RF, 8>(acc, Stg, As, v0, nullptr, pre_dr1, fn, false);
+    }
+  }
   stamp();
   zero_acc<RF>(acc);
+  float lse_s = 0.f;
+  if constexpr (EARLY) {
+    struct PrePool { float g[8]; float inv; };
+    const auto e = epi_early<false>(row0, nullptr, [&](int row, int col) {
+      PrePool pp;
+      pp.inv = 0.f;
+      if (row < rowEnd) {
+        const int vid = row / Cm;
+        pp.inv = 1.0f / (float)lens_s[vid - v0];
+        load8f(p.dpooled + (long)vid * (2 * FZ_D) + col, pp.g);
+      }
+      return pp;
+    });
+    if (pr_ < nrows) lse_s = p.self.lse[(long)(row0 + pr_) * 8 + ph];
+    gemm_run<RF, 12, true>(R, Ks, cqkv + 12L * 3 * 512, cqkv + 24L * 3 * 512, acc, lane);
+    gemm_run<RF, 12, true>(R, Vs, cqkv + 24L * 3 * 512, p.self.w2_kn + wave * GSZ, acc, lane);
+    const LnBwdIn<false, false> ln2 = glob_ln_bwd_load<false, false>(nullptr, 0, p.self.r2, p.self.ln2g, row0, rowEnd);
+    epilogue<RF, 8>(acc, Stg, As, row0, nullptr, [&](int, int) { return PrePool{}; },
+        [&](int row, int, float (&v)[8], const PrePool& pp, int) {
+          if (row < rowEnd) {
+#pragma unroll
+            for (int j = 0; j < 8; ++j) v[j] += pp.g[j] * pp.inv;
+          } else {
+#pragma unroll
+            for (int j = 0; j < 8; ++j) v[j] = 0.f;
+          }
+        }, true, nullptr, e);
+    __syncthreads();
+    stamp();
+    const QkvRows rows = {Qs, row0, nrows, row0, nrows};
+    glob_chain_bwd<DROP, false, true>(As, Stg, p.self, nullptr, 0, row0, rowEnd, sbase, R, sqkv, &ln2, &rows);
+    stamp();
+  } else {
   gemm_run<RF, 12, true>(R, Ks, cqkv + 12L * 3 * 512, cqkv + 24L * 3 * 512, acc, lane);
   gemm_run<RF, 12, true>(R, Vs, cqkv + 24L * 3 * 512, p.self.w2_kn + wave * GSZ, acc, lane);
   epilogue<RF, 8>(acc, Stg, As, row0, nullptr, [&](int, int) { return PreNone{}; },
@@ -1561,19 +1871,21 @@
   __syncthreads();
   stamp();
 
-  glob_chain_bwd<DROP, false>(As, Stg, p.self, nullptr, 0, row0, rowEnd, sbase, R, sqkv);
+  glob_chain_bwd<DROP, false, false>(As, Stg, p.self, nullptr, 0, row0, rowEnd, sbase, R, sqkv);
   stamp();
   load_rows32(Qs, p.self.q, p.self.ldq, 0, row0, nrows);
   load_rows32(Ks, p.self.k, p.self.ldk, 0, row0, nrows);
   load_rows32(Vs, p.self.v, p.self.ldv, 0, row0, nrows);
   __syncthreads();
+  }
   {
     const DropK dk_ = resolve_drop(p.self.d_attn, sbase);
     const bool on = pr_ < nrows;
     const int r = on ? pr_ : 0, sl = r / Cm, kr0 = sl * Cm, cpos = r - kr0;
-    const int nvalid = on ? (int)p.lens[v0 + sl] : 0;
+    const int nvalid = on ? (EARLY ? lens_s[sl] : (int)p.lens[v0 + sl]) : 0;
+    u32x4_t dqp[3];
     {
-      const float lse = on ? p.self.lse[(long)(row0 + r) * 8 + ph] : 0.f;
+      const float lse = EARLY ? lse_s : (on ? p.self.lse[(long)(row0 + r) * 8 + ph] : 0.f);
       float q[24], dO[24];
 #pragma unroll
       for (int c = 0; c < 3; ++c) {
@@ -1623,7 +1935,13 @@
 #pragma unroll
         for (int c = 0; c < 24; ++c) dq[c] += ds * kk[c];
       }
-      if (on) {
+      if constexpr (EARLY) {
+#pragma unroll
+        for (int c = 0; c < 3; ++c) {
+          dqp[c] = on ? pack8(&dq[c * 8]) : u32x4_t{0u, 0u, 0u, 0u};
+          if (on) gst16(p.self.dq, (unsigned)((row0 + r) * (int)p.self.lddq + coff + c * 8) * 2u, dqp[c]);
+        }
+      } else if (on) {
 #pragma unroll
         for (int c = 0; c < 3; ++c) gst16(p.self.dq, (unsigned)((row0 + r) * (int)p.self.lddq + coff + c * 8) * 2u, pack8(&dq[c * 8]));
       }
@@ -1659,7 +1977,20 @@
 #pragma unroll
         for (int c = 0; c < 24; ++c) { dkr[c] += ds * q[c]; dvr[c] += pd * dO[c]; }
       }
-      if (on) {
+      if constexpr (EARLY) {
+        lds_barrier();
+#pragma unroll
+        for (int c = 0; c < 3; ++c) {
+          const u32x4_t pk = on ? pack8(&dkr[c * 8]) : u32x4_t{0u, 0u, 0u, 0u}, pv = on ? pack8(&dvr[c * 8]) : u32x4_t{0u, 0u, 0u, 0u};
+          *reinterpret_cast<u32x4_t*>(&Qs[pr_ * APITCH + coff + c * 8]) = dqp[c];
+          *reinterpret_cast<u32x4_t*>(&Ks[pr_ * APITCH + coff + c * 8]) = pk;
+          *reinterpret_cast<u32x4_t*>(&Vs[pr_ * APITCH + coff + c * 8]) = pv;
+          if (on) {
+            gst16(p.self.dk, (unsigned)((row0 + r) * (int)p.self.lddk + coff + c * 8) * 2u, pk);
+            gst16(p.self.dv, (unsigned)((row0 + r) * (int)p.self.lddv + coff + c * 8) * 2u, pv);
+          }
+        }
+      } else if (on) {
 #pragma unroll
         for (int c = 0; c < 3; ++c) {
           gst16(p.self.dk, (unsigned)((row0 + r) * (int)p.self.lddk + coff + c * 8) * 2u, pack8(&dkr[c * 8]));
@@ -1668,29 +1999,41 @@
       }
     }
   }
-  __syncthreads();
+  if constexpr (EARLY) lds_barrier();
+  else __syncthreads();
   stamp();
   zero_acc<RF>(acc);
-  load_rows32(Qs, p.self.dq, p.self.lddq, 0, row0, nrows);
-  load_rows32(Ks, p.self.dk, p.self.lddk, 0, row0, nrows);
-  load_rows32(Vs, p.self.dv, p.self.lddv, 0, row0, nrows);
-  __syncthreads();
+  auto pre_dr1 = [&](int row, int col) { return PreRes{row < rowEnd ? gld16(p.self.dr1, (unsigned)(row * FZ_D + col) * 2u) : u32x4_t{0u, 0u, 0u, 0u}}; };
+  auto fn_dz = [&](int, int, float (&v)[8], const PreRes& pr, int) {
+    float r[8];
+    unpack8(pr.res, r);
+#pragma unroll
+    for (int j = 0; j < 8; ++j) v[j] += r[j];
+  };
+  const DropK none;
+  if constexpr (EARLY) {
+    const auto e = epi_early<false>(row0, nullptr, pre_dr1);
 #pragma unroll 1
-  for (int c = 0; c < 3; ++c) {
-    const bf16_t* Ts = c == 0 ? Qs : (c == 1 ? Ks : Vs);
-    gemm_run<RF, 12, true>(R, Ts, sqkv + (long)c * 12 * 3 * 512, sqkv + (long)(c < 2 ? c + 1 : c) * 12 * 3 * 512, acc, lane);
-  }
-  epilogue<RF, 8>(acc, Stg, As, row0, nullptr,
-      [&](int row, int col) { return PreRes{row < rowEnd ? gld16(p.self.dr1, (unsigned)(row * FZ_D + col) * 2u) : u32x4_t{0u, 0u, 0u, 0u}}; },
-      [&](int, int, float (&v)[8], const PreRes& pr, int) {
-        float r[8];
-        unpack8(pr.res, r);
-#pragma unroll
-        for (int j = 0; j < 8; ++j) v[j] += r[j];
-      }, true);
-  stamp();
-  {
-    const DropK none;
+    for (int c = 0; c < 3; ++c) {
+      const bf16_t* Ts = c == 0 ? Qs : (c == 1 ? Ks : Vs);
+      gemm_run<RF, 12, true>(R, Ts, sqkv + (long)c * 12 * 3 * 512, sqkv + (long)(c < 2 ? c + 1 : c) * 12 * 3 * 512, acc, lane);
+    }
+    const LnBwdIn<false, true> lnx = glob_ln_bwd_load<false, true>(nullptr, 0, p.x, p.n_gain, row0, rowEnd);
+    epilogue<RF, 8>(acc, Stg, As, row0, nullptr, pre_dr1, fn_dz, true, nullptr, e);
+    stamp();
+    glob_ln_bwd<false, false, false, true, true>(As, nullptr, 0, p.x, p.n_gain, row0, rowEnd, nullptr, nullptr, p.dx, none, none, Stg, p.g_n_gain, p.g_n_bias, &lnx);
+  } else {
+    load_rows32(Qs, p.self.dq, p.self.lddq, 0, row0, nrows);
+    load_rows32(Ks, p.self.dk, p.self.lddk, 0, row0, nrows);
+    load_rows32(Vs, p.self.dv, p.self.lddv, 0, row0, nrows);
+    __syncthreads();
+#pragma unroll 1
+    for (int c = 0; c < 3; ++c) {
+      const bf16_t* Ts = c == 0 ? Qs : (c == 1 ? Ks : Vs);
+      gemm_run<RF, 12, true>(R, Ts, sqkv + (long)c * 12 * 3 * 512, sqkv + (long)(c < 2 ? c + 1 : c) * 12 * 3 * 512, acc, lane);
+    }
+    epilogue<RF, 8>(acc, Stg, As, row0, nullptr, pre_dr1, fn_dz, true);
+    stamp();
     glob_ln_bwd<false, false, false, true>(As, nullptr, 0, p.x, p.n_gain, row0, rowEnd, nullptr, nullptr, p.dx, none, none, Stg, p.g_n_gain, p.g_n_bias);
   }
   stamp();
@@ -2066,6 +2409,9 @@
   if (first < 0 || count < 1 || first + count > 8) { first = 0; count = 8; }
   g_glob_xcd_first = first; g_glob_xcd_count = count;
 }
+static int g_glob_early_loads = 1;
+void set_glob_early_loads(int on) { g_glob_early_loads = on ? 1 : 0; }
+int get_glob_early_loads() { return g_glob_early_loads; }
 template <typename P>
 static int glob_grid(P& p, int tiles) {
   p.tiles = tiles;
@@ -2088,8 +2434,13 @@
                          p.ctx.d_ff1.thr && p.ctx.d_ff2.thr, "glob_fwd: dropout on some sites only");
   const double T = (double)p.B * p.Cmax;
   void* ts = timing_begin(TIMING_GLOB, 2.0 * 384.0 * 384.0 * (8.0 * T + 4.0 * p.B), 0, st);
-  if (drop) hipLaunchKernelGGL(glob_fwd_kernel<true>, dim3(grid), dim3(NTHR), 0, st, p);
-  else hipLaunchKernelGGL(glob_fwd_kernel<false>, dim3(grid), dim3(NTHR), 0, st, p);
+  if (g_glob_early_loads) {
+    if (drop) hipLaunchKernelGGL((glob_fwd_kernel<true, true>), dim3(grid), dim3(NTHR), 0, st, p);
+    else hipLaunchKernelGGL((glob_fwd_kernel<false, true>), dim3(grid), dim3(NTHR), 0, st, p);
+  } else {
+    if (drop) hipLaunchKernelGGL((glob_fwd_kernel<true, false>), dim3(grid), dim3(NTHR), 0, st, p);
+    else hipLaunchKernelGGL((glob_fwd_kernel<false, false>), dim3(grid), dim3(NTHR), 0, st, p);
+  }
   timing_end(ts, st);
   COOT_CHECK_LAUNCH("glob_fwd");
   return 0;
@@ -2106,8 +2457,13 @@
                          p.ctx.d_ff1.thr && p.ctx.d_ff2.thr && p.self.dr2m && p.ctx.dr2m, "glob_bwd: dropout on some sites only");
   const double T = (double)p.B * p.Cmax;
   void* ts = timing_begin(TIMING_GLOB, 2.0 * 384.0 * 384.0 * (6.0 * T + 6.0 * T + 4.0 * p.B), 0, st);
-  if (drop) hipLaunchKernelGGL(glob_bwd_kernel<true>, dim3(grid), dim3(NTHR), 0, st, p);
-  else hipLaunchKernelGGL(glob_bwd_kernel<false>, dim3(grid), dim3(NTHR), 0, st, p);
+  if (g_glob_early_loads) {
+    if (drop) hipLaunchKernelGGL((glob_bwd_kernel<true, true>), dim3(grid), dim3(NTHR), 0, st, p);
+    else hipLaunchKernelGGL((glob_bwd_kernel<false, true>), dim3(grid), dim3(NTHR), 0, st, p);
+  } else {
+    if (drop) hipLaunchKernelGGL((glob_bwd_kernel<true, false>), dim3(grid), dim3(NTHR), 0, st, p);
+    else hipLaunchKernelGGL((glob_bwd_kernel<false, false>), dim3(grid), dim3(NTHR), 0, st, p);
+  }
   timing_end(ts, st);
   COOT_CHECK_LAUNCH("glob_bwd");
   return 0;
```

Result: no change. 224,100 clip-pairs/s (median of 4 runs) (+0.2%).
